# tailuzhecom/wiser

Hardware: AMD Instinct MI355X
Metric: queries/sec + p50 lat, 2-term AND BM25 top-10 on Wikipedia, 1/2/4/8 GPU (higher is better)
Workload: dtype u32/f64; 1 GPU; C3 stand-in (en-Wikipedia-shaped): 5500000 docs, the en-Wikipedia df histogram x 1 (gen_synthetic_log.py:8-16), 100000 two-term AND queries (:191-214 rule, seed 7), 4096 queries per GPU per step, top-10, device-resident; global_batch=4096, parallelism=replicas1, k=10

## Files before the change

include/wiser_hip.h:

```cpp
#ifndef WISER_HIP_H
#define WISER_HIP_H

#include <stdint.h>

#ifdef __cplusplus
extern "C" {
#endif

#define WSR_MAX_TERMS 16
#define WSR_MAX_QUERY_TERMS 1024
#define WSR_MAX_PHRASE_TERMS 8
#define WSR_MAX_OR_TERMS 16
#define WSR_MAX_K 1024
#define WSR_SERVER_MAX_K WSR_MAX_K

enum {
  WSR_OK = 0,
  WSR_E_INVALID = -1,
  WSR_E_IO = -2,
  WSR_E_HIP = -3,
  WSR_E_LIMIT = -4,
  WSR_E_INTERNAL = -5
};

typedef struct wsr_handle wsr_handle;
typedef struct wsr_batch wsr_batch;

typedef struct wsr_open_opts {
  int32_t device;
  uint32_t doc_lo;
  uint32_t doc_hi;
  int32_t threads;
  int32_t positions;
  int32_t bloom_factor;
} wsr_open_opts;

typedef struct wsr_query {
  int32_t n_terms;
  int32_t k;
  int32_t list_ids[WSR_MAX_TERMS];
  int32_t flags;
  const int32_t* more_ids;
} wsr_query;
#define WSR_QUERY_PHRASE 1
#define WSR_QUERY_OR 2

typedef struct wsr_hit {
  int32_t doc_id;
  int32_t pad;
  double score;
} wsr_hit;

int wsr_snippet(wsr_handle* h, const wsr_query* q, int32_t doc_id, int32_t n_passages,
                char* out, int32_t cap, int32_t* len);
int wsr_snippets_batch(wsr_handle* h, const wsr_query* q, int32_t nq, const wsr_hit* hits,
                       const int32_t* n_hits, int32_t stride, int32_t n_passages, int32_t threads,
                       char* buf, uint64_t cap, uint64_t* ends, uint64_t* total);
int wsr_doc_get(wsr_handle* h, int32_t doc_id, char* out, int32_t cap, int32_t* len);
typedef struct wsr_docs wsr_docs;
int wsr_docs_open(const char* dir, wsr_docs** out);
void wsr_docs_close(wsr_docs* d);
int wsr_docs_lookup(wsr_docs* d, const char* term, int32_t* list_id, int32_t* doc_freq);
int wsr_docs_snippet(wsr_docs* d, const wsr_query* q, int32_t doc_id, int32_t n_passages, char* out,
                     int32_t cap, int32_t* len);
int wsr_docs_get(wsr_docs* d, int32_t doc_id, char* out, int32_t cap, int32_t* len);
int wsr_highlight(const int32_t* pairs, const int32_t* counts, int32_t n_terms, int32_t n_passages,
                  const char* text, char* out, int32_t cap, int32_t* len);

typedef struct wsr_batch_stats {
  uint64_t work_items;
  uint64_t survivors;
  uint64_t driver_blocks;
  uint64_t other_blocks;
  uint64_t algo_bytes;
  double plan_ms, segment_ms, replay_ms;
  uint64_t events;
  uint64_t max_query_events;
  double lean_ms;
  uint64_t skippable_blocks;
} wsr_batch_stats;

typedef struct wsr_image_info {
  uint64_t total_bytes;
  uint64_t blob_bytes;
  uint64_t dense_bytes;
  uint64_t tf8_bytes;
  uint64_t plen_bytes;
  uint64_t dir_bytes;
  uint64_t pos_bytes;
  uint32_t n_lists, dense_lists;
  uint64_t impact_bytes;
} wsr_image_info;

const char* wsr_last_error(void);
const char* wsr_version(void);
int wsr_runtime_info(char* buf, int32_t cap);

int wsr_open(const char* vacuum_dir, const wsr_open_opts* opts, wsr_handle** out);
void wsr_close(wsr_handle* h);
int wsr_image_info_get(wsr_handle* h, wsr_image_info* out);
int wsr_image_size(const char* dir, uint32_t doc_lo, uint32_t doc_hi, int32_t positions, int32_t bloom_factor,
                   int32_t threads, wsr_image_info* out);
int wsr_term_count(wsr_handle* h, int32_t* out);
int wsr_n_docs(wsr_handle* h, int32_t* out);
int wsr_lookup(wsr_handle* h, const char* term, int32_t* list_id, int32_t* doc_freq);
int wsr_list_bytes(wsr_handle* h, int32_t list_id, uint64_t* out);
int wsr_impact_byte(double avg, uint32_t tf, uint32_t c4, uint32_t* byte, double* value);

int wsr_check_query(wsr_handle* h, const wsr_query* q);

int wsr_search_batch(wsr_handle* h, const wsr_query* q, int32_t nq, int32_t hit_stride,
                     wsr_hit* hits, int32_t* n_hits);

int wsr_resolve_text(wsr_handle* h, const char* text, int64_t len, int32_t k, int32_t max_q,
                     wsr_query* q, int32_t* nq, int32_t* more_store, int64_t more_cap);
int wsr_search_text(wsr_handle* h, const char* text, int64_t len, int32_t k, int32_t hit_stride,
                    int32_t max_q, wsr_hit* hits, int32_t* n_hits, int32_t* nq);

int wsr_class_order(const wsr_query* q, int32_t nq, int32_t* order, int32_t* n_conj);

int wsr_batch_create(wsr_handle* h, int32_t max_queries, int32_t hit_stride, wsr_batch** out);
void wsr_batch_destroy(wsr_handle* h, wsr_batch* b);
int wsr_batch_upload(wsr_handle* h, wsr_batch* b, const wsr_query* q, int32_t nq);
int wsr_batch_run(wsr_handle* h, wsr_batch* b);
int wsr_sync(wsr_handle* h);
int wsr_batch_fetch(wsr_handle* h, wsr_batch* b, wsr_hit* hits, int32_t* n_hits);
int wsr_batch_stats_get(wsr_handle* h, wsr_batch* b, wsr_batch_stats* out);
typedef struct wsr_or_stats {
  uint64_t items, windows, windows_skipped, touched_docs, events;
} wsr_or_stats;
int wsr_batch_or_stats_get(wsr_handle* h, wsr_batch* b, wsr_or_stats* out);
int wsr_batch_fetch_cols(wsr_handle* h, wsr_batch* b, wsr_hit* hits, int32_t* n_hits, int32_t cols);
int wsr_pinned_alloc(uint64_t bytes, void** out);
void wsr_pinned_free(void* p);
int wsr_batch_ready(wsr_handle* h, wsr_batch* b);

typedef struct wsr_server wsr_server;
typedef struct wsr_serve_stats {
  uint64_t queries;
  double seconds, qps;
  double p50_ms, p99_ms;
  uint64_t batches;
  double mean_batch;
  double queue_ms;
  double gpu_ms;
  double handoff_ms;
} wsr_serve_stats;
int wsr_server_open(wsr_handle* h, int32_t max_batch, int32_t window_us, wsr_server** out);
void wsr_server_close(wsr_server* s);
int wsr_server_search(wsr_server* s, const wsr_query* q, wsr_hit* hits, int32_t* n_hits);
int wsr_server_bench(wsr_server* s, const wsr_query* q, int32_t nq, int32_t n_clients,
                     int32_t depth, double seconds, wsr_serve_stats* st);

int wsr_batch_fetch_range(wsr_handle* h, wsr_batch* b, int32_t q0, int32_t nq, wsr_hit* hits,
                          int32_t* n_hits);
int wsr_stream(wsr_handle* h, void** stream);
int wsr_batch_stream(wsr_handle* h, wsr_batch* b, void** stream);
int wsr_shard_fill(wsr_handle* h, wsr_batch* b, int32_t n_owners, int64_t* owner_totals);

#define WSR_COMM_ID_BYTES 128
typedef struct wsr_comm wsr_comm;
int wsr_comm_unique_id(uint8_t* id );
int wsr_comm_open(const uint8_t* id, int32_t world, int32_t rank, int32_t device, wsr_comm** out);
void wsr_comm_close(wsr_comm* c);
int wsr_shard_step(wsr_handle* h, wsr_batch* b, wsr_comm* c, int32_t q_per_owner, int64_t slot);
int wsr_shard_steps(wsr_handle* h, wsr_batch* const* b, int32_t n, wsr_comm* c, int32_t q_per_owner,
                    int64_t slot);
int wsr_comm_flush(wsr_comm* c);
typedef struct wsr_comm_stats {
  int64_t groups, steps, replays_in_lean, replays_on_stream;
} wsr_comm_stats;
int wsr_comm_stats_get(wsr_comm* c, wsr_comm_stats* out);
typedef struct wsr_loopback wsr_loopback;
int wsr_loopback_create(int32_t world, wsr_loopback** out);
void wsr_loopback_destroy(wsr_loopback* l);
int wsr_comm_open_loopback(wsr_loopback* l, int32_t rank, int32_t device, wsr_comm** out);
int wsr_shard_step_regions(int32_t q_per_owner, int64_t slot, uint64_t* region_bytes);
int wsr_shard_step_emit(wsr_handle* h, wsr_batch* b, int32_t world, int32_t q_per_owner, int64_t slot,
                        void* host_send);
int wsr_shard_step_replay(wsr_handle* h, wsr_batch* b, int32_t rank, int32_t world, int32_t q_per_owner,
                          int64_t slot, const void* host_recv);
int wsr_shard_step_replay_deferred(wsr_handle* h, wsr_batch* b, int32_t rank, int32_t world, int32_t q_per_owner,
                                   int64_t slot, const void* host_recv);
int wsr_shard_step_emit_async(wsr_handle* h, wsr_batch* b, int32_t world, int32_t q_per_owner, int64_t slot,
                              void* host_send);
int wsr_batch_stream_sync(wsr_handle* h, wsr_batch* b);
int wsr_batch_set_item_blocks(wsr_handle* h, wsr_batch* b, int32_t blocks);

int wsr_debug_decode_block(wsr_handle* h, int32_t list_id, int32_t block, int32_t which,
                           uint32_t* out, int32_t* count);

int wsr_debug_wg_stats(wsr_handle* h, wsr_batch* b, uint32_t* out, int32_t max_words,
                       int32_t* n_wg, int32_t* stride);

enum {
  WSR_CLASS_TWO_CONJ = 1 << 0,
  WSR_CLASS_ONE_CONJ = 1 << 1,
  WSR_CLASS_HAS_PHRASE = 1 << 2,
  WSR_CLASS_TWO_PH = 1 << 3,
  WSR_CLASS_HAS_WIDE = 1 << 4,
  WSR_CLASS_GEN_PHRASE = 1 << 5,
  WSR_CLASS_HAS_CONJ_LEAN = 1 << 6,
  WSR_CLASS_HAS_GEN = 1 << 7,
  WSR_CLASS_HAS_OR = 1 << 8,
  WSR_CLASS_RAN_CONJ = 1 << 9,
  WSR_CLASS_RAN_GEN = 1 << 10
};
int wsr_debug_batch_class(wsr_handle* h, wsr_batch* b, uint32_t* flags);

int wsr_debug_fail_runs(int32_t n);

int wsr_debug_dense_lookup(const char* dir, uint32_t doc_lo, uint32_t doc_hi, uint32_t dense_div,
                           const char* term, const uint32_t* docs, int32_t n, int32_t* tf_out,
                           int32_t* is_dense);

typedef struct wsr_build_stats {
  int64_t n_docs, n_terms, n_postings, vacuum_bytes, docs_char4_ge_0x80;
  double avg_length;
} wsr_build_stats;

int wsr_build_from_linedoc(const char* linedoc, int64_t n_rows, const char* format,
                           const char* out_dir, wsr_build_stats* st);
int wsr_build_from_linedoc_bloom(const char* linedoc, int64_t n_rows, const char* format,
                                 const char* out_dir, float ratio, int32_t expected_entries,
                                 wsr_build_stats* st);
int wsr_build_synthetic(const char* out_dir, int64_t n_docs, int64_t vocab, double zipf_s,
                        uint64_t seed, int32_t with_positions, int32_t threads,
                        wsr_build_stats* st);
int wsr_build_wiki_standin(const char* out_dir, int64_t n_docs, double term_scale, uint64_t seed,
                           int32_t threads, wsr_build_stats* st);
int wsr_build_wiki_standin_topics(const char* out_dir, int64_t n_docs, double term_scale, uint64_t seed,
                                  int32_t threads, int32_t topics, int32_t topics_per_term, double affinity,
                                  wsr_build_stats* st);
int wsr_gen_two_term_log(const char* index_dir, int64_t n_queries, uint64_t seed,
                         const char* out_path, int64_t* n_written);
int wsr_gen_mixed_log(const char* index_dir, int64_t n_queries, uint64_t seed,
                      const char* out_path, int64_t* n_written);
int wsr_gen_single_term_log(const char* index_dir, int32_t high, int64_t n_queries, uint64_t seed,
                            const char* out_path, int64_t* n_written);
int wsr_gen_phrase_log(const char* index_dir, int64_t n_queries, uint64_t seed,
                       const char* out_path, int64_t* n_written);

#ifdef __cplusplus
}
#endif

#endif
```

wiser_amd/_capi.py:

```python
from __future__ import annotations

import ctypes as C
import os
import re

HERE = os.path.dirname(os.path.abspath(__file__))
LIB_PATH = os.environ.get("WISER_HIP_LIB") or os.path.join(HERE, "_lib", "libwiser_hip.so")
HEADER = os.path.join(os.path.dirname(HERE), "include", "wiser_hip.h")

MAX_TERMS = 16
MAX_QUERY_TERMS = 1024
MAX_PHRASE_TERMS = 8
MAX_OR_TERMS = 16
MAX_K = 1024
SERVER_MAX_K = MAX_K

WSR_OK = 0
E_INVALID, E_IO, E_HIP, E_LIMIT, E_INTERNAL = -1, -2, -3, -4, -5
ERRORS = {-1: "WSR_E_INVALID", -2: "WSR_E_IO", -3: "WSR_E_HIP", -4: "WSR_E_LIMIT",
          -5: "WSR_E_INTERNAL"}


QUERY_PHRASE = 1
QUERY_OR = 2

CLASS_BITS = {"two_conj": 1 << 0, "one_conj": 1 << 1, "has_phrase": 1 << 2, "two_ph": 1 << 3,
              "has_wide": 1 << 4, "gen_phrase": 1 << 5, "has_conj_lean": 1 << 6, "has_gen": 1 << 7,
              "has_or": 1 << 8, "ran_conj": 1 << 9, "ran_gen": 1 << 10}


class OpenOpts(C.Structure):
    _fields_ = [("device", C.c_int32), ("doc_lo", C.c_uint32), ("doc_hi", C.c_uint32),
                ("threads", C.c_int32), ("positions", C.c_int32), ("bloom_factor", C.c_int32)]


class Query(C.Structure):
    _fields_ = [("n_terms", C.c_int32), ("k", C.c_int32), ("list_ids", C.c_int32 * MAX_TERMS),
                ("flags", C.c_int32), ("more_ids", C.POINTER(C.c_int32))]


class Hit(C.Structure):
    _fields_ = [("doc_id", C.c_int32), ("pad", C.c_int32), ("score", C.c_double)]


class BatchStats(C.Structure):
    _fields_ = [("work_items", C.c_uint64), ("survivors", C.c_uint64),
                ("driver_blocks", C.c_uint64), ("other_blocks", C.c_uint64),
                ("algo_bytes", C.c_uint64), ("plan_ms", C.c_double),
                ("segment_ms", C.c_double), ("replay_ms", C.c_double),
                ("events", C.c_uint64), ("max_query_events", C.c_uint64),
                ("lean_ms", C.c_double), ("skippable_blocks", C.c_uint64)]


class OrStats(C.Structure):
    _fields_ = [("items", C.c_uint64), ("windows", C.c_uint64), ("windows_skipped", C.c_uint64),
                ("touched_docs", C.c_uint64), ("events", C.c_uint64)]


class ImageInfo(C.Structure):
    _fields_ = [("total_bytes", C.c_uint64), ("blob_bytes", C.c_uint64), ("dense_bytes", C.c_uint64),
                ("tf8_bytes", C.c_uint64), ("plen_bytes", C.c_uint64), ("dir_bytes", C.c_uint64),
                ("pos_bytes", C.c_uint64), ("n_lists", C.c_uint32), ("dense_lists", C.c_uint32),
                ("impact_bytes", C.c_uint64)]


class ServeStats(C.Structure):
    _fields_ = [("queries", C.c_uint64), ("seconds", C.c_double), ("qps", C.c_double),
                ("p50_ms", C.c_double), ("p99_ms", C.c_double), ("batches", C.c_uint64),
                ("mean_batch", C.c_double), ("queue_ms", C.c_double), ("gpu_ms", C.c_double),
                ("handoff_ms", C.c_double)]


class CommStats(C.Structure):
    _fields_ = [("groups", C.c_int64), ("steps", C.c_int64), ("replays_in_lean", C.c_int64),
                ("replays_on_stream", C.c_int64)]


class BuildStats(C.Structure):
    _fields_ = [("n_docs", C.c_int64), ("n_terms", C.c_int64), ("n_postings", C.c_int64),
                ("vacuum_bytes", C.c_int64), ("docs_char4_ge_0x80", C.c_int64),
                ("avg_length", C.c_double)]


class WiserError(RuntimeError):
    def __init__(self, code, msg):
        super().__init__(f"{ERRORS.get(code, code)}: {msg}")
        self.code = code


if not os.path.exists(LIB_PATH):
    raise ImportError(f"{LIB_PATH} is missing: build it with `make` or __graft_entry__.build() "
                      "(the HIP engine has no CPU fallback)")

lib = C.CDLL(LIB_PATH)

_P = C.c_void_p
_sigs = {
    "wsr_last_error": (C.c_char_p, []),
    "wsr_version": (C.c_char_p, []),
    "wsr_runtime_info": (C.c_int, [C.c_char_p, C.c_int32]),
    "wsr_open": (C.c_int, [C.c_char_p, C.POINTER(OpenOpts), C.POINTER(_P)]),
    "wsr_close": (None, [_P]),
    "wsr_image_info_get": (C.c_int, [_P, C.POINTER(ImageInfo)]),
    "wsr_image_size": (C.c_int, [C.c_char_p, C.c_uint32, C.c_uint32, C.c_int32, C.c_int32, C.c_int32,
                                 C.POINTER(ImageInfo)]),
    "wsr_term_count": (C.c_int, [_P, C.POINTER(C.c_int32)]),
    "wsr_n_docs": (C.c_int, [_P, C.POINTER(C.c_int32)]),
    "wsr_lookup": (C.c_int, [_P, C.c_char_p, C.POINTER(C.c_int32), C.POINTER(C.c_int32)]),
    "wsr_list_bytes": (C.c_int, [_P, C.c_int32, C.POINTER(C.c_uint64)]),
    "wsr_impact_byte": (C.c_int, [C.c_double, C.c_uint32, C.c_uint32, C.POINTER(C.c_uint32),
                                  C.POINTER(C.c_double)]),
    "wsr_search_batch": (C.c_int, [_P, C.POINTER(Query), C.c_int32, C.c_int32, C.POINTER(Hit),
                                   C.POINTER(C.c_int32)]),
    "wsr_check_query": (C.c_int, [_P, C.POINTER(Query)]),
    "wsr_resolve_text": (C.c_int, [_P, C.c_char_p, C.c_int64, C.c_int32, C.c_int32, C.POINTER(Query),
                                   C.POINTER(C.c_int32), C.POINTER(C.c_int32), C.c_int64]),
    "wsr_search_text": (C.c_int, [_P, C.c_char_p, C.c_int64, C.c_int32, C.c_int32, C.c_int32,
                                  C.POINTER(Hit), C.POINTER(C.c_int32), C.POINTER(C.c_int32)]),
    "wsr_class_order": (C.c_int, [C.POINTER(Query), C.c_int32, C.POINTER(C.c_int32), C.POINTER(C.c_int32)]),
    "wsr_batch_create": (C.c_int, [_P, C.c_int32, C.c_int32, C.POINTER(_P)]),
    "wsr_batch_destroy": (None, [_P, _P]),
    "wsr_batch_upload": (C.c_int, [_P, _P, C.POINTER(Query), C.c_int32]),
    "wsr_batch_run": (C.c_int, [_P, _P]),
    "wsr_sync": (C.c_int, [_P]),
    "wsr_batch_fetch": (C.c_int, [_P, _P, C.POINTER(Hit), C.POINTER(C.c_int32)]),
    "wsr_batch_stats_get": (C.c_int, [_P, _P, C.POINTER(BatchStats)]),
    "wsr_batch_or_stats_get": (C.c_int, [_P, _P, C.POINTER(OrStats)]),
    "wsr_batch_fetch_range": (C.c_int, [_P, _P, C.c_int32, C.c_int32, C.POINTER(Hit),
                                        C.POINTER(C.c_int32)]),
    "wsr_stream": (C.c_int, [_P, C.POINTER(_P)]),
    "wsr_batch_stream": (C.c_int, [_P, _P, C.POINTER(_P)]),
    "wsr_shard_fill": (C.c_int, [_P, _P, C.c_int32, C.POINTER(C.c_int64)]),
    "wsr_comm_unique_id": (C.c_int, [C.POINTER(C.c_uint8)]),
    "wsr_comm_open": (C.c_int, [C.POINTER(C.c_uint8), C.c_int32, C.c_int32, C.c_int32, C.POINTER(_P)]),
    "wsr_comm_close": (None, [_P]),
    "wsr_loopback_create": (C.c_int, [C.c_int32, C.POINTER(_P)]),
    "wsr_loopback_destroy": (None, [_P]),
    "wsr_comm_open_loopback": (C.c_int, [_P, C.c_int32, C.c_int32, C.POINTER(_P)]),
    "wsr_comm_flush": (C.c_int, [_P]),
    "wsr_comm_stats_get": (C.c_int, [_P, C.POINTER(CommStats)]),
    "wsr_shard_step": (C.c_int, [_P, _P, _P, C.c_int32, C.c_int64]),
    "wsr_shard_steps": (C.c_int, [_P, _P, C.c_int32, _P, C.c_int32, C.c_int64]),
    "wsr_shard_step_emit_async": (C.c_int, [_P, _P, C.c_int32, C.c_int32, C.c_int64, _P]),
    "wsr_batch_stream_sync": (C.c_int, [_P, _P]),
    "wsr_batch_set_item_blocks": (C.c_int, [_P, _P, C.c_int32]),
    "wsr_shard_step_regions": (C.c_int, [C.c_int32, C.c_int64, C.POINTER(C.c_uint64)]),
    "wsr_shard_step_emit": (C.c_int, [_P, _P, C.c_int32, C.c_int32, C.c_int64, _P]),
    "wsr_shard_step_replay": (C.c_int, [_P, _P, C.c_int32, C.c_int32, C.c_int32, C.c_int64, _P]),
    "wsr_shard_step_replay_deferred": (C.c_int, [_P, _P, C.c_int32, C.c_int32, C.c_int32, C.c_int64, _P]),
    "wsr_debug_wg_stats": (C.c_int, [_P, _P, C.POINTER(C.c_uint32), C.c_int32,
                                     C.POINTER(C.c_int32), C.POINTER(C.c_int32)]),
    "wsr_debug_batch_class": (C.c_int, [_P, _P, C.POINTER(C.c_uint32)]),
    "wsr_debug_fail_runs": (C.c_int, [C.c_int32]),
    "wsr_debug_decode_block": (C.c_int, [_P, C.c_int32, C.c_int32, C.c_int32,
                                         C.POINTER(C.c_uint32), C.POINTER(C.c_int32)]),
    "wsr_debug_dense_lookup": (C.c_int, [C.c_char_p, C.c_uint32, C.c_uint32, C.c_uint32, C.c_char_p,
                                         C.POINTER(C.c_uint32), C.c_int32, C.POINTER(C.c_int32),
                                         C.POINTER(C.c_int32)]),
    "wsr_build_from_linedoc": (C.c_int, [C.c_char_p, C.c_int64, C.c_char_p, C.c_char_p,
                                         C.POINTER(BuildStats)]),
    "wsr_build_from_linedoc_bloom": (C.c_int, [C.c_char_p, C.c_int64, C.c_char_p, C.c_char_p,
                                               C.c_float, C.c_int32, C.POINTER(BuildStats)]),
    "wsr_build_synthetic": (C.c_int, [C.c_char_p, C.c_int64, C.c_int64, C.c_double, C.c_uint64,
                                      C.c_int32, C.c_int32, C.POINTER(BuildStats)]),
    "wsr_build_wiki_standin": (C.c_int, [C.c_char_p, C.c_int64, C.c_double, C.c_uint64,
                                         C.c_int32, C.POINTER(BuildStats)]),
    "wsr_build_wiki_standin_topics": (C.c_int, [C.c_char_p, C.c_int64, C.c_double, C.c_uint64, C.c_int32,
                                                C.c_int32, C.c_int32, C.c_double, C.POINTER(BuildStats)]),
    "wsr_gen_two_term_log": (C.c_int, [C.c_char_p, C.c_int64, C.c_uint64, C.c_char_p,
                                       C.POINTER(C.c_int64)]),
    "wsr_batch_ready": (C.c_int, [_P, _P]),
    "wsr_pinned_alloc": (C.c_int, [C.c_uint64, C.POINTER(_P)]),
    "wsr_pinned_free": (None, [_P]),
    "wsr_batch_fetch_cols": (C.c_int, [_P, _P, C.POINTER(Hit), C.POINTER(C.c_int32), C.c_int32]),
    "wsr_server_open": (C.c_int, [_P, C.c_int32, C.c_int32, C.POINTER(_P)]),
    "wsr_server_close": (None, [_P]),
    "wsr_server_search": (C.c_int, [_P, C.POINTER(Query), C.POINTER(Hit), C.POINTER(C.c_int32)]),
    "wsr_server_bench": (C.c_int, [_P, C.POINTER(Query), C.c_int32, C.c_int32, C.c_int32,
                                   C.c_double, C.POINTER(ServeStats)]),
    "wsr_gen_mixed_log": (C.c_int, [C.c_char_p, C.c_int64, C.c_uint64, C.c_char_p,
                                    C.POINTER(C.c_int64)]),
    "wsr_gen_single_term_log": (C.c_int, [C.c_char_p, C.c_int32, C.c_int64, C.c_uint64, C.c_char_p,
                                          C.POINTER(C.c_int64)]),
    "wsr_gen_phrase_log": (C.c_int, [C.c_char_p, C.c_int64, C.c_uint64, C.c_char_p,
                                     C.POINTER(C.c_int64)]),
    "wsr_snippet": (C.c_int, [_P, C.POINTER(Query), C.c_int32, C.c_int32, C.c_char_p, C.c_int32,
                              C.POINTER(C.c_int32)]),
    "wsr_doc_get": (C.c_int, [_P, C.c_int32, C.c_char_p, C.c_int32, C.POINTER(C.c_int32)]),
    "wsr_snippets_batch": (C.c_int, [_P, C.POINTER(Query), C.c_int32, C.POINTER(Hit),
                                     C.POINTER(C.c_int32), C.c_int32, C.c_int32, C.c_int32, C.c_char_p,
                                     C.c_uint64, C.POINTER(C.c_uint64), C.POINTER(C.c_uint64)]),
    "wsr_docs_open": (C.c_int, [C.c_char_p, C.POINTER(_P)]),
    "wsr_docs_close": (None, [_P]),
    "wsr_docs_lookup": (C.c_int, [_P, C.c_char_p, C.POINTER(C.c_int32), C.POINTER(C.c_int32)]),
    "wsr_docs_snippet": (C.c_int, [_P, C.POINTER(Query), C.c_int32, C.c_int32, C.c_char_p, C.c_int32,
                                   C.POINTER(C.c_int32)]),
    "wsr_docs_get": (C.c_int, [_P, C.c_int32, C.c_char_p, C.c_int32, C.POINTER(C.c_int32)]),
    "wsr_highlight": (C.c_int, [C.POINTER(C.c_int32), C.POINTER(C.c_int32), C.c_int32, C.c_int32,
                                C.c_char_p, C.c_char_p, C.c_int32, C.POINTER(C.c_int32)]),
}
for _name, (_res, _args) in _sigs.items():
    _f = getattr(lib, _name)
    _f.restype = _res
    _f.argtypes = _args


def check(rc):
    if rc != WSR_OK:
        raise WiserError(rc, lib.wsr_last_error().decode(errors="replace"))
    return rc


def text_call(fn, *args, cap: int = 4096) -> str:
    while True:
        buf = C.create_string_buffer(cap)
        n = C.c_int32()
        check(fn(*args, buf, cap, C.byref(n)))
        if n.value <= cap:
            return buf.raw[: n.value].decode("utf-8", errors="surrogateescape")
        cap = n.value


def snippets_batch(h, queries, hits, n_hits, stride: int, n_passages: int, threads: int = 0):
    nq = len(n_hits)
    ends = (C.c_uint64 * max(1, nq * stride))()
    total = C.c_uint64()
    cap = 1 << 16
    while True:
        buf = C.create_string_buffer(cap)
        rc = lib.wsr_snippets_batch(h, queries, nq, hits, n_hits, stride, n_passages, threads, buf, cap,
                                    ends, C.byref(total))
        if rc == -4 and total.value > cap:
            cap = total.value
            continue
        check(rc)
        break
    raw = buf.raw
    out, at = [], 0
    for i in range(nq):
        row = []
        for j in range(stride):
            e = ends[i * stride + j]
            if j < n_hits[i]:
                row.append(raw[at:e].decode("utf-8", errors="surrogateescape"))
            at = e
        out.append(row)
    return out


def highlight(offsets, n_passages: int, text: str) -> str:
    flat = [v for term in offsets for pr in term for v in pr]
    pairs = (C.c_int32 * max(1, len(flat)))(*flat)
    counts = (C.c_int32 * max(1, len(offsets)))(*[len(t) for t in offsets])
    return text_call(lib.wsr_highlight, pairs, counts, len(offsets), n_passages, text.encode())


def header_symbols(path: str = HEADER):
    text = open(path).read()
    return sorted(set(re.findall(r"^\s*(?:const\s+)?[\w\s\*]+?\b(wsr_\w+)\s*\(", text, re.M)))


def runtime_info() -> str:
    buf = C.create_string_buffer(1024)
    check(lib.wsr_runtime_info(buf, 1024))
    return buf.value.decode()
```

wiser_amd/csrc/engine.cc:

```cpp
#include <hip/hip_runtime.h>
#include <rccl/rccl.h>
#include <dlfcn.h>

#include <cstdio>

#include <algorithm>
#include <atomic>
#include <cmath>
#include <cstring>
#include <memory>
#include <cstdlib>
#include <mutex>
#include <stdexcept>
#include <string>
#include <thread>
#include <vector>

#include "engine_impl.h"
#include "format.h"
#include "writer.h"

using namespace wiser;

namespace wiser {
thread_local std::string g_err;
void set_last_error(const std::string& msg) { g_err = msg; }
}

namespace {

template <class T, class A>
uint64_t dev_upload(gpu::DevBuf<T>& dst, const std::vector<T, A>& src) {
  dst.alloc(std::max<size_t>(src.size(), 1));
  if (!src.empty()) HIP_OK(hipMemcpy(dst.get(), src.data(), src.size() * sizeof(T), hipMemcpyHostToDevice));
  return dst.bytes();
}

}

namespace {
template <class V>
uint64_t dev_bytes(const V& v) {
  return std::max<uint64_t>(v.size(), 1) * sizeof(typename V::value_type);
}

wsr_image_info image_info_of(const HostImage& img, size_t n_c4) {
  wsr_image_info o{};
  if (img.has_blooms) o.pos_bytes += dev_bytes(img.blm) + dev_bytes(img.blm_hash);
  if (img.has_positions)
    o.pos_bytes += dev_bytes(img.pos_blob) + dev_bytes(img.pos_lists) + dev_bytes(img.pos_pk) +
                   dev_bytes(img.pos_tail) + dev_bytes(img.pos_start);
  o.dense_bytes = dev_bytes(img.dense) + dev_bytes(img.dense_rank) + dev_bytes(img.bkt);
  o.tf8_bytes = dev_bytes(img.tf8);
  o.blob_bytes = dev_bytes(img.blob);
  o.plen_bytes = dev_bytes(img.plen);
  o.dir_bytes = dev_bytes(img.tails) + dev_bytes(img.lists) + dev_bytes(img.blocks) + dev_bytes(img.blk_last) +
                dev_bytes(img.blk_meta) + dev_bytes(img.bmax) + std::max<uint64_t>(n_c4, 1);
  o.impact_bytes = dev_bytes(img.impact);
  o.dir_bytes += o.impact_bytes;
  o.dense_lists = img.dense_lists;
  o.n_lists = static_cast<uint32_t>(img.lists.size());
  o.total_bytes = o.blob_bytes + o.dense_bytes + o.tf8_bytes + o.plen_bytes + o.dir_bytes + o.pos_bytes;
  return o;
}

uint32_t dense_div_knob() { return static_cast<uint32_t>(env_number("WSR_DENSE_DIV", 8192)); }
uint64_t dense_budget_knob() { return static_cast<uint64_t>(env_number("WSR_DENSE_BUDGET_GB", 48) * 1e9); }
}

extern "C" {

const char* wsr_last_error(void) { return g_err.c_str(); }
const char* wsr_version(void) { return "wiser-hip 0.2 (gfx950)"; }

int wsr_image_info_get(wsr_handle* h, wsr_image_info* out) {
  if (!h || !out) return fail(WSR_E_INVALID, "null argument");
  *out = h->info;
  out->total_bytes = out->blob_bytes + out->dense_bytes + out->tf8_bytes + out->plen_bytes + out->dir_bytes +
                     out->pos_bytes;
  return WSR_OK;
}


int wsr_image_size(const char* dir, uint32_t doc_lo, uint32_t doc_hi, int32_t positions, int32_t bloom_factor,
                   int32_t threads, wsr_image_info* out) {
  if (!dir || !out) return fail(WSR_E_INVALID, "null argument");
  try {
    VacuumIndex idx;
    idx.open(dir);
    const int t = threads > 0 ? threads : static_cast<int>(std::thread::hardware_concurrency());
    const HostImage img = build_image(idx, doc_lo, doc_hi ? doc_hi : 0xFFFFFFFFu, std::min(t, 32), dense_div_knob(),
                                      positions != 0, dense_budget_knob(), positions && bloom_factor > 0);
    *out = image_info_of(img, idx.char4_lengths().size());
  } catch (const std::exception& e) {
    return fail(WSR_E_IO, e.what());
  }
  return WSR_OK;
}

int wsr_runtime_info(char* buf, int32_t cap) {
  if (!buf || cap <= 0) return fail(WSR_E_INVALID, "null argument");
  int ver = 0;
  (void)hipRuntimeGetVersion(&ver);
  Dl_info hip{}, rccl{};
  const char* hp = dladdr(reinterpret_cast<void*>(&hipRuntimeGetVersion), &hip) && hip.dli_fname ? hip.dli_fname : "?";
  const char* rp = dladdr(reinterpret_cast<void*>(&ncclGetUniqueId), &rccl) && rccl.dli_fname ? rccl.dli_fname : "?";
  std::snprintf(buf, static_cast<size_t>(cap), "hipRuntimeGetVersion=%d libamdhip64=%s librccl=%s", ver, hp, rp);
  return WSR_OK;
}

int wsr_open(const char* dir, const wsr_open_opts* opts, wsr_handle** out) {
  if (!dir || !out) return fail(WSR_E_INVALID, "null argument");
  *out = nullptr;
  std::unique_ptr<wsr_handle> h(new wsr_handle());
  try {
    h->idx.open(dir);
    h->docs.open(dir);
    h->rows.reset(new SkipRowCache(h->idx));
  } catch (const std::exception& e) {
    return fail(WSR_E_IO, e.what());
  }
  try {
    const int dev = opts ? opts->device : 0;
    int ndev = 0;
    if (hipGetDeviceCount(&ndev) != hipSuccess || ndev <= dev)
      return fail(WSR_E_HIP, "no HIP device " + std::to_string(dev) + " (MI355X required; no CPU fallback)");
    HIP_OK(hipSetDevice(dev));
    h->device = dev;
    uint32_t lo = opts ? opts->doc_lo : 0, hi = opts ? opts->doc_hi : 0;
    if (hi == 0) hi = 0xFFFFFFFFu;
    int threads = opts && opts->threads > 0 ? opts->threads : static_cast<int>(std::thread::hardware_concurrency());
    const uint32_t dense_div = dense_div_knob();
    const uint64_t dense_budget = dense_budget_knob();
    const float dense_ratio = static_cast<float>(env_number("WSR_DENSE_RATIO", 1.0));
    h->positions = opts && opts->positions;
    const uint32_t bloom_factor = opts && opts->bloom_factor > 0 ? static_cast<uint32_t>(opts->bloom_factor) : 0u;
    size_t hbm_free = 0, hbm_total = 0;
    HIP_OK(hipMemGetInfo(&hbm_free, &hbm_total));
    HostImage img = build_image(h->idx, lo, hi, std::min(threads, 32), dense_div, h->positions, dense_budget,
                                bloom_factor > 0, hbm_free);
    if (img.has_blooms) {
      h->info.pos_bytes += dev_upload(h->d_blm, img.blm);
      h->info.pos_bytes += dev_upload(h->d_blm_hash, img.blm_hash);
      h->args.blm = reinterpret_cast<const uint4*>(h->d_blm.get());
      h->args.blm_hash = reinterpret_cast<const uint2*>(h->d_blm_hash.get());
      h->args.blm_bits = img.blm_bits;
      h->args.blm_hashes = img.blm_hashes;
      h->args.bloom_factor = bloom_factor;
      big_vector<uint8_t>().swap(img.blm);
    }
    if (h->positions) {
      h->info.pos_bytes += dev_upload(h->d_pos_blob, img.pos_blob);
      h->info.pos_bytes += dev_upload(h->d_pos_lists, img.pos_lists);
      h->info.pos_bytes += dev_upload(h->d_pos_pk, img.pos_pk);
      h->info.pos_bytes += dev_upload(h->d_pos_tail, img.pos_tail);
      h->info.pos_bytes += dev_upload(h->d_pos_start, img.pos_start);
      h->args.pos_blob = h->d_pos_blob.get();
      h->args.pos_lists = h->d_pos_lists.get();
      h->args.pos_pk = reinterpret_cast<const uint2*>(h->d_pos_pk.get());
      h->args.pos_tail = h->d_pos_tail.get();
      h->args.pos_start = reinterpret_cast<const uint2*>(h->d_pos_start.get());
      h->pos_bytes = img.pos_list_bytes;
      std::vector<uint8_t>().swap(img.pos_blob);
      std::vector<uint32_t>().swap(img.pos_start);
    }
    h->info.dense_bytes = dev_upload(h->d_dense, img.dense);
    h->info.dense_bytes += dev_upload(h->d_dense_rk, img.dense_rank);
    h->info.dense_bytes += dev_upload(h->d_bkt, img.bkt);
    h->info.tf8_bytes = dev_upload(h->d_tf8, img.tf8);
    h->dense_lists = img.dense_lists;
    h->info.dense_lists = img.dense_lists;
    h->info.n_lists = static_cast<uint32_t>(img.lists.size());
    h->args.dense = h->d_dense.get();
    h->args.dense_rk = h->d_dense_rk.get();
    h->args.bkt = reinterpret_cast<const uint2*>(h->d_bkt.get());
    h->args.tf8 = h->d_tf8.get();
    h->args.dense_span = img.dense_span;
    h->args.dense_ratio = dense_ratio;
    h->args.seg_cap = kSegCost;
    h->info.blob_bytes = dev_upload(h->d_blob, img.blob);
    h->info.plen_bytes = dev_upload(h->d_plen, img.plen);
    h->args.plen = h->d_plen.get();
    h->info.impact_bytes = dev_upload(h->d_impact, img.impact);
    h->info.dir_bytes += h->info.impact_bytes;
    h->args.impact = h->d_impact.get();
    {
      float nm = static_cast<float>(img.norm_min);
      if (static_cast<double>(nm) > img.norm_min) nm = std::nextafter(nm, 0.0f);
      h->args.norm_min = nm;
    }
    h->info.dir_bytes += dev_upload(h->d_bmax, img.bmax);
    h->args.bmax = h->d_bmax.get();
    h->info.dir_bytes += dev_upload(h->d_tails, img.tails);
    h->args.tails = h->d_tails.get();
    h->info.dir_bytes += dev_upload(h->d_lists, img.lists);
    h->info.dir_bytes += dev_upload(h->d_blocks, img.blocks);
    h->info.dir_bytes += dev_upload(h->d_last, img.blk_last);
    h->info.dir_bytes += dev_upload(h->d_meta, img.blk_meta);
    h->info.dir_bytes += dev_upload(h->d_c4, h->idx.char4_lengths());
    std::vector<double> cache(h->idx.bm25_cache(), h->idx.bm25_cache() + 256);
    dev_upload(h->d_cache, cache);
    h->lists = img.lists;
    h->blocks.assign(img.blocks.begin(), img.blocks.end());
    h->meta.assign(img.blk_meta.begin(), img.blk_meta.end());
    h->list_bytes = img.list_bytes;
    h->args.blob = h->d_blob.get();
    h->args.lists = h->d_lists.get();
    h->args.blocks = h->d_blocks.get();
    h->args.blk_last = h->d_last.get();
    h->args.blk_meta = h->d_meta.get();
    h->args.c4 = h->d_c4.get();
    h->args.cache = h->d_cache.get();
    h->args.n_c4 = static_cast<uint32_t>(h->idx.char4_lengths().size());
    h->args.n_lists = static_cast<uint32_t>(img.lists.size());
    h->args.doc_lo = lo;
    h->args.doc_hi = hi;
    h->args.avg = h->idx.avg_length();
    h->stream = gpu::make_stream();

    hipDeviceProp_t prop;
    HIP_OK(hipGetDeviceProperties(&prop, dev));
    int occ = segment_kernel_occupancy();
    if (occ < 1) occ = 1;
    h->grid = prop.multiProcessorCount * std::min(occ, 32);
    const int gen_per_cu = static_cast<int>(env_number("WSR_GEN_PER_CU", 4));
    h->gen_cap = prop.multiProcessorCount * std::max(1, std::min(std::min(occ, 32), gen_per_cu) + 1);
    int locc = lean_kernel_occupancy(false);
    if (locc < 1) locc = 1;
    h->lean_wgs = prop.multiProcessorCount * std::min(locc, 16);
    int pocc = lean_kernel_occupancy(true);
    if (pocc < 1) pocc = 1;
    h->lean_wgs_ph = prop.multiProcessorCount * std::min(std::min(pocc, locc), 16);
    h->lean_wgs_two = prop.multiProcessorCount * std::min(locc + 1, 16);
  } catch (const std::exception& e) {
    return fail(WSR_E_HIP, e.what());
  }
  *out = h.release();
  return WSR_OK;
}

void wsr_close(wsr_handle* h) {
  if (!h) return;
  for (wsr_batch* b : h->pool) wsr_batch_destroy(h, b);
  h->pool.clear();
  if (h->stream) (void)hipStreamSynchronize(h->stream);
  delete h;
}

int wsr_term_count(wsr_handle* h, int32_t* out) {
  if (!h || !out) return fail(WSR_E_INVALID, "null argument");
  *out = h->idx.n_lists();
  return WSR_OK;
}

int wsr_n_docs(wsr_handle* h, int32_t* out) {
  if (!h || !out) return fail(WSR_E_INVALID, "null argument");
  *out = h->idx.n_docs();
  return WSR_OK;
}

int wsr_lookup(wsr_handle* h, const char* term, int32_t* list_id, int32_t* df) {
  if (!h || !term) return fail(WSR_E_INVALID, "null argument");
  const int32_t id = h->idx.find(term);
  if (list_id) *list_id = id;
  if (df) *df = id < 0 ? 0 : static_cast<int32_t>(h->idx.df(id));
  return WSR_OK;
}

struct wsr_docs {
  VacuumIndex idx;
  DocStore docs;
  std::unique_ptr<SkipRowCache> rows;
};

namespace {
int copy_out(const std::string& s, char* out, int32_t cap, int32_t* len) {
  if (len) *len = static_cast<int32_t>(s.size());
  if (out && cap > 0) std::memcpy(out, s.data(), std::min<size_t>(s.size(), static_cast<size_t>(cap)));
  return WSR_OK;
}

int check_snippet_query(const VacuumIndex& idx, const DocStore& docs, const wsr_query* q) {
  if (q->n_terms < 1 || q->n_terms > WSR_MAX_QUERY_TERMS) return fail(WSR_E_LIMIT, "bad term count");
  if (q->n_terms > WSR_MAX_TERMS && !q->more_ids) return fail(WSR_E_INVALID, "more_ids missing");
  if (q->flags & WSR_QUERY_OR) return fail(WSR_E_INVALID, "no snippets for a disjunctive query");
  if (!docs.is_open()) return fail(WSR_E_INVALID, "the index has no doc store (my.fdx / my.fdt)");
  for (int32_t id : query_terms(*q))
    if (id < 0 || id >= idx.n_lists())
      return fail(WSR_E_INVALID, "a query term is not in the index (no result entries)");
  return WSR_OK;
}

int snippet_of(const VacuumIndex& idx, const SkipRowCache& rows, const DocStore& docs, const wsr_query* q,
               int32_t doc, int32_t n_passages, char* out, int32_t cap, int32_t* len) {
  if (!q || !len || n_passages < 0) return fail(WSR_E_INVALID, "bad snippet arguments");
  const int rc = check_snippet_query(idx, docs, q);
  if (rc != WSR_OK) return rc;
  try {
    const std::vector<int32_t> ids = query_terms(*q);
    return copy_out(make_snippet(idx, rows, docs, ids.data(), q->n_terms,
                                 (q->flags & WSR_QUERY_PHRASE) != 0, doc, n_passages),
                    out, cap, len);
  } catch (const std::exception& e) {
    return fail(WSR_E_INVALID, e.what());
  }
}

int doc_text(const DocStore& docs, int32_t doc, char* out, int32_t cap, int32_t* len) {
  if (!len) return fail(WSR_E_INVALID, "null argument");
  try {
    return copy_out(docs.get(doc), out, cap, len);
  } catch (const std::exception& e) {
    return fail(WSR_E_INVALID, e.what());
  }
}
}

int wsr_snippet(wsr_handle* h, const wsr_query* q, int32_t doc, int32_t n_passages, char* out,
                int32_t cap, int32_t* len) {
  if (!h) return fail(WSR_E_INVALID, "null argument");
  return snippet_of(h->idx, *h->rows, h->docs, q, doc, n_passages, out, cap, len);
}

int wsr_snippets_batch(wsr_handle* h, const wsr_query* q, int32_t nq, const wsr_hit* hits,
                       const int32_t* n_hits, int32_t stride, int32_t n_passages, int32_t threads,
                       char* buf, uint64_t cap, uint64_t* ends, uint64_t* total) {
  if (!h || (nq > 0 && (!q || !hits || !n_hits || !ends)) || !total || nq < 0 || stride <= 0 ||
      n_passages < 0)
    return fail(WSR_E_INVALID, "bad snippet batch arguments");
  std::vector<std::pair<int32_t, int32_t>> work;
  for (int32_t i = 0; i < nq; ++i) {
    if (n_hits[i] < 0 || n_hits[i] > stride) return fail(WSR_E_INVALID, "bad hit count");
    if (n_hits[i] == 0) continue;
    const int rc = check_snippet_query(h->idx, h->docs, &q[i]);
    if (rc != WSR_OK) return rc;
    for (int32_t j = 0; j < n_hits[i]; ++j) work.emplace_back(i, j);
  }
  std::vector<std::string> out(static_cast<size_t>(nq) * stride);
// ... 578 lines not shown
  auto disj = [&](int32_t i) { return (q[i].flags & WSR_QUERY_OR) != 0; };
  auto phrase = [&](int32_t i) {
    return !disj(i) && (q[i].flags & WSR_QUERY_PHRASE) != 0 && q[i].n_terms > 1;
  };
  int32_t n = 0;
  for (int32_t i = 0; i < nq; ++i)
    if (!phrase(i) && !disj(i)) order[n++] = i;
  *n_conj = n;
  for (int32_t i = 0; i < nq; ++i)
    if (phrase(i)) order[n++] = i;
  for (int32_t i = 0; i < nq; ++i)
    if (disj(i)) order[n++] = i;
  return WSR_OK;
}

int wsr_shard_fill(wsr_handle* h, wsr_batch* b, int32_t n_owners, int64_t* owner_totals) {
  if (!h || !b || !b->x.fused || !owner_totals || n_owners <= 0 || n_owners > b->x.world)
    return fail(WSR_E_INVALID, "call wsr_shard_step (or wsr_shard_step_emit) first");
  try {
    HIP_OK(hipSetDevice(h->device));
    HIP_OK(hipStreamSynchronize(b->st));
    if (b->x.join()) HIP_OK(hipEventSynchronize(b->x.ev[1]));
    std::vector<uint32_t> fill(n_owners);
    HIP_OK(hipMemcpy(fill.data(), b->d_ctr + kNumCounters, sizeof(uint32_t) * n_owners, hipMemcpyDeviceToHost));
    for (int i = 0; i < n_owners; ++i) owner_totals[i] = fill[i];
  } catch (const std::exception& e) {
    return fail(WSR_E_HIP, e.what());
  }
  return WSR_OK;
}

int wsr_batch_stream(wsr_handle* h, wsr_batch* b, void** stream) {
  if (!h || !b || !stream) return fail(WSR_E_INVALID, "null argument");
  *stream = b->st;
  return WSR_OK;
}

int wsr_batch_set_item_blocks(wsr_handle* h, wsr_batch* b, int32_t blocks) {
  if (!h || !b || blocks < 1 || blocks > kSegCost) return fail(WSR_E_INVALID, "item blocks must be 1..63");
  b->seg_cap = static_cast<uint32_t>(blocks);
  return WSR_OK;
}

int wsr_batch_stream_sync(wsr_handle* h, wsr_batch* b) {
  if (!h || !b) return fail(WSR_E_INVALID, "null argument");
  const hipError_t e = hipStreamSynchronize(b->st);
  return e == hipSuccess ? WSR_OK : fail(WSR_E_HIP, hipGetErrorString(e));
}

int wsr_batch_fetch_range(wsr_handle* h, wsr_batch* b, int32_t q0, int32_t nq, wsr_hit* hits,
                          int32_t* n_hits) {
  if (!h || !b || q0 < 0 || nq < 0 || q0 + nq > b->nq) return fail(WSR_E_INVALID, "bad range");
  try {
    HIP_OK(hipSetDevice(h->device));
    HIP_OK(hipStreamSynchronize(b->st));
    if (b->x.join()) HIP_OK(hipEventSynchronize(b->x.ev[1]));
    uint32_t ctr[kNumCounters];
    HIP_OK(hipMemcpy(ctr, b->d_ctr, sizeof ctr, hipMemcpyDeviceToHost));
    if (ctr[kCtrError])
      return fail(WSR_E_INTERNAL, "device reported error flags " + std::to_string(ctr[kCtrError]) +
                                      (ctr[kCtrError] & kErrExchange ? " (an exchange slot overflowed)" : ""));
    if (nq && hits)
      HIP_OK(hipMemcpy(hits, b->d_hits + static_cast<size_t>(q0) * b->stride,
                       sizeof(HitDev) * static_cast<size_t>(nq) * b->stride, hipMemcpyDeviceToHost));
    if (nq && n_hits)
      HIP_OK(hipMemcpy(n_hits, b->d_nhits + q0, sizeof(int32_t) * nq, hipMemcpyDeviceToHost));
  } catch (const std::exception& e) {
    return fail(WSR_E_HIP, e.what());
  }
  return WSR_OK;
}

int wsr_stream(wsr_handle* h, void** stream) {
  if (!h || !stream) return fail(WSR_E_INVALID, "null argument");
  *stream = h->stream;
  return WSR_OK;
}

int wsr_debug_decode_block(wsr_handle* h, int32_t id, int32_t block, int32_t which, uint32_t* out,
                           int32_t* count) {
  if (!h || !out || id < 0 || id >= static_cast<int32_t>(h->lists.size()))
    return fail(WSR_E_INVALID, "bad list id");
  const ListDev& L = h->lists[id];
  if (block < 0 || static_cast<uint32_t>(block) >= L.nblk) return fail(WSR_E_INVALID, "bad block");
  std::lock_guard<std::mutex> g(h->mu);
  const BlockDev& bd = h->blocks[L.blk0 + block];
  const uint32_t cnt = static_cast<uint32_t>(block) == L.nblk - 1 ? L.tail_cnt : 128u;
  try {
    gpu::DevBuf<uint32_t> d_out;
    d_out.alloc(128);
    const uint8_t* p = h->d_blob.get() + L.base + (which ? bd.tf_rel : bd.doc_rel);
    const uint32_t bits = which ? (h->meta[L.blk0 + block] >> 8) : (h->meta[L.blk0 + block] & 0xFF);
    HIP_OK(launch_decode_probe(p, bits, cnt, which == 0, bd.prev, d_out, h->stream));
    HIP_OK(hipStreamSynchronize(h->stream));
    HIP_OK(hipMemcpy(out, d_out, d_out.bytes(), hipMemcpyDeviceToHost));
  } catch (const std::exception& ex) {
    return fail(WSR_E_HIP, ex.what());
  }
  if (count) *count = static_cast<int32_t>(cnt);
  return WSR_OK;
}

int wsr_debug_wg_stats(wsr_handle* h, wsr_batch* b, uint32_t* out, int32_t max_words,
                       int32_t* n_wg, int32_t* stride) {
  if (!h || !b) return fail(WSR_E_INVALID, "null argument");
  std::lock_guard<std::mutex> g(h->mu);
  const int rows = b->cls.seg_grid + kLeanWaves * (b->cls.lean_wgs + (b->cls.has_phrase ? b->cls.lean_wgs_ph : 0));
  if (n_wg) *n_wg = rows;
  if (stride) *stride = kStatStride;
  if (!out) return WSR_OK;
  const size_t n = std::min<size_t>(static_cast<size_t>(std::max(max_words, 0)),
                                    static_cast<size_t>(kStatStride) * rows);
  try {
    HIP_OK(hipStreamSynchronize(b->st));
    if (b->x.join()) HIP_OK(hipEventSynchronize(b->x.ev[1]));
    HIP_OK(hipMemcpy(out, b->d_stats, n * sizeof(uint32_t), hipMemcpyDeviceToHost));
  } catch (const std::exception& e) {
    return fail(WSR_E_HIP, e.what());
  }
  return WSR_OK;
}

int wsr_debug_batch_class(wsr_handle* h, wsr_batch* b, uint32_t* flags) {
  if (!h || !b || !flags) return fail(WSR_E_INVALID, "null argument");
  const BatchClass& c = b->cls;
  *flags = (c.two_conj ? WSR_CLASS_TWO_CONJ : 0u) | (c.one_conj ? WSR_CLASS_ONE_CONJ : 0u) |
           (c.has_phrase ? WSR_CLASS_HAS_PHRASE : 0u) | (c.two_ph ? WSR_CLASS_TWO_PH : 0u) |
           (c.has_wide ? WSR_CLASS_HAS_WIDE : 0u) | (c.gen_phrase ? WSR_CLASS_GEN_PHRASE : 0u) |
           (c.has_conj_lean ? WSR_CLASS_HAS_CONJ_LEAN : 0u) | (c.has_gen ? WSR_CLASS_HAS_GEN : 0u) |
           (c.has_or ? WSR_CLASS_HAS_OR : 0u) | (b->launched.conj ? WSR_CLASS_RAN_CONJ : 0u) |
           (b->launched.gen ? WSR_CLASS_RAN_GEN : 0u);
  return WSR_OK;
}

int wsr_debug_dense_lookup(const char* dir, uint32_t doc_lo, uint32_t doc_hi, uint32_t dense_div,
                           const char* term, const uint32_t* docs, int32_t n, int32_t* tf_out,
                           int32_t* is_dense) {
  if (!dir || !term || (n > 0 && (!docs || !tf_out))) return fail(WSR_E_INVALID, "null argument");
  try {
    VacuumIndex idx;
    idx.open(dir);
    const HostImage img = build_image(idx, doc_lo, doc_hi ? doc_hi : 0xFFFFFFFFu, 4, dense_div);
    const int32_t id = idx.find(term);
    const bool dense = id >= 0 && img.lists[id].bm != kNoDense;
    if (is_dense) *is_dense = dense ? 1 : 0;
    for (int32_t i = 0; i < n; ++i)
      tf_out[i] = dense ? static_cast<int32_t>(dense_lookup_host(img, img.lists[id], docs[i])) : -1;
  } catch (const std::exception& e) {
    return fail(WSR_E_IO, e.what());
  }
  return WSR_OK;
}

static void fill_stats(const BuildStats& s, wsr_build_stats* st) {
  if (!st) return;
  st->n_docs = s.n_docs;
  st->n_terms = s.n_terms;
  st->n_postings = s.n_postings;
  st->vacuum_bytes = s.vacuum_bytes;
  st->docs_char4_ge_0x80 = s.docs_char4_ge_0x80;
  st->avg_length = s.avg_length;
}

int wsr_build_from_linedoc(const char* linedoc, int64_t n_rows, const char* format,
                           const char* out_dir, wsr_build_stats* st) {
  if (!linedoc || !format || !out_dir) return fail(WSR_E_INVALID, "null argument");
  try {
    fill_stats(build_from_linedoc(linedoc, n_rows, format, out_dir), st);
  } catch (const std::exception& e) {
    return fail(WSR_E_IO, e.what());
  }
  return WSR_OK;
}

int wsr_build_from_linedoc_bloom(const char* linedoc, int64_t n_rows, const char* format,
                                 const char* out_dir, float ratio, int32_t expected_entries,
                                 wsr_build_stats* st) {
  if (!linedoc || !format || !out_dir) return fail(WSR_E_INVALID, "null argument");
  if (!(ratio > 0.0f && ratio < 1.0f) || expected_entries < 1)
    return fail(WSR_E_INVALID, "bloom ratio must be in (0, 1) and expected entries >= 1");
  try {
    BloomSpec b;
    b.on = true;
    b.ratio = ratio;
    b.entries = expected_entries;
    fill_stats(build_from_linedoc(linedoc, n_rows, format, out_dir, b), st);
  } catch (const std::exception& e) {
    return fail(WSR_E_IO, e.what());
  }
  return WSR_OK;
}

int wsr_build_synthetic(const char* out_dir, int64_t n_docs, int64_t vocab, double zipf_s,
                        uint64_t seed, int32_t with_positions, int32_t threads,
                        wsr_build_stats* st) {
  if (!out_dir || n_docs <= 0 || vocab <= 0) return fail(WSR_E_INVALID, "bad arguments");
  try {
    SyntheticSpec sp;
    sp.n_docs = n_docs;
    sp.vocab = vocab;
    sp.zipf_s = zipf_s;
    sp.seed = seed;
    sp.with_positions = with_positions != 0;
    sp.threads = threads;
    fill_stats(build_synthetic(sp, out_dir), st);
  } catch (const std::exception& e) {
    return fail(WSR_E_IO, e.what());
  }
  return WSR_OK;
}

int wsr_build_wiki_standin(const char* out_dir, int64_t n_docs, double term_scale, uint64_t seed,
                           int32_t threads, wsr_build_stats* st) {
  if (!out_dir || n_docs < 16 || !(term_scale > 0)) return fail(WSR_E_INVALID, "bad arguments");
  try {
    WikiSpec sp;
    sp.n_docs = n_docs;
    sp.term_scale = term_scale;
    sp.seed = seed;
    sp.threads = threads;
    fill_stats(build_wiki_standin(sp, out_dir), st);
  } catch (const std::exception& e) {
    return fail(WSR_E_IO, e.what());
  }
  return WSR_OK;
}

int wsr_build_wiki_standin_topics(const char* out_dir, int64_t n_docs, double term_scale, uint64_t seed,
                                  int32_t threads, int32_t topics, int32_t topics_per_term, double affinity,
                                  wsr_build_stats* st) {
  if (!out_dir || n_docs < 16 || !(term_scale > 0) || topics < 1 || topics_per_term < 1 || topics_per_term > 16 ||
      !(affinity >= 0 && affinity <= 1) || topics > n_docs)
    return fail(WSR_E_INVALID, "bad arguments");
  try {
    WikiSpec sp;
    sp.n_docs = n_docs;
    sp.term_scale = term_scale;
    sp.seed = seed;
    sp.threads = threads;
    sp.topics = topics;
    sp.topics_per_term = topics_per_term;
    sp.affinity = affinity;
    fill_stats(build_wiki_standin(sp, out_dir), st);
  } catch (const std::exception& e) {
    return fail(WSR_E_IO, e.what());
  }
  return WSR_OK;
}

int wsr_gen_two_term_log(const char* index_dir, int64_t n_queries, uint64_t seed,
                         const char* out_path, int64_t* n_written) {
  if (!index_dir || !out_path) return fail(WSR_E_INVALID, "null argument");
  try {
    int64_t n = gen_two_term_log(index_dir, n_queries, seed, out_path);
    if (n_written) *n_written = n;
  } catch (const std::exception& e) {
    return fail(WSR_E_IO, e.what());
  }
  return WSR_OK;
}

int wsr_gen_mixed_log(const char* index_dir, int64_t n_queries, uint64_t seed,
                      const char* out_path, int64_t* n_written) {
  if (!index_dir || !out_path) return fail(WSR_E_INVALID, "null argument");
  try {
    int64_t n = gen_mixed_log(index_dir, n_queries, seed, out_path);
    if (n_written) *n_written = n;
  } catch (const std::exception& e) {
    return fail(WSR_E_IO, e.what());
  }
  return WSR_OK;
}

int wsr_gen_single_term_log(const char* index_dir, int32_t high, int64_t n_queries, uint64_t seed,
                      const char* out_path, int64_t* n_written) {
  if (!index_dir || !out_path) return fail(WSR_E_INVALID, "null argument");
  try {
    int64_t n = gen_single_term_log(index_dir, high != 0, n_queries, seed, out_path);
    if (n_written) *n_written = n;
  } catch (const std::exception& e) {
    return fail(WSR_E_IO, e.what());
  }
  return WSR_OK;
}

int wsr_gen_phrase_log(const char* index_dir, int64_t n_queries, uint64_t seed,
                       const char* out_path, int64_t* n_written) {
  if (!index_dir || !out_path) return fail(WSR_E_INVALID, "null argument");
  try {
    int64_t n = gen_phrase_log(index_dir, n_queries, seed, out_path);
    if (n_written) *n_written = n;
  } catch (const std::exception& e) {
    return fail(WSR_E_IO, e.what());
  }
  return WSR_OK;
}

}
```

wiser_amd/csrc/engine_impl.h:

```cpp
#pragma once

#include <hip/hip_runtime.h>

#include <atomic>
#include <cstdlib>
#include <deque>
#include <memory>
#include <mutex>
#include <string>
#include <vector>

#include "../../include/wiser_hip.h"
#include "batch_plan.h"
#include "dev_mem.h"
#include "engine_types.h"
#include "index.h"
#include "kernels.h"
#include "shard_layout.h"
#include "snippet.h"

namespace wiser {
extern thread_local std::string g_err;
inline int fail(int code, const std::string& msg) {
  g_err = msg;
  return code;
}

inline double env_number(const char* name, double dflt) {
  const char* v = std::getenv(name);
  if (!v || !*v) return dflt;
  char* end = nullptr;
  const double x = std::strtod(v, &end);
  return (end && *end == 0 && x >= 0) ? x : dflt;
}
}

struct wsr_handle {
  std::mutex mu;
  int device = 0;
  gpu::Stream stream;
  wiser::VacuumIndex idx;
  wiser::DocStore docs;
  std::unique_ptr<wiser::SkipRowCache> rows;
  std::mutex pool_mu;
  std::vector<wsr_batch*> pool;
  wiser::IndexArgs args{};
  gpu::DevBuf<uint8_t> d_blob;
  gpu::DevBuf<wiser::ListDev> d_lists;
  gpu::DevBuf<wiser::BlockDev> d_blocks;
  gpu::DevBuf<uint32_t> d_last, d_meta;
  gpu::DevBuf<uint8_t> d_c4;
  gpu::DevBuf<double> d_cache;
  gpu::DevBuf<wiser::DenseEnt> d_dense;
  gpu::DevBuf<uint32_t> d_dense_rk;
  gpu::DevBuf<uint32_t> d_bkt;
  gpu::DevBuf<uint8_t> d_tf8, d_plen, d_impact;
  gpu::DevBuf<float> d_bmax;
  gpu::DevBuf<uint32_t> d_tails;
  gpu::DevBuf<uint8_t> d_pos_blob;
  gpu::DevBuf<wiser::PosDev> d_pos_lists;
  gpu::DevBuf<uint32_t> d_pos_pk, d_pos_tail, d_pos_start;
  gpu::DevBuf<uint8_t> d_blm;
  gpu::DevBuf<uint32_t> d_blm_hash;
  bool positions = false;
  uint32_t dense_lists = 0;
  wsr_image_info info{};
  std::vector<wiser::ListDev> lists;
  std::vector<uint64_t> list_bytes;
  std::vector<uint64_t> pos_bytes;
  std::vector<wiser::BlockDev> blocks;
  std::vector<uint32_t> meta;
  std::mutex hdef_mu;
  std::deque<wsr_batch*> hdef_q;
  int grid = 0;
  int lean_wgs = 0;
  int lean_wgs_ph = 0;
  int lean_wgs_two = 0;
  int gen_cap = 0;
  wiser::ImageView view() const {
    wiser::ImageView v;
    v.lists = lists.data();
    v.n_lists = lists.size();
    v.blocks = blocks.data();
    v.n_blocks = blocks.size();
    v.list_bytes = list_bytes.data();
    v.pos_bytes = pos_bytes.empty() ? nullptr : pos_bytes.data();
    v.dense_ratio = args.dense_ratio;
    v.doc_lo = args.doc_lo;
    v.doc_hi = args.doc_hi;
    v.positions = positions;
    v.lean_wgs = lean_wgs;
    v.lean_wgs_two = lean_wgs_two;
    v.lean_wgs_ph = lean_wgs_ph;
    v.gen_cap = gen_cap;
    return v;
  }
};

struct ShardExchange {
  explicit ShardExchange(wsr_batch* b) : batch(b) {}
  wsr_batch* const batch;
  gpu::DevBuf<wiser::Event> send, recv;
  int pairs = 0;
  gpu::Event ev[2];
  std::atomic<bool> pending{false};
  std::atomic<uint64_t> req{0};
  std::atomic<uint64_t> enq{0};
  std::atomic<wsr_comm*> comm{nullptr};
  bool fused = false;
  std::atomic<wsr_handle*> hdef{nullptr};
  int32_t hdef_rank = 0;
  int world = 0, qpr = 0;
  int64_t slot = 0;
  wiser::ShardLayout layout() const { return wiser::ShardLayout(qpr, slot); }

  void request() { req.fetch_add(1, std::memory_order_acq_rel); }
  void enqueued(bool ok, bool deferred) {
    if (ok) pending = true;
    if (deferred) comm.store(nullptr, std::memory_order_release);
    enq.fetch_add(1, std::memory_order_release);
  }
  bool join();
};

struct wsr_batch {
  int max_q = 0, stride = 0, nq = 0;
  gpu::DevBuf<uint8_t> d_qb;
  wiser::QueryIn* d_q() const { return reinterpret_cast<wiser::QueryIn*>(d_qb.get()); }
  gpu::DevBuf<wiser::QueryPlan> d_plan;
  gpu::DevBuf<wiser::QueryDesc> d_desc;
  gpu::DevBuf<wiser::PlanPart> d_part;
  gpu::DevBuf<uint32_t> d_ctr;
  gpu::PinnedBuf<uint32_t> h_ctr;
  gpu::DevBuf<wiser::Event> d_events;
  gpu::DevBuf<uint32_t> d_evcnt, d_itemq;
  gpu::DevBuf<wiser::HitDev> d_hits;
  gpu::DevBuf<int32_t> d_nhits;
  gpu::DevBuf<uint32_t> d_qdone;
  gpu::DevBuf<uint64_t> d_pub;
  gpu::DevBuf<uint32_t> d_stats;
  gpu::DevBuf<uint32_t> d_ph;
  wiser::BatchClass cls;
  wiser::Launches launched;
  uint32_t seg_cap = wiser::kSegCost;
  ShardExchange x{this};
  gpu::DevBuf<wiser::OrQuery> d_orq;
  gpu::DevBuf<wiser::OrItem> d_oritem;
  gpu::DevBuf<uint32_t> d_orevcnt;
  gpu::DevBuf<wiser::Event> d_orev;
  gpu::DevBuf<unsigned long long> d_orstat;
  gpu::Event ev[5];
  gpu::Stream st, st2, st_pad;
  gpu::Event fork, join, join_ph;
  bool ran = false;
};

int batch_run(wsr_handle* h, wsr_batch* b, const wiser::EmitView* se = nullptr, const wiser::OwnerJob* oj = nullptr);
wsr_batch* take_host_replay(wsr_handle* h, const wsr_batch* b, wiser::OwnerJob* oj);
bool host_replay_enqueue(wsr_batch* pb, wsr_handle* h);
```

wiser_amd/csrc/engine_types.h:

```cpp
#pragma once

#include <cstdint>

namespace wiser {

constexpr int kMaxTerms = 16;
constexpr int kMaxQueryTerms = 1024;
constexpr int kMaxPhraseTerms = 8;
constexpr int kMaxK = 64;
constexpr int kMaxKWide = 1024;

struct ListDev {
  uint64_t base;
  uint32_t blk0;
  uint32_t nblk;
  uint32_t df;
  uint32_t tail_cnt;
  double idf;
  uint64_t bm;
  uint64_t tf8;
  uint64_t tail;
  uint32_t last;
  uint32_t tfmax;
};
static_assert(sizeof(ListDev) == 64, "ListDev layout");
constexpr uint64_t kNoTail = ~0ull;

constexpr uint64_t kNoDense = ~0ull;
constexpr uint8_t kTf8Escape = 255;

constexpr float kImpactScale = 0x1.010102p-8f;
inline double impact_value(uint32_t q) { return static_cast<double>(static_cast<float>(q) * kImpactScale); }
inline uint8_t impact_byte(uint32_t tf, double nrm) {
  const double f = static_cast<double>(static_cast<int32_t>(tf));
  const double x = f / (f + nrm);
  if (!(x > 0.0)) return 0;
  if (!(x < 1.0)) return 255;
  uint32_t q = static_cast<uint32_t>(x * 255.0);
  while (q < 255 && impact_value(q) < x) ++q;
  return static_cast<uint8_t>(q);
}

constexpr uint32_t kProbeShiftBit = 56;
constexpr uint64_t kProbeBaseMask = (1ull << kProbeShiftBit) - 1;
constexpr uint32_t kBucketDensity = 40;
constexpr uint32_t kBucketMinShift = 3, kBucketMaxShift = 8;
constexpr uint32_t kBucketInline = 4;
constexpr uint32_t kBucketWindow = 9;
constexpr uint32_t kBucketCrowdedDiv = 1024;
inline uint32_t probe_shift(uint64_t bm) { return static_cast<uint32_t>(bm >> kProbeShiftBit); }
inline uint64_t bucket_count(uint32_t span, uint32_t c) { return (static_cast<uint64_t>(span) + (1u << c) - 1) >> c; }
inline uint32_t bucket_shift(uint64_t n, uint32_t span) {
  if (!span || n * kBucketDensity >= span || n >= (1u << 23) - 1024) return 0;
  uint32_t c = kBucketMinShift;
  while (c < kBucketMaxShift && (n << (c + 1)) <= 2ull * span) ++c;
  return c;
}
inline uint64_t bucket_words(uint64_t n, uint32_t span, uint32_t c) {
  return 2 * bucket_count(span, c) + (n + 7) / 8 * 2;
}

constexpr uint32_t kDenseDocs = 32;
struct DenseEnt {
  uint32_t w;
};
static_assert(sizeof(DenseEnt) == 4, "DenseEnt layout");
constexpr uint32_t kRankWords = 2;
constexpr uint64_t kDenseEntBytes = 4 + 4 * kRankWords;

inline bool dense_ent_bit(const DenseEnt& e, uint32_t sh) { return (e.w >> sh) & 1u; }
inline uint32_t dense_ent_rank(const DenseEnt& e, uint32_t rank, uint32_t sh) {
  return rank + static_cast<uint32_t>(__builtin_popcount(e.w & ((1u << sh) - 1u)));
}

struct BlockDev {
  uint32_t prev;
  uint32_t last;
  uint32_t doc_rel;
  uint32_t tf_rel;
};
static_assert(sizeof(BlockDev) == 16, "BlockDev layout");

struct QueryIn {
  int32_t n_terms;
  int32_t k;
  int32_t list[kMaxTerms];
  int32_t flags;
  uint32_t ext;
};
static_assert(sizeof(QueryIn) == 80, "QueryIn layout");
constexpr int32_t kQueryPhrase = 1;

constexpr int kLeanWaves = 4;
constexpr int kSegCost = 63;
static_assert(kSegCost < 64, "a segment's driver directory is one entry per lane");
constexpr int kSingleWindows = 8;

template <class Image>
constexpr bool probe_by_bitmap(const Image& ix, bool has_bm, uint32_t nblk_b, uint32_t nblk_driver) {
  return has_bm && static_cast<float>(nblk_b) >= ix.dense_ratio * static_cast<float>(nblk_driver);
}
constexpr bool is_phrase_query(int32_t n_terms, int32_t flags) { return n_terms > 1 && (flags & kQueryPhrase); }
constexpr bool is_lean_query(bool others_by_bitmap, int32_t n_terms, int32_t flags) {
  return others_by_bitmap && !(n_terms > 2 && (flags & kQueryPhrase));
}

struct PosDev {
  uint64_t base;
  uint64_t tail;
  uint32_t pk0;
  uint32_t npk;
};
static_assert(sizeof(PosDev) == 24, "PosDev layout");

struct QueryPlan {
  uint32_t item_base;
  uint32_t n_items;
  uint32_t seg_blocks;
  uint32_t driver;
  uint64_t ev_base;
};
static_assert(sizeof(QueryPlan) == 24, "QueryPlan layout");

struct QueryDesc {
  uint64_t a_base;
  uint64_t a_tail;
  uint64_t o_bm;
  uint64_t o_tf8;
  uint64_t ev_base;
  uint64_t rsv0, rsv1;
  double a_idf, o_idf;
  uint32_t a_blk0, a_nblk, a_tail_cnt;
  uint32_t min_last;
  uint32_t item_base, n_items, seg;
  uint32_t slots;
  uint32_t o_list;
  uint32_t k;
  float b_id, b_iom, b_m;
  uint32_t nt;
};
static_assert(sizeof(QueryDesc) == 128, "QueryDesc layout");
constexpr uint32_t kNoSlot = 0xFFFFu;

constexpr int32_t kQueryOr = 2;
constexpr int kMaxOrTerms = 16;
constexpr uint32_t kOrWindow = 2048;
struct OrQuery {
  int32_t q;
  int32_t k;
  int32_t nt;
  uint32_t item_base;
  uint32_t n_items;
  uint32_t pad;
  int32_t list[kMaxOrTerms];
  double ubsum[kMaxOrTerms];
};
static_assert(sizeof(OrQuery) == 216, "OrQuery layout");
struct OrItem {
  uint32_t oq;
  uint32_t doc_lo, doc_hi;
  uint32_t ev_cap;
  uint64_t ev_base;
};
static_assert(sizeof(OrItem) == 24, "OrItem layout");
enum { kOrStatItems = 0, kOrStatWindows, kOrStatSkipped, kOrStatTouched, kOrStatEvents, kNumOrStats };

struct Event {
  double score;
  int32_t doc;
  int32_t pad;
};
static_assert(sizeof(Event) == 16, "Event layout");

struct HitDev {
  int32_t doc;
  int32_t pad;
  double score;
};
static_assert(sizeof(HitDev) == 16, "HitDev layout");

struct OwnerJob {
  const QueryIn* qs;
  const int32_t* meta;
  const Event* recv;
  HitDev* hits;
  int32_t* n_hits;
  uint32_t* counters;
  uint64_t meta_stride, stride;
  int32_t q0, nq, n_shards, hit_stride;
};

}
```

wiser_amd/csrc/index.cc:

```cpp
#include "index.h"

#include <algorithm>
#include <atomic>
#include <chrono>
#include <cstdio>
#include <cstdlib>
#include <cmath>
#include <cstring>
#include <fcntl.h>
#include <fstream>
#include <limits>
#include <mutex>
#include <stdexcept>
#include <sys/mman.h>
#include <sys/stat.h>
#include <thread>
#include <unistd.h>

#include "bloom.h"
#include "format.h"

namespace wiser {

VacuumIndex::~VacuumIndex() {
// ... 151 lines not shown
    {
      const size_t n = ents.size();
      const int nt = static_cast<int>(std::max<size_t>(1, std::min<size_t>(16, n / 65536)));
      std::atomic<size_t> bad{~size_t{0}};
      auto work = [&](int t) {
        for (size_t i = n * t / nt; i < n * (t + 1) / nt; ++i) {
          Ent& e = ents[i];
          uint64_t df = 0;
          if (e.off + 2 > map_len_ || map_[e.off] != kPostingListMagic ||
              !get_varint(map_ + e.off + 1, map_ + map_len_, &df) || df == 0) {
            size_t cur = bad.load();
            while (i < cur && !bad.compare_exchange_weak(cur, i)) {}
            return;
          }
          e.df = df;
        }
      };
      std::vector<std::thread> ts;
      for (int t = 1; t < nt; ++t) ts.emplace_back(work, t);
      work(0);
      for (auto& t : ts) t.join();
      if (bad.load() != ~size_t{0})
        throw std::runtime_error("posting list of '" + all.substr(ents[bad].at, ents[bad].len) +
                                 "' has a wrong magic byte or a bad doc freq");
    }
    uint64_t cap = 16;
    while (cap < 2 * ents.size()) cap <<= 1;
    tslot_.assign(cap, 0);
    tmask_ = cap - 1;
    terms_.reserve(ents.size());
    off_.reserve(ents.size());
    df_.reserve(ents.size());
    for (const Ent& e : ents) {
      const uint64_t off = e.off, df = e.df;
      const int32_t next = static_cast<int32_t>(terms_.size());
      terms_.emplace_back(all, e.at, e.len);
      const int32_t id = insert_term(terms_.back().data(), terms_.back().size(), next);
      if (id != next) {
        terms_.pop_back();
        off_[id] = off;
        df_[id] = static_cast<uint32_t>(df);
        continue;
      }
      off_.push_back(off);
      df_.push_back(static_cast<uint32_t>(df));
    }
  }
  idf_.resize(df_.size());
  for (size_t i = 0; i < df_.size(); ++i) {
    const int N = n_docs_, d = static_cast<int>(df_[i]);
    idf_[i] = std::log(1 + (N - d + 0.5) / (d + 0.5));
  }
}

std::vector<SkipRow> VacuumIndex::rows(int32_t id) const {
  std::vector<SkipRow> out;
  rows_into(id, &out);
  return out;
}

void VacuumIndex::rows_into(int32_t id, std::vector<SkipRow>* dst) const {
  const uint8_t* end = map_ + map_len_;
  const uint8_t* p = map_ + off_[id];
  uint64_t v;
  int l = get_varint(p + 1, end, &v);
  if (!l) throw std::runtime_error("bad df varint");
  p += 1 + l + 8;
  if (p >= end || p[0] != kSkipListMagic) throw std::runtime_error("bad skip list magic");
  uint64_t n = 0;
  l = get_varint(p + 1, end, &n);
  p += 1 + l;
  if (n > map_len_) throw std::runtime_error("bad skip list length");
  std::vector<SkipRow>& out = *dst;
  out.resize(n);
  uint64_t pd = 0, pdo = 0, pto = 0, ppo = 0, poo = 0;
  for (uint64_t r = 0; r < n; ++r) {
    uint64_t f[7];
    for (int k = 0; k < 7; ++k) {
      l = get_varint(p, end, &f[k]);
      if (!l) throw std::runtime_error("truncated skip list");
      p += l;
    }
    pd = static_cast<uint32_t>(pd + f[0]);
    pdo += f[1]; pto += f[2]; ppo += f[3]; poo += f[5];
    out[r] = SkipRow{static_cast<uint32_t>(pd), pdo, pto, ppo, static_cast<uint32_t>(f[4]), poo,
                     static_cast<uint32_t>(f[6])};
  }
}

bool host_decode_block(const uint8_t* p, const uint8_t* end, int cnt, bool delta,
                       uint32_t prev, uint32_t* out) {
  if (p >= end) return false;
  if (p[0] == kPackMagic) {
    if (cnt != kPackSize || p + 2 > end) return false;
    const int b = p[1];
    if (b < 1 || b > 32 || p + 2 + 16 * b > end) return false;
    const uint8_t* d = p + 2;
    const uint64_t mask = b == 32 ? 0xFFFFFFFFull : ((1ull << b) - 1);
    for (int j = 0; j < kPackSize; ++j) {
      const uint64_t bit = static_cast<uint64_t>(j) * b;
      uint64_t w = 0;
      const uint64_t at = bit >> 3, avail = 16u * b - at;
      std::memcpy(&w, d + at, avail < 8 ? avail : 8);
      out[j] = static_cast<uint32_t>((w >> (bit & 7)) & mask);
    }
  } else if (p[0] == kVIntsMagic) {
    uint64_t nb = 0;
    int l = get_varint(p + 1, end, &nb);
    if (!l) return false;
    const uint8_t* q = p + 1 + l;
    const uint8_t* qe = q + nb;
    if (qe > end) return false;
    for (int j = 0; j < cnt; ++j) {
      uint64_t v;
      int m = get_varint(q, qe, &v);
      if (!m) return false;
      q += m;
      out[j] = static_cast<uint32_t>(v);
    }
  } else {
    return false;
  }
  if (delta) {
    uint32_t acc = prev;
    for (int j = 0; j < cnt; ++j) { acc += out[j]; out[j] = acc; }
  }
  return true;
}

namespace {
template <class F>
void for_each_list(int32_t L, int threads, F&& fn) {
  std::atomic<int32_t> next{0};
  std::atomic<bool> failed{false};
  std::string err;
  std::mutex err_mu;
  auto work = [&](int worker) {
    try {
      for (int32_t s; (s = next.fetch_add(256)) < L && !failed;)
        for (int32_t id = s; id < std::min(L, s + 256) && !failed; ++id) fn(id, worker);
    } catch (const std::exception& ex) {
      std::lock_guard<std::mutex> g(err_mu);
      if (!failed.exchange(true)) err = ex.what();
    }
  };
  std::vector<std::thread> ts;
  for (int i = 1; i < threads; ++i) ts.emplace_back(work, i);
  work(0);
  for (auto& t : ts) t.join();
  if (failed) throw std::runtime_error(err);
}
}

HostImage build_image(const VacuumIndex& idx, uint32_t doc_lo, uint32_t doc_hi, int threads,
                      uint32_t dense_div, bool positions, uint64_t dense_budget, bool blooms,
                      uint64_t hbm_free) {
  const int32_t L = idx.n_lists();
  const uint8_t* file = idx.file();
  const uint8_t* fend = file + idx.file_bytes();
  const uint64_t span_end = std::min<uint64_t>(doc_hi, static_cast<uint64_t>(std::max(idx.n_docs(), 0)));
  const uint32_t span = span_end > doc_lo ? static_cast<uint32_t>(span_end - doc_lo) : 0u;
  const uint64_t n_ent = (static_cast<uint64_t>(span) + kDenseDocs - 1) / kDenseDocs;
  const std::vector<uint8_t>& c4 = idx.char4_lengths();
  const double* norm = idx.bm25_cache();
  struct Info {
    uint32_t r0 = 0, r1 = 0;
    uint32_t fcnt = 0;
    uint32_t tail_cnt = 0;
    uint64_t bytes = 0;
    uint8_t dense = 0, vtail = 0;
    uint8_t shift = 0;
  };
  std::vector<Info> info(L);
  struct Scratch {
    std::vector<SkipRow> rows;
    std::vector<uint32_t> last, docs, tfs;
    bool code_used[256] = {false};
  };
  if (threads < 1) threads = 1;
  std::vector<Scratch> scratch(threads);
  auto load_rows = [&](int32_t id, Scratch& s, uint32_t* fcnt) {
    idx.rows_into(id, &s.rows);
    const uint32_t df = idx.df(id);
    const uint64_t nrows = s.rows.size();
    if (nrows == 0 || nrows != (df + kPackSize - 1) / kPackSize)
      throw std::runtime_error("skip rows do not match df for '" + idx.term(id) + "'");
    s.last.resize(nrows);
    for (uint64_t r = 0; r + 1 < nrows; ++r) s.last[r] = s.rows[r + 1].prev_doc;
    *fcnt = static_cast<uint32_t>(df - kPackSize * (nrows - 1));
    uint32_t tmp[kPackSize];
    if (!host_decode_block(file + s.rows[nrows - 1].doc_off, fend, static_cast<int>(*fcnt), true,
                           s.rows[nrows - 1].prev_doc, tmp))
      throw std::runtime_error("cannot decode the last block of '" + idx.term(id) + "'");
    s.last[nrows - 1] = tmp[*fcnt - 1];
  };
  auto row_cnt = [](const Info& in, uint64_t r, uint64_t nrows) {
    return r + 1 == nrows ? static_cast<int>(in.fcnt) : kPackSize;
  };

  const bool timing = std::getenv("WSR_LOAD_TIMING") != nullptr;
  auto t_mark = std::chrono::steady_clock::now();
  auto lap = [&](const char* what) {
    if (!timing) return;
    const auto now = std::chrono::steady_clock::now();
    std::fprintf(stderr, "[wsr load] %s %.3f s\n", what, std::chrono::duration<double>(now - t_mark).count());
    t_mark = now;
  };
  for_each_list(L, threads, [&](int32_t id, int worker) {
    Scratch& s = scratch[worker];
    Info& in = info[id];
    load_rows(id, s, &in.fcnt);
    const uint64_t nrows = s.rows.size();
    uint64_t r0 = nrows, r1 = 0;
    for (uint64_t r = 0; r < nrows; ++r) {
      const bool below_hi = (r == 0) || (static_cast<uint64_t>(s.rows[r].prev_doc) + 1 < doc_hi);
      if (below_hi && s.last[r] >= doc_lo) { r0 = std::min(r0, r); r1 = r + 1; }
    }
    if (r0 >= r1) { in.r0 = in.r1 = 0; return; }
    in.r0 = static_cast<uint32_t>(r0);
    in.r1 = static_cast<uint32_t>(r1);
    const uint64_t d0 = s.rows[r0].doc_off;
    const uint64_t d1 = s.rows[r1 - 1].doc_off + blob_bytes(file + s.rows[r1 - 1].doc_off, fend);
    const uint64_t t0 = s.rows[r0].tf_off;
    const uint64_t t1 = s.rows[r1 - 1].tf_off + blob_bytes(file + s.rows[r1 - 1].tf_off, fend);
    if (d1 <= d0 || t1 <= t0 || d1 > idx.file_bytes() || t1 > idx.file_bytes() ||
        d1 - d0 + (t1 - t0) >= (1ull << 32))
      throw std::runtime_error("bad blob span for '" + idx.term(id) + "'");
    in.bytes = (d1 - d0) + (t1 - t0);
    in.tail_cnt = (r1 == nrows) ? in.fcnt : kPackSize;
    in.vtail = r1 == nrows && file[s.rows[nrows - 1].doc_off] == kVIntsMagic;
    const uint64_t n_img = (r1 - r0 - 1) * kPackSize + in.tail_cnt;
    if (dense_div && span && n_img * dense_div >= span) {
      bool ok = true;
      const uint64_t lim = static_cast<uint64_t>(doc_lo) + span;
      for (uint64_t r = r0; r < r1 && ok; ++r) {
        if (s.last[r] < lim) continue;
        if (r > 0 && static_cast<uint64_t>(s.rows[r].prev_doc) + 1 >= doc_hi) continue;
        uint32_t docs[kPackSize];
        const int cnt = row_cnt(in, r, nrows);
        if (!host_decode_block(file + s.rows[r].doc_off, fend, cnt, true, s.rows[r].prev_doc, docs))
          throw std::runtime_error("cannot decode a block for the dense image");
        for (int i = 0; i < cnt; ++i)
          if (docs[i] >= lim && docs[i] < doc_hi) ok = false;
      }
      in.dense = ok;
      uint64_t n_in = 0;
      for (uint64_t r = r0; r < r1 && ok; ++r) {
        const int cnt = row_cnt(in, r, nrows);
        const bool inside = (r == 0 ? doc_lo == 0 : s.rows[r].prev_doc + 1ull >= doc_lo) && s.last[r] < lim;
        if (inside) {
          n_in += static_cast<uint64_t>(cnt);
        } else {
          uint32_t docs[kPackSize];
          if (!host_decode_block(file + s.rows[r].doc_off, fend, cnt, true, s.rows[r].prev_doc, docs))
            throw std::runtime_error("cannot decode a block for the dense image");
          for (int i = 0; i < cnt; ++i) n_in += docs[i] >= doc_lo && docs[i] < lim;
        }
      }
      in.shift = static_cast<uint8_t>(bucket_shift(n_in, span));
      if (in.shift) {
        const uint32_t c = in.shift;
        uint64_t crowded = 0, run = 0, cur = ~0ull;
        for (uint64_t r = r0; r < r1; ++r) {
          uint32_t docs[kPackSize];
          const int cnt = row_cnt(in, r, nrows);
          if (!host_decode_block(file + s.rows[r].doc_off, fend, cnt, true, s.rows[r].prev_doc, docs))
            throw std::runtime_error("cannot decode a block for the dense image");
          for (int i = 0; i < cnt; ++i) {
            if (docs[i] < doc_lo || docs[i] >= lim) continue;
            const uint64_t bk = (docs[i] - doc_lo) >> c;
            if (bk != cur) { cur = bk; run = 0; }
            if (++run == kBucketWindow + 1) ++crowded;
          }
        }
        if (crowded * kBucketCrowdedDiv > bucket_count(span, c)) in.shift = 0;
      }
    }
  });

  lap("pass 1 (sizes)");
  if (hbm_free) {
    uint64_t other = static_cast<uint64_t>(std::max(idx.n_docs(), 0));
    for (int32_t id = 0; id < L; ++id) {
      const Info& in = info[id];
      if (in.r1 <= in.r0) continue;
      const uint64_t nbl = in.r1 - in.r0;
      other += in.bytes + nbl * (sizeof(BlockDev) + 12 + 2 * kPackSize) + (in.vtail ? 8ull * in.tail_cnt : 0);
      if (blooms && positions) other += nbl * kPackSize * 32;
    }
    const uint64_t cap = hbm_free / 10 * 9;
    const uint64_t room = cap > other ? cap - other : 0;
    if (!dense_budget || dense_budget > room) dense_budget = room ? room : 1;
  }
  if (dense_budget) {
    std::vector<std::pair<uint64_t, int32_t>> cand;
    for (int32_t id = 0; id < L; ++id)
      if (info[id].dense)
        cand.emplace_back((info[id].r1 - info[id].r0 - 1) * uint64_t{kPackSize} + info[id].tail_cnt, id);
    std::sort(cand.begin(), cand.end(), [](const auto& a, const auto& b) {
      return a.first != b.first ? a.first > b.first : a.second < b.second;
    });
    uint64_t used = 0;
    for (const auto& c : cand) {
      const uint32_t sh = info[c.second].shift;
      const uint64_t bytes = (sh ? 4 * bucket_words(c.first, span, sh) : n_ent * kDenseEntBytes) + c.first;
      if (used + bytes > dense_budget) info[c.second].dense = 0;
      else used += bytes;
    }
  }
  HostImage img;
  img.doc_lo = doc_lo;
  img.doc_hi = doc_hi;
  img.dense_span = span;
  img.lists.resize(L);
  img.list_bytes.resize(L);
  img.has_positions = positions;
  uint64_t at = 0, nb = 0, ne = 0, ntf8 = 0, ntail = 0, nbk = 0;
  for (int32_t id = 0; id < L; ++id) {
    const Info& in = info[id];
    ListDev& ld = img.lists[id];
    const uint32_t nbl = in.r1 > in.r0 ? in.r1 - in.r0 : 0u;
    ld.base = at;
    ld.blk0 = static_cast<uint32_t>(nb);
    ld.nblk = nbl;
    ld.df = idx.df(id);
    ld.tail_cnt = nbl ? in.tail_cnt : 0u;
    ld.idf = idx.idf(id);
    ld.bm = kNoDense;
    ld.tf8 = 0;
    ld.tail = kNoTail;
    ld.last = 0;
    ld.tfmax = 0;
    if (!nbl) { img.list_bytes[id] = 0; continue; }
    if (in.vtail) { ld.tail = ntail; ntail += 2ull * in.tail_cnt; }
    if (in.dense) {
      const uint64_t n_img = (nbl - 1) * static_cast<uint64_t>(kPackSize) + in.tail_cnt;
      if (in.shift) {
        ld.bm = (static_cast<uint64_t>(in.shift) << kProbeShiftBit) | (nbk / 2);
        nbk += bucket_words(n_img, span, in.shift);
        ++img.bucket_lists;
      } else {
        ld.bm = ne;
        ne += n_ent;
      }
      ld.tf8 = ntf8;
      ntf8 += n_img;
      ++img.dense_lists;
    }
    img.list_bytes[id] = in.bytes;
    img.docid_tf_bytes += in.bytes;
    at += (in.bytes + 15) & ~15ull;
    nb += nbl;
  }
  if (nb >= (1ull << 32)) throw std::runtime_error("more than 2^32 blocks in one image");
  img.blob.resize(at + 64);
  std::memset(&img.blob[at], 0, 64);
  img.blocks.resize(nb);
  img.blk_last.resize(nb);
  img.blk_meta.resize(nb);
  img.plen.resize(nb * kPackSize);
  img.impact.resize(nb * kPackSize);
  img.bmax.resize(nb);
  img.tails.resize(ntail);
  img.dense.resize(ne);
  img.dense_rank.resize(kRankWords * ne);
  img.tf8.resize(ntf8);
  img.bkt.resize(nbk + 4);
  for (uint64_t i = nbk; i < nbk + 4; ++i) img.bkt[i] = 0;

  lap("pass 2 (offsets, allocation)");
  struct PosPart {
    std::vector<uint8_t> bytes;
    std::vector<uint32_t> pk, tail;
  };
  std::vector<PosPart> pos_parts(positions ? L : 0);
  if (positions) {
    img.pos_start.assign(2 * nb * kPackSize, 0);
  }
  const BloomShape bshape(static_cast<int>(idx.bloom_entries()), idx.bloom_ratio());
  const uint32_t bbytes = idx.bloom_bytes();
  const bool with_blm = blooms && positions && idx.has_bloom() && bbytes >= 1 && bbytes <= 16 &&
                        bshape.bits > 0 && static_cast<uint32_t>(bshape.bits) <= 8 * bbytes && bshape.hashes > 0;
  if (with_blm) {
    img.has_blooms = true;
    img.blm_bits = static_cast<uint32_t>(bshape.bits);
    img.blm_hashes = static_cast<uint32_t>(bshape.hashes);
    img.blm.resize(nb * kPackSize * 32);
    img.blm_hash.assign(2 * static_cast<size_t>(L), 0);
  }
  for_each_list(L, threads, [&](int32_t id, int worker) {
    const Info& in = info[id];
    if (with_blm) {
      const std::string& t = idx.term(id);
      const uint32_t a = murmurhash2(t.data(), static_cast<int>(t.size()), 0x9747b28c);
      img.blm_hash[2 * id] = a;
      img.blm_hash[2 * id + 1] = murmurhash2(t.data(), static_cast<int>(t.size()), a);
    }
    if (in.r1 <= in.r0) return;
    Scratch& s = scratch[worker];
    uint32_t fcnt;
    load_rows(id, s, &fcnt);
    const uint64_t nrows = s.rows.size();
    const uint64_t r0 = in.r0, r1 = in.r1;
    const ListDev& ld = img.lists[id];
    const uint64_t d0 = s.rows[r0].doc_off;
    const uint64_t d1 = s.rows[r1 - 1].doc_off + blob_bytes(file + s.rows[r1 - 1].doc_off, fend);
    const uint64_t t0 = s.rows[r0].tf_off;
    const uint64_t t1 = s.rows[r1 - 1].tf_off + blob_bytes(file + s.rows[r1 - 1].tf_off, fend);
    std::memcpy(&img.blob[ld.base], file + d0, d1 - d0);
    std::memcpy(&img.blob[ld.base + (d1 - d0)], file + t0, t1 - t0);
    const uint64_t gap = ((in.bytes + 15) & ~15ull) - in.bytes;
    if (gap) std::memset(&img.blob[ld.base + in.bytes], 0, gap);
    const uint64_t n_img = (r1 - r0 - 1) * kPackSize + in.tail_cnt;
    if (in.dense) { s.docs.resize(n_img); s.tfs.resize(n_img); }
    uint32_t tfmax = 0;
    for (uint64_t r = r0; r < r1; ++r) {
      const uint64_t j = ld.blk0 + (r - r0);
      img.blocks[j] = BlockDev{s.rows[r].prev_doc, s.last[r], static_cast<uint32_t>(s.rows[r].doc_off - d0),
                               static_cast<uint32_t>((d1 - d0) + s.rows[r].tf_off - t0)};
      img.blk_last[j] = s.last[r];
      if (r == r1 - 1) img.lists[id].last = s.last[r];
      const uint8_t* pd = file + s.rows[r].doc_off;
      const uint8_t* pf = file + s.rows[r].tf_off;
      const uint32_t bd = pd[0] == kPackMagic ? pd[1] : 0u;
      const uint32_t bf = pf[0] == kPackMagic ? pf[1] : 0u;
      if ((pd[0] != kPackMagic && pd[0] != kVIntsMagic) || (pf[0] != kPackMagic && pf[0] != kVIntsMagic) ||
          bd > 32 || bf > 32 || (pd[0] == kPackMagic && bd == 0) || (pf[0] == kPackMagic && bf == 0))
        throw std::runtime_error("bad blob header in '" + idx.term(id) + "'");
      img.blk_meta[j] = bd | (bf << 8);
      const int cnt = row_cnt(in, r, nrows);
      uint32_t docs[kPackSize], tfs[kPackSize];
      if (!host_decode_block(pd, fend, cnt, true, s.rows[r].prev_doc, docs))
        throw std::runtime_error("cannot decode a block of '" + idx.term(id) + "'");
      uint8_t* o = &img.plen[j * kPackSize];
      for (int i = 0; i < cnt; ++i) o[i] = docs[i] < c4.size() ? c4[docs[i]] : 0;
      for (int i = cnt; i < kPackSize; ++i) o[i] = 0;
      const bool last_vints = in.vtail && r + 1 == nrows;
      if (!host_decode_block(pf, fend, cnt, false, 0, tfs))
        throw std::runtime_error("cannot decode the tfs of '" + idx.term(id) + "'");
      double bm = 0.0;
      for (int i = 0; i < cnt; ++i) {
        tfmax = std::max(tfmax, tfs[i]);
        const double f = static_cast<double>(static_cast<int32_t>(tfs[i]));
        const double t = (f * (1.2 + 1)) / (f + norm[o[i]]);
        bm = t > bm ? t : bm;
      }
      uint8_t* im = &img.impact[j * kPackSize];
      for (int i = 0; i < cnt; ++i) {
        im[i] = impact_byte(tfs[i], norm[o[i]]);
        s.code_used[o[i]] = true;
      }
      for (int i = cnt; i < kPackSize; ++i) im[i] = 0;
      float bmf = static_cast<float>(bm);
      if (static_cast<double>(bmf) < bm) bmf = std::nextafter(bmf, std::numeric_limits<float>::infinity());
      img.bmax[j] = bmf;
      if (last_vints) {
        std::memcpy(&img.tails[ld.tail], docs, cnt * sizeof(uint32_t));
        std::memcpy(&img.tails[ld.tail + cnt], tfs, cnt * sizeof(uint32_t));
      }
      if (in.dense) {
        std::memcpy(&s.docs[(r - r0) * kPackSize], docs, cnt * sizeof(uint32_t));
        std::memcpy(&s.tfs[(r - r0) * kPackSize], tfs, cnt * sizeof(uint32_t));
      }
    }
    img.lists[id].tfmax = tfmax;
    if (in.dense && in.shift) {
      const uint32_t c = in.shift, w = 1u << c;
      const uint64_t nbkt = bucket_count(span, c);
      uint32_t* ent = &img.bkt[2 * (ld.bm & kProbeBaseMask)];
      uint8_t* offs = reinterpret_cast<uint8_t*>(ent + 2 * nbkt);
      uint64_t i = 0;
      for (uint64_t e = 0; e < nbkt; ++e) {
        const uint64_t start = doc_lo + (e << c);
        while (i < n_img && s.docs[i] < start) ++i;
        uint64_t j = i;
        uint32_t in4 = 0xFFFFFFFFu;
        while (j < n_img && s.docs[j] < start + w) {
          const uint32_t o = static_cast<uint32_t>(s.docs[j] - start);
          offs[j] = static_cast<uint8_t>(o);
          if (j - i < kBucketInline) in4 = (in4 & ~(0xFFu << (8 * (j - i)))) | (o << (8 * (j - i)));
          ++j;
        }
        ent[2 * e] = static_cast<uint32_t>(i << 9 | (j - i));
        ent[2 * e + 1] = in4;
      }
      for (uint64_t j = n_img; j < (n_img + 7) / 8 * 8; ++j) offs[j] = 0;
      uint8_t* t8 = &img.tf8[ld.tf8];
      for (uint64_t j = 0; j < n_img; ++j) t8[j] = static_cast<uint8_t>(s.tfs[j] < kTf8Escape ? s.tfs[j] : kTf8Escape);
    } else if (in.dense) {
      DenseEnt* de = &img.dense[ld.bm];
      uint64_t i = 0;
      for (uint64_t e = 0; e < n_ent; ++e) {
        const uint64_t start = doc_lo + e * kDenseDocs;
        while (i < n_img && s.docs[i] < start) ++i;
        DenseEnt ent{};
        img.dense_rank[kRankWords * (ld.bm + e)] = static_cast<uint32_t>(i);
        uint32_t t4 = 0xFFFFFFFFu;
        for (uint64_t j = i, n = 0; n < 4 && j < n_img && s.docs[j] < start + kDenseDocs; ++j, ++n) {
          const uint32_t t = s.tfs[j] < kTf8Escape ? s.tfs[j] : kTf8Escape;
          t4 = (t4 & ~(0xFFu << (8 * n))) | (t << (8 * n));
        }
        img.dense_rank[kRankWords * (ld.bm + e) + 1] = t4;
        for (uint64_t j = i; j < n_img && s.docs[j] < start + kDenseDocs; ++j)
          ent.w |= 1u << static_cast<uint32_t>(s.docs[j] - start);
        de[e] = ent;
      }
      uint8_t* t8 = &img.tf8[ld.tf8];
      for (uint64_t j = 0; j < n_img; ++j) t8[j] = static_cast<uint8_t>(s.tfs[j] < kTf8Escape ? s.tfs[j] : kTf8Escape);
    }
    if (positions) {
      PosPart& pt = pos_parts[id];
      const std::string& term = idx.term(id);
      std::vector<uint64_t> cum(nrows * kPackSize + 1, 0);
      uint64_t n = 0;
      for (uint64_t r = 0; r < nrows; ++r) {
        const int cnt = row_cnt(in, r, nrows);
        uint32_t tfs[kPackSize];
        if (!host_decode_block(file + s.rows[r].tf_off, fend, cnt, false, 0, tfs))
          throw std::runtime_error("cannot decode the tfs of '" + term + "'");
        for (int i = 0; i < cnt; ++i) { cum[n + 1] = cum[n] + tfs[i]; ++n; }
      }
      const uint64_t total = cum[n];
      if (total >= (1ull << 32)) throw std::runtime_error("position box of '" + term + "' over 2^32 entries");
      const uint64_t p0 = s.rows[0].pos_off;
      const uint64_t npk = total / kPackSize, rem = total % kPackSize;
      std::vector<uint64_t> blob_at(npk + (rem ? 1 : 0));
      std::vector<uint32_t> width(npk);
      uint64_t pa = p0;
      for (uint64_t k = 0; k < npk; ++k) {
        const uint8_t* b = file + pa;
        if (b + 2 > fend || b[0] != kPackMagic || b[1] < 1 || b[1] > 32)
          throw std::runtime_error("bad position pack in '" + term + "'");
        blob_at[k] = pa;
        width[k] = b[1];
        pa += 2 + 16ull * b[1];
      }
      if (rem) {
        blob_at[npk] = pa;
        pt.tail.resize(rem);
        if (file[pa] != kVIntsMagic ||
            !host_decode_block(file + pa, fend, static_cast<int>(rem), false, 0, pt.tail.data()))
          throw std::runtime_error("bad position VInts blob in '" + term + "'");
        pa += blob_bytes(file + pa, fend);
      }
      if (pa > idx.file_bytes() || pa - p0 >= (1ull << 32))
        throw std::runtime_error("position box of '" + term + "' out of range");
      for (uint64_t r = 0; r < nrows; ++r) {
        const uint64_t e = cum[r * kPackSize];
        if (s.rows[r].pos_off != blob_at[e / kPackSize] || s.rows[r].pos_idx != e % kPackSize)
          throw std::runtime_error("skip row position pointer disagrees with the box of '" + term + "'");
      }
      const uint64_t e_lo = cum[r0 * kPackSize], e_hi = cum[std::min<uint64_t>(n, r1 * kPackSize)];
      const uint64_t k0 = std::min<uint64_t>(e_lo / kPackSize, npk);
      const uint64_t k1 = std::min<uint64_t>((e_hi + kPackSize - 1) / kPackSize, npk);
      const bool with_tail = rem && e_hi > npk * kPackSize;
      const uint64_t b_lo = k0 < blob_at.size() ? blob_at[k0] : pa;
      const uint64_t b_hi = k1 < blob_at.size() ? blob_at[k1] : pa;
      for (uint64_t k = k0; k < k1; ++k) {
        pt.pk.push_back(static_cast<uint32_t>(blob_at[k] - b_lo));
        pt.pk.push_back(width[k]);
      }
      if (!with_tail) pt.tail.clear();
      pt.bytes.assign(file + b_lo, file + std::max(b_lo, b_hi));
      const uint64_t e0 = k0 * kPackSize;
      const uint64_t n_pk = k1 - k0;
      for (uint64_t r = r0; r < r1; ++r)
        for (uint64_t i = 0; i < kPackSize && r * kPackSize + i < n; ++i) {
          const uint64_t slot = (ld.blk0 + r - r0) * kPackSize + i;
          const uint64_t er = cum[r * kPackSize + i] - e0;
          img.pos_start[2 * slot] = static_cast<uint32_t>(er);
          const uint64_t kk = er / kPackSize;
          if (kk < n_pk && pt.pk[2 * kk] < (1u << 26))
            img.pos_start[2 * slot + 1] = (pt.pk[2 * kk] << 6) | pt.pk[2 * kk + 1];
        }
    }
    if (with_blm) {
      const std::string& term = idx.term(id);
      const uint8_t* pl = file + idx.list_offset(id);
      uint64_t v, so[2];
      const uint8_t* q = pl + 1;
      int l = get_varint(q, fend, &v);
      q += l;
      for (int side = 0; side < 2; ++side) {
        l = get_varint(q, fend, &so[side]);
        if (!l) throw std::runtime_error("bad bloom section pointer in '" + term + "'");
        q += l;
      }
      uint8_t* dst = &img.blm[ld.blk0 * kPackSize * 32];
      std::memset(dst, 0, (r1 - r0) * kPackSize * 32);
      for (int side = 0; side < 2; ++side) {
        const uint8_t* p = pl + so[side];
        uint64_t nbox = 0;
        if (p >= fend || p[0] != kBloomSkipListMagic || !(l = get_varint(p + 1, fend, &nbox)) || nbox != nrows)
          throw std::runtime_error("bad bloom skip list in '" + term + "'");
        p += 1 + l;
        uint64_t boff = 0;
        for (uint64_t b = 0; b < r1; ++b) {
          uint64_t d;
          if (!(l = get_varint(p, fend, &d))) throw std::runtime_error("truncated bloom skip list in '" + term + "'");
          p += l;
          boff += d;
          if (b < r0) continue;
          const uint8_t* bx = pl + boff;
          uint64_t n = 0;
          if (bx >= fend || bx[0] != kBloomBoxMagic || !(l = get_varint(bx + 1, fend, &n)) || n > kPackSize)
            throw std::runtime_error("bad bloom box in '" + term + "'");
          const uint8_t* bm = bx + 1 + l;
          const uint8_t* items = bm + (n + 7) / 8;
          if (items > fend) throw std::runtime_error("bloom box bitmap of '" + term + "' out of range");
          uint64_t phys = 0;
          for (uint64_t i = 0; i < n; ++i) {
            if (!(bm[i / 8] & (0x80u >> (i % 8)))) continue;
            const uint8_t* a = items + phys * bbytes;
            if (a + bbytes > fend) throw std::runtime_error("bloom box of '" + term + "' out of range");
            std::memcpy(dst + ((b - r0) * kPackSize + i) * 32 + side * 16, a, bbytes);
            ++phys;
          }
        }
      }
    }
  });

  lap("pass 3 (fill)");
  {
    bool any = false;
    double nm = 0.0;
    for (int c = 0; c < 256; ++c) {
      bool used = false;
      for (const Scratch& s : scratch) used = used || s.code_used[c];
      if (used && (!any || norm[c] < nm)) { nm = norm[c]; any = true; }
    }
    if (!any) {
      nm = norm[0];
      for (int c = 1; c < 256; ++c) nm = std::min(nm, norm[c]);
    }
    img.norm_min = nm;
  }
  if (positions) {
    uint64_t pb = 0;
    for (auto& p : pos_parts) pb += (p.bytes.size() + 15) & ~15ull;
    img.pos_blob.resize(pb + 64, 0);
    img.pos_lists.resize(L, PosDev{0, 0, 0, 0});
    img.pos_list_bytes.assign(L, 0);
    uint64_t pat = 0;
    for (int32_t id = 0; id < L; ++id) {
      PosPart& p = pos_parts[id];
      PosDev& pd = img.pos_lists[id];
      pd.base = pat;
      pd.pk0 = static_cast<uint32_t>(img.pos_pk.size() / 2);
      pd.npk = static_cast<uint32_t>(p.pk.size() / 2);
      pd.tail = img.pos_tail.size();
      img.pos_list_bytes[id] = p.bytes.size();
      if (!p.bytes.empty()) std::memcpy(&img.pos_blob[pat], p.bytes.data(), p.bytes.size());
      pat += (p.bytes.size() + 15) & ~15ull;
      img.pos_pk.insert(img.pos_pk.end(), p.pk.begin(), p.pk.end());
      img.pos_tail.insert(img.pos_tail.end(), p.tail.begin(), p.tail.end());
      PosPart().bytes.swap(p.bytes);
    }
  }
  return img;
}

int64_t dense_lookup_host(const HostImage& img, const ListDev& L, uint32_t doc) {
  if (L.bm == kNoDense || doc < img.doc_lo || doc >= img.doc_hi) return -1;
  const uint32_t rel = doc - img.doc_lo;
  if (rel >= img.dense_span) return -1;
  uint32_t idx = 0;
  if (const uint32_t c = probe_shift(L.bm)) {
    const uint64_t base = L.bm & kProbeBaseMask;
    const uint32_t* ent = &img.bkt[2 * (base + (rel >> c))];
    const uint8_t* offs = reinterpret_cast<const uint8_t*>(&img.bkt[2 * (base + bucket_count(img.dense_span, c))]);
    const uint32_t rank = ent[0] >> 9, cnt = ent[0] & 511u, o = rel & ((1u << c) - 1u);
    bool hit = false;
    for (uint32_t j = 0; j < cnt && !hit; ++j) {
      const uint32_t b = j < kBucketInline ? (ent[1] >> (8 * j)) & 255u : offs[rank + j];
      if (b == o) { hit = true; idx = rank + j; }
    }
    if (!hit) return -1;
  } else {
    const DenseEnt& e = img.dense[L.bm + rel / kDenseDocs];
    const uint32_t sh = rel % kDenseDocs;
    if (!dense_ent_bit(e, sh)) return -1;
    idx = dense_ent_rank(e, img.dense_rank[kRankWords * (L.bm + rel / kDenseDocs)], sh);
  }
  const uint8_t t = img.tf8[L.tf8 + idx];
  if (t != kTf8Escape) return t;
  const uint32_t j = idx / kPackSize;
  const BlockDev& bd = img.blocks[L.blk0 + j];
  const uint32_t cnt = j + 1 == L.nblk ? L.tail_cnt : kPackSize;
  uint32_t out[kPackSize];
  const uint8_t* p = img.blob.data() + L.base + bd.tf_rel;
  if (!host_decode_block(p, img.blob.data() + img.blob.size(), static_cast<int>(cnt), false, 0, out))
    return -1;
  return out[idx % kPackSize];
}

}
```

wiser_amd/csrc/index.h:

```cpp
#pragma once

#include <cstdint>
#include <string>
#include <memory>
#include <unordered_map>
#include <utility>
#include <vector>

#include "engine_types.h"

namespace wiser {

struct SkipRow {
  uint32_t prev_doc;
  uint64_t doc_off;
  uint64_t tf_off;
  uint64_t pos_off;
  uint32_t pos_idx;
  uint64_t off_off;
  uint32_t off_idx;
};

class VacuumIndex {
 public:
  VacuumIndex() = default;
  ~VacuumIndex();
  VacuumIndex(const VacuumIndex&) = delete;
  VacuumIndex& operator=(const VacuumIndex&) = delete;

  void open(const std::string& dir);

  int32_t n_lists() const { return static_cast<int32_t>(terms_.size()); }
  int32_t find(const std::string& term) const;
  int32_t find(const char* p, size_t n) const;
  void find_many(const char* const* p, const uint32_t* n, size_t cnt, int32_t* out) const;
  const std::string& term(int32_t id) const { return terms_[id]; }
  uint32_t df(int32_t id) const { return df_[id]; }
  uint64_t list_offset(int32_t id) const { return off_[id]; }
  double idf(int32_t id) const { return idf_[id]; }

  int32_t n_docs() const { return n_docs_; }
  double avg_length() const { return avg_; }
  const std::vector<uint8_t>& char4_lengths() const { return c4_; }
  const double* bm25_cache() const { return cache_; }

  std::vector<SkipRow> rows(int32_t id) const;
  void rows_into(int32_t id, std::vector<SkipRow>* out) const;
  const uint8_t* file() const { return map_; }
  bool has_bloom() const { return has_bloom_; }
  uint32_t bloom_bytes() const { return bloom_bytes_; }
  uint32_t bloom_entries() const { return bloom_entries_; }
  float bloom_ratio() const { return bloom_ratio_; }
  uint64_t file_bytes() const { return map_len_; }

 private:
  std::vector<std::string> terms_;
  std::vector<uint64_t> tslot_;
  uint64_t tmask_ = 0;
  int32_t insert_term(const char* p, size_t n, int32_t id);
  std::vector<uint64_t> off_;
  std::vector<uint32_t> df_;
  std::vector<double> idf_;
  std::vector<uint8_t> c4_;
  int32_t n_docs_ = 0;
  double avg_ = 0;
  double cache_[256] = {0};
  uint8_t* map_ = nullptr;
  uint64_t map_len_ = 0;
  bool has_bloom_ = false;
  uint32_t bloom_bytes_ = 0, bloom_entries_ = 0;
  float bloom_ratio_ = 0;
};

template <class T>
struct uninit_alloc : std::allocator<T> {
  template <class U>
  struct rebind { using other = uninit_alloc<U>; };
  uninit_alloc() = default;
  template <class U>
  uninit_alloc(const uninit_alloc<U>&) {}
  template <class U, class... A>
  void construct(U* p, A&&... a) {
    if constexpr (sizeof...(A) == 0) ::new (static_cast<void*>(p)) U;
    else ::new (static_cast<void*>(p)) U(std::forward<A>(a)...);
  }
};
template <class T>
using big_vector = std::vector<T, uninit_alloc<T>>;

struct HostImage {
  big_vector<uint8_t> blob;
  std::vector<ListDev> lists;
  big_vector<BlockDev> blocks;
  big_vector<uint32_t> blk_last;
  big_vector<uint32_t> blk_meta;
  std::vector<uint64_t> list_bytes;
  uint32_t doc_lo = 0, doc_hi = 0;
  uint64_t docid_tf_bytes = 0;
  big_vector<DenseEnt> dense;
  big_vector<uint32_t> dense_rank;
  big_vector<uint8_t> tf8;
  big_vector<uint32_t> bkt;
  uint32_t dense_span = 0;
  uint32_t dense_lists = 0;
  uint32_t bucket_lists = 0;
  big_vector<uint32_t> tails;
  big_vector<uint8_t> plen;
  big_vector<float> bmax;
  big_vector<uint8_t> impact;
  double norm_min = 0.0;
  bool has_positions = false;
  std::vector<uint8_t> pos_blob;
  std::vector<PosDev> pos_lists;
  std::vector<uint32_t> pos_pk;
  std::vector<uint32_t> pos_tail;
  std::vector<uint32_t> pos_start;
  std::vector<uint64_t> pos_list_bytes;
  bool has_blooms = false;
  uint32_t blm_bits = 0, blm_hashes = 0;
  big_vector<uint8_t> blm;
  std::vector<uint32_t> blm_hash;
};

bool host_decode_block(const uint8_t* p, const uint8_t* end, int cnt, bool delta,
                       uint32_t prev, uint32_t* out);

HostImage build_image(const VacuumIndex& idx, uint32_t doc_lo, uint32_t doc_hi, int threads,
                      uint32_t dense_div = 0, bool positions = false, uint64_t dense_budget = 0,
                      bool blooms = false, uint64_t hbm_free = 0);

int64_t dense_lookup_host(const HostImage& img, const ListDev& L, uint32_t doc);

}
```

wiser_amd/csrc/kernels.h:

```cpp
#pragma once

#include <hip/hip_runtime.h>

#include <cstdint>

#include "engine_types.h"

namespace wiser {

struct IndexArgs {
  const uint8_t* blob;
  const ListDev* lists;
  const BlockDev* blocks;
  const uint32_t* blk_last;
  const uint32_t* blk_meta;
  const uint8_t* c4;
  const double* cache;
  uint32_t n_c4;
  uint32_t n_lists;
  uint32_t doc_lo, doc_hi;
  double avg;
  const DenseEnt* dense;
  const uint32_t* dense_rk;
  const uint2* bkt;
  const uint8_t* tf8;
  uint32_t dense_span;
  float dense_ratio;
  uint32_t seg_cap;
  const uint8_t* plen;
  const float* bmax;
  const uint8_t* impact;
  float norm_min;
  const uint32_t* tails;
  const uint8_t* pos_blob;
  const PosDev* pos_lists;
  const uint2* pos_pk;
  const uint32_t* pos_tail;
  const uint2* pos_start;
  const uint4* blm;
  const uint2* blm_hash;
  uint32_t blm_bits, blm_hashes, bloom_factor;
};

enum { kCtrItems = 0, kCtrEvCap = 2, kCtrError = 4, kCtrLean = 6, kCtrLeanConj = 8, kCtrHead0 = 16,
       kQueueShards = 8,
       kCtrPHead0 = kCtrHead0 + 16 * kQueueShards,
       kCtrGHead0 = kCtrPHead0 + 16 * kQueueShards,
       kNumCounters = kCtrGHead0 + 16 * kQueueShards };
constexpr uint32_t kPlanSlotMask = 0x7FFu;
constexpr int kPlanBucketShift = 12;
constexpr uint32_t kPlanLean = 1u << 16;
constexpr uint32_t kPlanPhrase = 1u << 17;
static_assert(kMaxQueryTerms <= static_cast<int>(kPlanSlotMask) + 1, "driver slot field");
constexpr int kStatStride = 4;
enum { kErrLimit = 1, kErrCapacity = 2, kErrExchange = 4, kErrClass = 8 };
constexpr int kMaxOwners = 1024;

constexpr uint32_t kPhraseSegCap = 48;
constexpr int kCostBuckets = 5;
constexpr uint32_t kHeavyQueryItems = 4;
constexpr float kItemFixedCost = 4.0f;

struct FusedReplay {
  uint32_t* q_done;
  HitDev* hits;
  int hit_stride;
  int32_t* n_hits;
  Event* x_send;
  int32_t* x_meta;
  uint32_t* x_fill;
  uint32_t* x_err;
  uint64_t x_slot;
  uint64_t x_stride;
  uint64_t x_meta_stride;
  int32_t x_qpr;
  OwnerJob oj;
  __device__ int32_t* meta_of(uint32_t q) const {
    const uint32_t o = q / static_cast<uint32_t>(x_qpr);
    return x_meta + o * x_meta_stride + 2ull * (q - o * static_cast<uint32_t>(x_qpr));
  }
};

constexpr int kPlanThreads = 256;
struct PlanPart {
  uint32_t items[3 * kCostBuckets];
  uint64_t cap;
};

constexpr int kPhraseScratch = kMaxPhraseTerms * 256;

hipError_t launch_plan(const IndexArgs& ix, const QueryIn* q, int nq, QueryPlan* plan,
                       uint32_t* counters, uint64_t ev_capacity, uint32_t item_capacity,
                       int lean_grid, int lean_grid_ph, int seg_grid, const FusedReplay& fr, uint32_t* item_q,
                       uint64_t* pub, QueryDesc* desc, PlanPart* part, hipStream_t st);
hipError_t launch_segments(const IndexArgs& ix, const QueryIn* q, const QueryPlan* plan, int nq,
                           uint32_t* counters, Event* events, uint32_t* ev_cnt, uint32_t* stats,
                           int grid, const FusedReplay& fr, const uint32_t* item_q,
                           uint64_t* pub, uint32_t* ph, hipStream_t st);

hipError_t launch_lean(const IndexArgs& ix, const QueryIn* q, const QueryPlan* plan, int nq,
                       uint32_t* counters, Event* events, uint32_t* ev_cnt, uint32_t* stats,
                       int lean_wgs, const FusedReplay& fr, const uint32_t* item_q,
                       uint64_t* pub, const QueryDesc* desc, bool phrase, bool two, bool one,
                       hipStream_t st);
int lean_kernel_occupancy(bool phrase);
hipError_t launch_wide_replay(const QueryIn* q, const QueryPlan* plan, int nq, const Event* events,
                              const uint32_t* ev_cnt, HitDev* hits, int hit_stride, int32_t* n_hits,
                              hipStream_t st);
hipError_t launch_decode_probe(const uint8_t* p, uint32_t bits, uint32_t cnt, bool delta,
                               uint32_t seed, uint32_t* out, hipStream_t st);
hipError_t launch_owner_replay(const OwnerJob& oj, bool any_wide, hipStream_t st);
int segment_kernel_occupancy();

hipError_t launch_or_items(const IndexArgs& ix, const OrQuery* oq, const OrItem* items, uint32_t n_items,
                           int nt_max, Event* events, uint32_t* ev_cnt, uint32_t* counters,
                           unsigned long long* stats, hipStream_t st);
hipError_t launch_or_replay(const OrQuery* oq, uint32_t n_or, const OrItem* items, const Event* events,
                            const uint32_t* ev_cnt, HitDev* hits, int hit_stride, int32_t* n_hits,
                            bool narrow, bool wide, hipStream_t st);

}
```

wiser_amd/csrc/kernels.hip:

```cpp
#include <hip/hip_runtime.h>

#include <algorithm>
#include <cstdint>

#include "kernels.h"

namespace wiser {

constexpr uint32_t kNoBlock = 0xFFFFFFFFu;

__device__ __forceinline__ uint32_t uni(uint32_t x) { return __builtin_amdgcn_readfirstlane(x); }

__device__ __forceinline__ uint64_t lanemask_lt() {
  const uint32_t l = threadIdx.x & 63;
  return l ? (~0ull >> (64 - l)) : 0ull;
}

__device__ __forceinline__ double readlane_f64(double v, int lane) {
  const uint64_t u = __double_as_longlong(v);
  const uint32_t lo = __builtin_amdgcn_readlane(static_cast<uint32_t>(u), lane);
  const uint32_t hi = __builtin_amdgcn_readlane(static_cast<uint32_t>(u >> 32), lane);
  return __longlong_as_double(static_cast<long long>((static_cast<uint64_t>(hi) << 32) | lo));
}

// ... 313 lines not shown
}

template <class T>
__device__ __forceinline__ T wave_incl_scan_any(T x) {
  const uint32_t l = threadIdx.x & 63;
#pragma unroll
  for (int d = 1; d < 64; d <<= 1) {
    const T y = __shfl_up(x, d, 64);
    if (l >= static_cast<uint32_t>(d)) x += y;
  }
  return x;
}
template <int N>
struct ScanLds {
  uint32_t w[N][kPlanThreads / 64];
  uint64_t w64[kPlanThreads / 64];
};
template <int N>
__device__ __forceinline__ void block_excl_scan_n(const uint32_t (&x)[N], uint64_t y, uint32_t (&ex)[N],
                                                  uint32_t (&tot)[N], uint64_t& ey, uint64_t& toty,
                                                  ScanLds<N>& S) {
  const uint32_t w = threadIdx.x >> 6, l = threadIdx.x & 63;
  uint32_t inc[N];
#pragma unroll
  for (int k = 0; k < N; ++k) inc[k] = wave_incl_scan(x[k]);
  const uint64_t incy = wave_incl_scan_any(y);
  __syncthreads();
  if (l == 63) {
#pragma unroll
    for (int k = 0; k < N; ++k) S.w[k][w] = inc[k];
    S.w64[w] = incy;
  }
  __syncthreads();
#pragma unroll
  for (int k = 0; k < N; ++k) {
    uint32_t below = 0, t = 0;
#pragma unroll
    for (uint32_t i = 0; i < kPlanThreads / 64; ++i) {
      below += i < w ? S.w[k][i] : 0u;
      t += S.w[k][i];
    }
    ex[k] = below + inc[k] - x[k];
    tot[k] = t;
  }
  uint64_t below = 0, t = 0;
#pragma unroll
  for (uint32_t i = 0; i < kPlanThreads / 64; ++i) {
    below += i < w ? S.w64[i] : 0ull;
    t += S.w64[i];
  }
  ey = below + incy - y;
  toty = t;
}

__global__ __launch_bounds__(kPlanThreads) void plan_query_kernel(IndexArgs ix, const QueryIn* __restrict__ qs,
                                                         int nq, QueryPlan* __restrict__ plan,
                                                         uint32_t* __restrict__ counters, FusedReplay fr,
                                                         QueryDesc* __restrict__ desc,
                                                         PlanPart* __restrict__ part) {
  __shared__ ScanLds<kPlanKeys> S;
  const int i = blockIdx.x * blockDim.x + threadIdx.x;
  QueryPlan p{0, 0, 1, 0, 0};
  if (i < nq) {
    const QueryIn q = qs[i];
    const int32_t* ql = qlist_of(qs, i);
    const int nt = q.n_terms;
    bool ok = nt > 0 && q.k > 0;
    if (nt > kMaxQueryTerms || q.k > kMaxKWide || (nt > kMaxPhraseTerms && (q.flags & kQueryPhrase))) {
      ok = false;
      atomicOr(&counters[kCtrError], static_cast<uint32_t>(kErrLimit));
    }
    uint32_t d = 0, nd = 0xFFFFFFFFu, o1 = kNoSlot, min_last = 0xFFFFFFFFu;
    float cost = 1.0f;
    bool lean = true;
    if (nt <= kMaxTerms) {
      uint32_t nb[kMaxTerms], last[kMaxTerms];
      bool dn[kMaxTerms];
#pragma unroll
      for (int s = 0; s < kMaxTerms; ++s) {
        nb[s] = 0xFFFFFFFFu;
        last[s] = 0xFFFFFFFFu;
        dn[s] = false;
        const int32_t id = q.list[s];
        const bool in = s < nt;
        if (in && (id < 0 || static_cast<uint32_t>(id) >= ix.n_lists)) ok = false;
        if (in && id >= 0 && static_cast<uint32_t>(id) < ix.n_lists) {
          const ListDev& L = ix.lists[id];
          nb[s] = L.nblk;
          dn[s] = L.bm != kNoDense;
          last[s] = L.last;
        }
      }
#pragma unroll
      for (int s = 0; s < kMaxTerms; ++s)
        if (s < nt && nb[s] == 0) ok = false;
      nd = nb[0];
#pragma unroll
      for (int s = 1; s < kMaxTerms; ++s) if (nb[s] < nd) { d = s; nd = nb[s]; }
      uint32_t o_nb = 0xFFFFFFFFu;
#pragma unroll
      for (int s = 0; s < kMaxTerms; ++s) {
        if (s >= nt || s == static_cast<int>(d)) continue;
        const bool dense = use_dense(ix, dn[s], nb[s], nd);
        cost += dense ? 0.0f : fminf(static_cast<float>(nb[s]) / nd, 64.0f);
        if (!dense) lean = false;
        min_last = last[s] < min_last ? last[s] : min_last;
        if (nb[s] < o_nb) { o1 = s; o_nb = nb[s]; }
      }
    } else if (ok) {
      for (int s = 0; s < nt; ++s) {
        const int32_t id = ql[s];
        if (id < 0 || static_cast<uint32_t>(id) >= ix.n_lists) { ok = false; break; }
        const uint32_t n = ix.lists[id].nblk;
        if (n == 0) ok = false;
        if (n < nd) { d = s; nd = n; }
      }
      uint32_t o_nb = 0xFFFFFFFFu;
      for (int s = 0; ok && s < nt; ++s) {
        if (s == static_cast<int>(d)) continue;
        const ListDev& L = ix.lists[ql[s]];
        const bool dense = use_dense(ix, L.bm != kNoDense, L.nblk, nd);
        cost += dense ? 0.0f : fminf(static_cast<float>(L.nblk) / nd, 64.0f);
        if (!dense) lean = false;
        min_last = L.last < min_last ? L.last : min_last;
        if (L.nblk < o_nb) { o1 = s; o_nb = L.nblk; }
      }
    }
    lean = is_lean_query(lean, nt, q.flags);
    if (ok) {
      uint32_t seg = static_cast<uint32_t>(kSegCost / cost);
      seg = seg > ix.seg_cap ? ix.seg_cap : seg;
      if (nt == 1) seg *= kSingleWindows;
      if (is_phrase_query(nt, q.flags)) seg = seg > kPhraseSegCap ? kPhraseSegCap : seg;
      seg = seg < 1 ? 1 : (seg > nd ? nd : seg);
      const float item_cost = static_cast<float>(seg) * cost + kItemFixedCost;
      const uint32_t ic = static_cast<uint32_t>(item_cost);
      const uint32_t lg = 31u - __clz(ic > 4u ? ic : 4u);
      const uint32_t n_items = (nd + seg - 1) / seg;
      const uint32_t bucket = n_items >= kHeavyQueryItems ? static_cast<uint32_t>(kCostBuckets - 1)
                                                          : min(lg - 2u, static_cast<uint32_t>(kCostBuckets - 2));
      const bool lean_ph = lean && is_phrase_query(nt, q.flags);
      p.driver = d | (bucket << kPlanBucketShift) | (lean ? kPlanLean : 0u) | (lean_ph ? kPlanPhrase : 0u);
      p.seg_blocks = seg;
      p.n_items = n_items;
      if (lean) {
        const ListDev A = ix.lists[ql[d]];
        QueryDesc D;
        D.a_base = A.base;
        D.a_tail = A.tail;
        D.a_idf = A.idf;
        D.a_blk0 = A.blk0;
        D.a_nblk = A.nblk;
        D.a_tail_cnt = A.tail_cnt;
        D.o_bm = 0; D.o_tf8 = 0; D.o_idf = 0.0; D.o_list = 0;
        if (o1 != kNoSlot) {
          const ListDev O = ix.lists[ql[o1]];
          D.o_bm = O.bm; D.o_tf8 = O.tf8; D.o_idf = O.idf;
          D.o_list = static_cast<uint32_t>(ql[o1]);
        }
        D.min_last = min_last;
        D.ev_base = 0;
        D.item_base = 0;
        D.n_items = p.n_items;
        D.seg = seg;
        D.slots = d | (o1 << 16);
        D.k = static_cast<uint32_t>(q.k);
        double io = 0.0;
        uint32_t mm = 0;
        for (int s = 0; s < nt; ++s) {
          if (s == static_cast<int>(d)) continue;
          const ListDev& L = ix.lists[ql[s]];
          io += 2.2 * L.idf;
          mm = L.tfmax > mm ? L.tfmax : mm;
        }
        const float mf = o1 != kNoSlot ? static_cast<float>(mm) : 1.0f;
        D.b_id = static_cast<float>(2.2 * A.idf);
        D.b_m = mf;
        D.b_iom = static_cast<float>(io * static_cast<double>(mf));
        D.nt = static_cast<uint32_t>(nt);
        desc[i] = D;
      }
    }
    plan[i] = p;
    if (fr.q_done) {
      fr.q_done[i] = 0;
      if (p.n_items == 0) fr.n_hits[i] = 0;
      if (p.n_items == 0 && fr.x_meta) {
        int32_t* m = fr.meta_of(static_cast<uint32_t>(i));
        m[0] = 0;
        m[1] = 0;
      }
    }
  }
  const uint32_t key = plan_key(p.driver);
  uint32_t v[kPlanKeys], ex[kPlanKeys], tot[kPlanKeys];
#pragma unroll
  for (int k = 0; k < kPlanKeys; ++k) v[k] = key == static_cast<uint32_t>(k) ? p.n_items : 0u;
  uint64_t cex, ctot;
  block_excl_scan_n<kPlanKeys>(v, static_cast<uint64_t>(p.n_items) * p.seg_blocks * 128, ex, tot, cex, ctot, S);
  if (threadIdx.x == 0) {
#pragma unroll
    for (int k = 0; k < kPlanKeys; ++k) part[blockIdx.x].items[k] = tot[k];
    part[blockIdx.x].cap = ctot;
  }
}

__global__ __launch_bounds__(kPlanThreads) void plan_fill_kernel(int nq, QueryPlan* __restrict__ plan,
                                                        const PlanPart* __restrict__ part, int n_part,
                                                        uint32_t* __restrict__ counters,
                                                        uint64_t ev_capacity, uint32_t item_capacity,
                                                        uint32_t lean_grid, uint32_t lean_grid_ph,
                                                        uint32_t seg_grid,
                                                        uint32_t* __restrict__ item_q,
                                                        uint64_t* __restrict__ pub,
                                                        QueryDesc* __restrict__ desc) {
  __shared__ ScanLds<kPlanKeys> S;
  __shared__ uint32_t s_key_all[kPlanKeys], s_key_below[kPlanKeys];
  __shared__ uint64_t s_cap_all, s_cap_below;
  const uint32_t t = threadIdx.x;
  if (t < 64) {
    uint32_t all[kPlanKeys], below[kPlanKeys];
#pragma unroll
    for (int k = 0; k < kPlanKeys; ++k) all[k] = below[k] = 0;
    uint64_t call = 0, cbelow = 0;
    for (int g = static_cast<int>(t); g < n_part; g += 64) {
      const PlanPart P = part[g];
      const bool lo = g < static_cast<int>(blockIdx.x);
#pragma unroll
      for (int k = 0; k < kPlanKeys; ++k) { all[k] += P.items[k]; below[k] += lo ? P.items[k] : 0u; }
      call += P.cap;
      cbelow += lo ? P.cap : 0ull;
    }
#pragma unroll
    for (int k = 0; k < kPlanKeys; ++k) {
      all[k] = __builtin_amdgcn_readlane(wave_incl_scan(all[k]), 63);
      below[k] = __builtin_amdgcn_readlane(wave_incl_scan(below[k]), 63);
    }
    call = wave_incl_scan_any(call);
    cbelow = wave_incl_scan_any(cbelow);
    if (t == 63) {
#pragma unroll
      for (int k = 0; k < kPlanKeys; ++k) { s_key_all[k] = all[k]; s_key_below[k] = below[k]; }
      s_cap_all = call;
      s_cap_below = cbelow;
    }
  }
  __syncthreads();
  uint32_t key_base[kPlanKeys];
  uint32_t run = 0, n_lean = 0, n_conj = 0;
#pragma unroll
  for (int k = 0; k < kPlanKeys; ++k) {
    key_base[k] = run + s_key_below[k];
    run += s_key_all[k];
    if (k == kCostBuckets - 1) n_conj = run;
    if (k == 2 * kCostBuckets - 1) n_lean = run;
  }
  const uint32_t total_items = run;
  const bool fits = s_cap_all <= ev_capacity && total_items <= item_capacity;
  const int i = blockIdx.x * blockDim.x + t;
  QueryPlan p{0, 0, 1, 0, 0};
  if (i < nq) p = plan[i];
  const uint32_t key = plan_key(p.driver);
  uint32_t v[kPlanKeys], ex[kPlanKeys], tot[kPlanKeys];
#pragma unroll
  for (int k = 0; k < kPlanKeys; ++k) v[k] = key == static_cast<uint32_t>(k) ? p.n_items : 0u;
  const uint64_t cap = static_cast<uint64_t>(p.n_items) * p.seg_blocks * 128;
  uint64_t cex, ctot;
  block_excl_scan_n<kPlanKeys>(v, cap, ex, tot, cex, ctot, S);
  uint32_t base = 0;
#pragma unroll
  for (int k = 0; k < kPlanKeys; ++k)
    if (key == static_cast<uint32_t>(k)) base = key_base[k] + ex[k];
  const uint64_t cb = s_cap_below + cex;
  if (i < nq) {
    plan[i].item_base = base;
    plan[i].ev_base = cb;
    if (fits && (p.driver & kPlanLean)) {
      desc[i].item_base = base;
      desc[i].ev_base = cb;
    }
  }
  __shared__ ScanLds<1> S1;
  __shared__ uint32_t s_off[kPlanThreads + 1], s_base[kPlanThreads];
  const uint32_t mine[1] = {(i < nq && fits) ? p.n_items : 0u};
  uint32_t off[1], n_run[1];
  uint64_t u_ex, u_tot;
  block_excl_scan_n<1>(mine, 0ull, off, n_run, u_ex, u_tot, S1);
  s_off[t] = off[0];
  s_base[t] = base;
  if (t == 0) s_off[kPlanThreads] = n_run[0];
  __syncthreads();
  for (uint32_t j = t; j < n_run[0]; j += kPlanThreads) {
    uint32_t lo = 0, hi = kPlanThreads;
    while (hi - lo > 1) {
      const uint32_t mid = (lo + hi) >> 1;
      if (s_off[mid] <= j) lo = mid;
      else hi = mid;
    }
    const uint32_t slot = s_base[lo] + (j - s_off[lo]);
    item_q[slot] = blockIdx.x * blockDim.x + lo;
    if (pub) pub[slot] = 0;
  }
  if (blockIdx.x == 0) {
    if (t == 0) {
      if (!fits) atomicOr(&counters[kCtrError], static_cast<uint32_t>(kErrCapacity));
      if ((lean_grid == 0 && n_conj > 0) || (lean_grid_ph == 0 && n_lean > n_conj) ||
// ... 701 lines not shown
        }
        const uint32_t sh = static_cast<uint32_t>(bit - wb);
        const uint64_t x = ((static_cast<uint64_t>(w1) << 32) | w0) >> sh;
        v = static_cast<uint32_t>(x) & (bits >= 32 ? 0xFFFFFFFFu : ((1u << bits) - 1u));
      } else {
        v = pack_value(data, bits, e & 127u);
      }
    } else {
      v = ix.pos_tail[P.tail + (e - (P.npk << 7))];
    }
    ++e;
    cur += static_cast<int32_t>(v);
    return true;
  }
};

__device__ __forceinline__ bool bloom_may(const IndexArgs& ix, uint32_t slot, uint32_t side, int32_t elem) {
  const uint2 h = ix.blm_hash[elem];
  const uint4 w = ix.blm[2 * slot + side];
  for (uint32_t i = 0; i < ix.blm_hashes; ++i) {
    const uint32_t x = (h.x + i * h.y) % ix.blm_bits;
    const uint32_t q = x >> 5;
    const uint32_t d = q == 0 ? w.x : q == 1 ? w.y : q == 2 ? w.z : w.w;
    if (!((d >> (x & 31u)) & 1u)) return false;
  }
  return true;
}

__device__ __forceinline__ bool bloom_possible(const IndexArgs& ix, const int32_t* qlist, uint32_t nt,
                                               const uint32_t* ph, uint32_t v) {
  if (nt == 2) {
    const uint64_t f = ix.bloom_factor;
    const uint64_t s1 = ix.lists[qlist[0]].df, s2 = ix.lists[qlist[1]].df;
    if (f * s1 <= s2) return bloom_may(ix, ph[v], 1, qlist[1]);
    if (f * s2 < s1) return bloom_may(ix, ph[256 + v], 0, qlist[0]);
    return true;
  }
  for (uint32_t i = 0; i + 1 < nt; ++i)
    if (!bloom_may(ix, ph[i * 256 + v], 1, qlist[i + 1])) return false;
  return true;
}

__device__ __forceinline__ bool phrase_match2(const IndexArgs& ix, uint32_t l0, uint32_t l1, uint32_t slot0,
                                              uint32_t tf0, uint32_t slot1, uint32_t tf1) {
  if (ix.bloom_factor) {
    const uint64_t f = ix.bloom_factor;
    const uint64_t s1 = ix.lists[l0].df, s2 = ix.lists[l1].df;
    if (f * s1 <= s2) {
      if (!bloom_may(ix, slot0, 1, static_cast<int32_t>(l1))) return false;
    } else if (f * s2 < s1) {
      if (!bloom_may(ix, slot1, 0, static_cast<int32_t>(l0))) return false;
    }
  }
  const PosDev P0 = ix.pos_lists[l0], P1 = ix.pos_lists[l1];
  PosStream s0, s1;
  s0.init(ix, P0, slot0, tf0);
  s1.init(ix, P1, slot1, tf1);
  if (kPosPrime) {
    s0.prime();
    s1.prime();
  }
  if (!s0.next(ix, P0) || !s1.next(ix, P1)) return false;
  for (;;) {
    const int32_t a = s0.cur + 1, b = s1.cur;
    if (a == b) return true;
    if (a < b) { if (!s0.next(ix, P0)) return false; }
    else if (!s1.next(ix, P1)) return false;
  }
}

__device__ __noinline__ bool phrase_match(const IndexArgs& ix, const int32_t* qlist, uint32_t nt,
                                          const uint32_t* ph, uint32_t v) {
  if (ix.bloom_factor && !bloom_possible(ix, qlist, nt, ph, v)) return false;
  if (nt == 2) {
    const PosDev P0 = ix.pos_lists[qlist[0]], P1 = ix.pos_lists[qlist[1]];
    PosStream s0, s1;
    s0.init(ix, P0, ph[v], ph[128 + v]);
    s1.init(ix, P1, ph[256 + v], ph[384 + v]);
    if (!s0.next(ix, P0) || !s1.next(ix, P1)) return false;
    for (;;) {
      const int32_t a = s0.cur + 1, b = s1.cur;
      if (a == b) return true;
      if (a < b) { if (!s0.next(ix, P0)) return false; }
      else if (!s1.next(ix, P1)) return false;
    }
  }
  PosStream st[kMaxPhraseTerms];
#pragma unroll
  for (uint32_t i = 0; i < kMaxPhraseTerms; ++i) {
    const PosDev Pi = ix.pos_lists[i < nt ? qlist[i] : qlist[0]];
    st[i].init(ix, Pi, i < nt ? ph[i * 256 + v] : 0u, i < nt ? ph[i * 256 + 128 + v] : 0u);
    if (i < nt && !st[i].next(ix, Pi)) return false;
  }
  int32_t a = 0;
  for (;;) {
    bool moved = false;
#pragma unroll
    for (uint32_t i = 0; i < kMaxPhraseTerms; ++i) {
      if (i < nt) {
        const int32_t ii = static_cast<int32_t>(i);
        if (st[i].cur - ii < a) {
          const PosDev P = ix.pos_lists[qlist[i]];
          do {
            if (!st[i].next(ix, P)) return false;
          } while (st[i].cur - ii < a);
        }
        if (st[i].cur - ii > a) {
          a = st[i].cur - ii;
          moved = true;
        }
      }
    }
    if (!moved) return true;
  }
}

__device__ __forceinline__ uint32_t byte_word(const uint8_t* p, uint32_t* sh) {
  *sh = static_cast<uint32_t>(reinterpret_cast<uintptr_t>(p) & 3) << 3;
  return *reinterpret_cast<const uint32_t*>(__builtin_align_down(p, 4));
}

__device__ __forceinline__ void pair_words(const uint8_t* d, uint32_t b, uint32_t l, uint32_t& w0,
                                           uint32_t& w1, uint32_t& w2, uint32_t& sh) {
  const uint32_t bit = 2 * l * b;
  const uint8_t* a = d + (bit >> 3);
  const uint32_t mis = static_cast<uint32_t>(reinterpret_cast<uintptr_t>(a) & 3);
  const uint32_t* w = reinterpret_cast<const uint32_t*>(__builtin_align_down(a, 4));
  w0 = w[0];
  w1 = w[1];
  w2 = w[2];
  sh = (mis << 3) + (bit & 7);
}

__device__ __forceinline__ void pair_values(uint32_t w0, uint32_t w1, uint32_t w2, uint32_t sh,
                                            uint32_t b, uint32_t& v0, uint32_t& v1) {
  const uint32_t mask = b >= 32 ? 0xFFFFFFFFu : ((1u << b) - 1u);
  v0 = __builtin_amdgcn_alignbit(w1, w0, sh) & mask;
  const uint32_t s2 = sh + b;
  const bool up = s2 >= 32;
  v1 = __builtin_amdgcn_alignbit(up ? w2 : w1, up ? w1 : w0, s2 & 31u) & mask;
}

constexpr uint32_t kFloorRefresh = 8;
constexpr int kLeanDeep = 0;
constexpr uint32_t kLeanEvs = 64;
template <bool kPh>
struct LeanLdsT {
  uint32_t q[kPh ? 1536 : 1024];
  Event evs[kLeanEvs];
  uint4 dblk[64];
  uint32_t dmeta[64];
};

template <bool kPh, bool kTwo = false, bool kBk = false, int kDeep = 0>
__device__ __forceinline__ void lean_segment(const IndexArgs& ix, LeanLdsT<kPh>& S, const double* norm_tab,
                                             const QueryDesc& Q, const int32_t* qlist,
                                             bool phrase, uint32_t b0, uint32_t b1, bool dtail,
                                             uint32_t tdoc0, uint32_t tdoc1, uint32_t ttf0, uint32_t ttf1,
                                             uint64_t floor0, const uint64_t* prev_pub, uint32_t n_prev,
                                             uint64_t* my_pub,
                                             Event* ev_out, uint32_t& ev_n, uint32_t& evb,
                                             double& pt, uint32_t& pt_n,
                                             double& last_pub, uint32_t& n_surv, uint32_t& n_dblk,
                                             uint32_t& n_empty) {
  const uint32_t l = threadIdx.x & 63;
  const uint64_t lt = lanemask_lt();
  const uint32_t d = kTwo ? (Q.slots & 1u) : (Q.slots & 0xFFFFu);
  const uint32_t o1 = kTwo ? (d ^ 1u) : (Q.slots >> 16);
  const uint32_t nt = kTwo ? 2u : (Q.nt & 0xFFFFu), k = Q.k;
  const bool wide = !kTwo && k > static_cast<uint32_t>(kMaxK);
  const uint32_t min_last = in_vgpr(Q.min_last);
  const uint32_t* o_mk = kBk ? ix.blk_last : &ix.dense[Q.o_bm].w;
  const uint2* o_rk = kBk ? reinterpret_cast<const uint2*>(ix.blk_last)
                          : reinterpret_cast<const uint2*>(ix.dense_rk) + Q.o_bm;
  auto o_probe = [&](uint32_t e) __attribute__((always_inline)) { return o_mk[e]; };
  auto probe_bit = [&](uint32_t v, uint32_t sh) __attribute__((always_inline)) { return ((v >> sh) & 1u) != 0u; };
  auto probe_rank = [&](uint32_t v, uint32_t sh) __attribute__((always_inline)) {
    return static_cast<uint32_t>(__popc(v & ((1u << sh) - 1u)));
  };
  const uint8_t* o_tf8 = ix.tf8 + Q.o_tf8;
  const uint32_t bsh = kBk ? static_cast<uint32_t>(Q.o_bm >> kProbeShiftBit) : 0u;
  const uint2* o_bk = kBk ? ix.bkt + (Q.o_bm & kProbeBaseMask) : nullptr;
  const uint8_t* o_off = kBk ? bucket_offsets(ix, Q.o_bm) : nullptr;
  const uint32_t o_tf8_mis = static_cast<uint32_t>(reinterpret_cast<uintptr_t>(o_tf8)) & 3u;
  const uint32_t o_off_mis = static_cast<uint32_t>(reinterpret_cast<uintptr_t>(o_off)) & 3u;
  const uint8_t* a_blob = ix.blob + Q.a_base;
  const uint32_t lo = in_vgpr(ix.doc_lo), span = in_vgpr(ix.dense_span);
  const uint32_t hi_rel = in_vgpr(ix.doc_hi - ix.doc_lo);
  const double idf_d = in_vgpr(Q.a_idf), idf_o = in_vgpr(Q.o_idf);
  constexpr bool kImp = !kPh;
  uint32_t* qdoc = S.q;
  uint32_t* qc4 = qdoc + 256;
  uint32_t* qtd = qdoc + 512;
  uint32_t* qto = qdoc + 768;
  uint32_t* qpd = qdoc + (kPh ? 1024 : 256);
  uint32_t* qpo = qdoc + (kPh ? 1280 : 0);
  const uint32_t o_slot0 = (kPh && phrase) ? ix.lists[Q.o_list].blk0 * 128u : 0u;
  uint32_t qhead = 0, qtail = 0;
  uint32_t bend = b1;
  uint64_t floor_bits = prev_pub ? floor_max(floor0) : 0ull;
  double pub_val = 0.0;
  uint64_t floor_next = 0;
  double sent = 0.0;
  constexpr float kPruneMargin = 0.998f;
  const float b_idq = Q.b_id * kImpactScale;
  const float b_ob = Q.b_iom * __builtin_amdgcn_rcpf(Q.b_m + ix.norm_min);
  float thr_s = wide ? -1.0f
                     : static_cast<float>(__longlong_as_double(static_cast<long long>(
                           (static_cast<uint64_t>(uni(static_cast<uint32_t>(floor_bits >> 32))) << 32) |
                           uni(static_cast<uint32_t>(floor_bits))))) * kPruneMargin;
  auto bound = [&](uint32_t q) __attribute__((always_inline)) {
    return __builtin_fmaf(b_idq, static_cast<float>(q), b_ob);
  };
  const float b_id = Q.b_id, b_iom = Q.b_iom, b_m = Q.b_m;
  auto bound_tc = [&](uint32_t t, uint32_t c) __attribute__((always_inline)) {
    const float nf = static_cast<float>(norm_tab[c]);
    const float f = static_cast<float>(t);
    return b_id * f * __builtin_amdgcn_rcpf(f + nf) + b_iom * __builtin_amdgcn_rcpf(b_m + nf);
  };
  const uint32_t a_slot0 = Q.a_blk0 * 128u;

  auto flush = [&]() __attribute__((always_inline)) {
    __builtin_amdgcn_wave_barrier();
    if (l < evb) store_event_coherent(&ev_out[ev_n - evb + l], S.evs[l]);
    __builtin_amdgcn_wave_barrier();
    evb = 0;
  };
  auto score_chunk = [&](uint32_t n) __attribute__((always_inline)) {
    __builtin_amdgcn_wave_barrier();
    const uint32_t e = (qhead + l) & 255u;
    bool alive = l < n;
    const uint32_t doc = qdoc[e];
    const uint32_t pd = (!kImp || alive) ? qpd[e] : a_slot0 + b0 * 128u;
    uint32_t to = qto[e];
    const uint32_t po = kPh ? qpo[e] : 0u;
    const uint32_t pbi = kImp ? (pd - a_slot0) / 128u - b0 : 0u;
    const uint32_t ptb = S.dmeta[pbi] >> 8;
    const uint32_t ptw = S.dblk[pbi].w;
    uint32_t c4 = kImp ? 0u : (qc4[e] & 255u), td = kImp ? 0u : qtd[e];
    __builtin_amdgcn_wave_barrier();
    qhead += n;
    if constexpr (kImp) {
      uint32_t csh;
      const uint32_t cw = byte_word(ix.plen + pd, &csh);
      const uint32_t tb = ptb ? ptb : 1u;
      const uint32_t bit = (pd & 127u) * tb;
      const uint8_t* ta = a_blob + ptw + 2 + (bit >> 3);
      const uint32_t tsh = (static_cast<uint32_t>(reinterpret_cast<uintptr_t>(ta) & 3) << 3) + (bit & 7u);
      const uint32_t* tw = reinterpret_cast<const uint32_t*>(__builtin_align_down(ta, 4));
      const uint32_t t0 = tw[0], t1 = tw[1];
      const int tl4 = static_cast<int>((pd & 126u) << 1);
      const uint32_t v0 = static_cast<uint32_t>(__builtin_amdgcn_ds_bpermute(tl4, static_cast<int>(ttf0)));
      const uint32_t v1 = static_cast<uint32_t>(__builtin_amdgcn_ds_bpermute(tl4, static_cast<int>(ttf1)));
      c4 = (cw >> csh) & 0xFFu;
      const uint64_t both = (static_cast<uint64_t>(t1) << 32) | t0;
      td = static_cast<uint32_t>(both >> tsh) & (tb >= 32 ? 0xFFFFFFFFu : ((1u << tb) - 1u));
      if (ptb == 0) td = (pd & 1u) ? v1 : v0;
    }
    if (__ballot(alive && (to & 0x80000000u))) {
      const bool rk = alive && (to & 0x80000000u);
      uint32_t t = load_byte(o_tf8 + (rk ? (to & 0x7FFFFFFFu) : 0u));
      if (__ballot(rk && t == kTf8Escape)) {
        const ListDev O = ix.lists[Q.o_list];
        if (rk && t == kTf8Escape) t = dense_tf_slow(ix, O, to & 0x7FFFFFFFu);
      }
      if (rk) to = t;
    }
    const double norm = norm_tab[c4];
    double sc = 0.0;
    if constexpr (kTwo) {
      const double sd = bm25_term(idf_d, alive ? td : 0u, norm), so = bm25_term(idf_o, alive ? to : 0u, norm);
      if (d == 0) { sc += sd; sc += so; } else { sc += so; sc += sd; }
    }
    for (uint32_t s = 0; s < (kTwo ? 0u : nt); ++s) {
      if (s == d) {
        sc += bm25_term(idf_d, alive ? td : 0u, norm);
      } else if (s == o1) {
        sc += bm25_term(idf_o, alive ? to : 0u, norm);
      } else {
        const ListDev B = ix.lists[qlist[s]];
        uint32_t t = 0, x = 0;
        const DenseVal v = dense_load(ix, B, doc, alive);
        alive = alive && dense_resolve(ix, B, doc, v, &t, &x);
        if (__ballot(alive) == 0) break;
        sc += bm25_term(B.idf, alive ? t : 0u, norm);
      }
    }
    if (kPh && phrase && __ballot(alive)) {
      bool need = alive;
      if (!wide) {
        const uint64_t fb0 = floor_bits;
        const double flo0 = __longlong_as_double(static_cast<long long>(
            (static_cast<uint64_t>(uni(static_cast<uint32_t>(fb0 >> 32))) << 32) |
            uni(static_cast<uint32_t>(fb0))));
        const double kth0 = pt_n >= k ? readlane_f64(pt, static_cast<int>(k) - 1) : 0.0;
        need = alive && sc > flo0 && (pt_n < k || sc > kth0);
      }
      if (__ballot(need)) {
        const uint32_t so = o_slot0 + po;
        if (need)
          need = d == 0 ? phrase_match2(ix, qlist[0], qlist[1], pd, td, so, to)
                        : phrase_match2(ix, qlist[0], qlist[1], so, to, pd, td);
      }
      alive = need;
    }
    const uint64_t am = __ballot(alive);
    if (am == 0) return;
    n_surv += __popcll(am);
    if (wide) {
      if (evb + __popcll(am) > kLeanEvs) flush();
      if (alive) {
        Event ev;
        ev.score = sc;
        ev.doc = static_cast<int32_t>(doc);
        ev.pad = 0;
        S.evs[evb + __popcll(am & lt)] = ev;
      }
      ev_n += __popcll(am);
      evb += __popcll(am);
      return;
    }
    const uint64_t fb = floor_bits;
    const double flo = __longlong_as_double(static_cast<long long>(
        (static_cast<uint64_t>(uni(static_cast<uint32_t>(fb >> 32))) << 32) |
        uni(static_cast<uint32_t>(fb))));
    const double kth = pt_n >= k ? readlane_f64(pt, static_cast<int>(k) - 1) : 0.0;
    uint64_t cm = __ballot(alive && sc > flo && (pt_n < k || sc > kth));
    while (cm) {
      const int fl = __builtin_ctzll(cm);
      cm &= cm - 1;
      const double sv = readlane_f64(sc, fl);
      const uint32_t dv = __builtin_amdgcn_readlane(doc, fl);
      const uint32_t pos = __popcll(__ballot(l < pt_n && pt >= sv));
      if (pos < k) {
        if (evb == kLeanEvs) flush();
        if (l == 0) {
          Event ev;
          ev.score = sv;
          ev.doc = static_cast<int32_t>(dv);
          ev.pad = 0;
          S.evs[evb] = ev;
        }
        ++ev_n;
        ++evb;
        const double up = wave_shr1_f64(pt);
        if (l > pos) pt = up;
        else if (l == pos) pt = sv;
        pt_n = pt_n + 1 > k ? k : pt_n + 1;
      }
    }
    const double kn = pt_n >= k ? readlane_f64(pt, static_cast<int>(k) - 1) : 0.0;
    const double pv = kn > flo ? kn : flo;
    pub_val = pv > pub_val ? pv : pub_val;
    thr_s = static_cast<float>(pv) * kPruneMargin;
  };

  struct Regs {
    uint32_t w0 = 0, w1 = 0, w2 = 0;
    uint32_t wi = 0;
    uint32_t wc = 0;
    uint32_t wt0 = 0, wt1 = 0, wt2 = 0;
    uint32_t da0 = ~0u, da1 = ~0u;
    uint32_t dcc = 0, dt0 = 0, dt1 = 0;
    std::conditional_t<kBk, uint2, uint32_t> de0{}, de1{};
    uint32_t ha0 = 0, ha1 = 0;
    uint32_t hc0 = 0, hc1 = 0, ht0 = 0, ht1 = 0;
    uint2 hf0 = make_uint2(0, 0), hf1 = make_uint2(0, 0);
    uint32_t hx0 = 0x80000000u, hx1 = 0x80000000u;

  };
  Regs R0, R1;
  auto pair_shift = [&](uint32_t rel, uint32_t bits) __attribute__((always_inline)) {
    const uint32_t bit = 2 * l * bits;
    const uint32_t a = static_cast<uint32_t>(reinterpret_cast<uintptr_t>(a_blob)) + rel + 2 +
                       (bit >> 3);
    return ((a & 3u) << 3) + (bit & 7u);
  };

  auto issue_words = [&](uint32_t b, Regs& Y) __attribute__((always_inline)) {
    const uint32_t bi = b < b1 ? b - b0 : 0u;
    const uint32_t m = uni(S.dmeta[bi]);
    const uint4 e = S.dblk[bi];
    uint32_t sh;
    pair_words(a_blob + uni(e.z) + 2, (m & 0xFF) ? (m & 0xFF) : 1u, l, Y.w0, Y.w1, Y.w2, sh);
    if constexpr (kImp) {
      Y.wi = reinterpret_cast<const uint16_t*>(ix.impact)[(Q.a_blk0 + (b < b1 ? b : b0)) * 64u + l];
    } else {
      Y.wc = reinterpret_cast<const uint32_t*>(ix.plen)[(Q.a_blk0 + (b < b1 ? b : b0)) * 32u + (l >> 1)];
      pair_words(a_blob + uni(e.w) + 2, (m >> 8) ? (m >> 8) : 1u, l, Y.wt0, Y.wt1, Y.wt2, sh);
    }
  };
  auto stage_C = [&](Regs& X, Regs& Y, uint32_t j) __attribute__((always_inline)) {
    if (j >= b0 + 2 + kDeep) {
      uint32_t rk0, rk1, f0, f1, hx0 = X.hx0, hx1 = X.hx1;
      if constexpr (kBk) {
        const bool s0 = (hx0 >> 30) == 1u, s1 = (hx1 >> 30) == 1u;
        if (__ballot(s0 || s1)) {
          const uint32_t m = (1u << bsh) - 1u;
          auto resolve = [&](uint32_t hx, uint2 win, uint32_t doc) __attribute__((always_inline)) {
            const uint32_t rk = hx & 0x7FFFFFu, cn = (hx >> 23) & 127u, o = (doc - lo) & m;
            uint32_t next = 0;
            const uint32_t pos = bucket_window(win.x, win.y, (o_off_mis + rk + kBucketInline) & 3u, cn, o, &next);
            if (pos < 8u) return (rk + kBucketInline + pos) | 0x40000000u;
            if (pos == kWindowScan) {
              const uint32_t c = cn < 127u ? cn : (o_bk[(doc - lo) >> bsh].x & 511u);
              uint32_t i = 0;
              if (bucket_scan(o_off, rk, c, o, &i, next)) return i | 0x40000000u;
            }
            return 0x80000000u;
          };
          if (s0) hx0 = resolve(hx0, X.hf0, X.ha0);
          if (s1) hx1 = resolve(hx1, X.hf1, X.ha1);
        }
        rk0 = hx0 & 0x3FFFFFFFu;
        rk1 = hx1 & 0x3FFFFFFFu;
        f0 = (hx0 & 0x40000000u) ? kTf8Escape : (X.hf0.x >> (((o_tf8_mis + rk0) & 3u) << 3)) & 0xFFu;
        f1 = (hx1 & 0x40000000u) ? kTf8Escape : (X.hf1.x >> (((o_tf8_mis + rk1) & 3u) << 3)) & 0xFFu;
      } else {
        rk0 = X.hf0.x + hx0;
        rk1 = X.hf1.x + hx1;
        f0 = hx0 < 4u ? (X.hf0.y >> ((hx0 & 3u) << 3)) & 0xFFu : kTf8Escape;
        f1 = hx1 < 4u ? (X.hf1.y >> ((hx1 & 3u) << 3)) & 0xFFu : kTf8Escape;
      }
      const uint32_t to0 = f0 != kTf8Escape ? f0 : (0x80000000u | rk0);
      const uint32_t to1 = f1 != kTf8Escape ? f1 : (0x80000000u | rk1);
      const bool hh0 = !(hx0 >> 31), hh1 = !(hx1 >> 31);
      const uint64_t m0 = __ballot(hh0), m1 = __ballot(hh1);
      const uint32_t r0 = qtail + __popcll(m0 & lt) + __popcll(m1 & lt);
      const uint32_t r1 = r0 + (hh0 ? 1u : 0u);
      const uint32_t spare = (qhead - 1u) & 255u;
      const uint32_t e0 = hh0 ? (r0 & 255u) : spare, e1 = hh1 ? (r1 & 255u) : spare;
      const uint32_t pd0 = a_slot0 + (j - 2 - kDeep) * 128u + 2 * l;
      qdoc[e0] = X.ha0; qpd[e0] = pd0; qto[e0] = to0;
      qdoc[e1] = X.ha1; qpd[e1] = pd0 + 1; qto[e1] = to1;
      if (kPh) {
        qpo[e0] = rk0;
        qpo[e1] = rk1;
      }
      if (!kImp) {
        qc4[e0] = X.hc0; qtd[e0] = X.ht0;
        qc4[e1] = X.hc1; qtd[e1] = X.ht1;
      }
      qtail += __popcll(m0) + __popcll(m1);
#pragma nounroll
      for (int c = 0; c < 2 && qtail - qhead >= 64; ++c) score_chunk(64);
    }
  };
  auto stage_H = [&](Regs& X, Regs& Yh, uint32_t j) __attribute__((always_inline)) {
    Regs& Y = kDeep >= 2 ? X : Yh;
    if constexpr (kBk) {
      const uint32_t q0 = X.da0 - lo, q1 = X.da1 - lo;
      const uint32_t m = (1u << bsh) - 1u;
      const bool v0 = (X.da0 != ~0u) & (q0 < span), v1 = (X.da1 != ~0u) & (q1 < span);
      const uint32_t ps0 = bucket_pos(X.de0, q0 & m), ps1 = bucket_pos(X.de1, q1 & m);
      const bool h0 = v0 & (ps0 < kBucketInline), h1 = v1 & (ps1 < kBucketInline);
      const bool sc0 = v0 & (ps0 == kBucketScan), sc1 = v1 & (ps1 == kBucketScan);
      const uint32_t r0 = X.de0.x >> 9, r1 = X.de1.x >> 9;
      const uint32_t k0 = r0 + (h0 ? ps0 : 0u), k1 = r1 + (h1 ? ps1 : 0u);
      const uint32_t* p0 = reinterpret_cast<const uint32_t*>(
          sc0 ? __builtin_align_down(o_off + r0 + kBucketInline, 4) : __builtin_align_down(o_tf8 + (h0 ? k0 : 0u), 4));
      const uint32_t* p1 = reinterpret_cast<const uint32_t*>(
          sc1 ? __builtin_align_down(o_off + r1 + kBucketInline, 4) : __builtin_align_down(o_tf8 + (h1 ? k1 : 0u), 4));
      Y.hf0.x = p0[0];
      Y.hf1.x = p1[0];
      Y.hf0.y = p0[1];
      Y.hf1.y = p1[1];
      const uint32_t n0 = min(X.de0.x & 511u, 127u), n1 = min(X.de1.x & 511u, 127u);
      Y.hx0 = h0 ? k0 : sc0 ? (0x40000000u | (n0 << 23) | r0) : 0x80000000u;
      Y.hx1 = h1 ? k1 : sc1 ? (0x40000000u | (n1 << 23) | r1) : 0x80000000u;
      Y.ha0 = X.da0; Y.ha1 = X.da1;
      if (!kImp) {
        Y.hc0 = X.dcc & 0xFFu;
        Y.hc1 = X.dcc >> 8;
        Y.ht0 = X.dt0;
        Y.ht1 = X.dt1;
      }
    } else {
      const uint32_t q0 = X.da0 - lo, q1 = X.da1 - lo;
      const uint32_t s0 = q0 % kDenseDocs, s1 = q1 % kDenseDocs;
      const bool h0 = (X.da0 != ~0u) & (q0 < span) & probe_bit(X.de0, s0);
      const bool h1 = (X.da1 != ~0u) & (q1 < span) & probe_bit(X.de1, s1);
      const uint32_t x0 = probe_rank(X.de0, s0);
      const uint32_t x1 = probe_rank(X.de1, s1);
      Y.hf0 = o_rk[h0 ? q0 / kDenseDocs : 0u];
      Y.hf1 = o_rk[h1 ? q1 / kDenseDocs : 0u];
      Y.hx0 = h0 ? (x0 & 0x7FFFFFFFu) : 0x80000000u;
      Y.hx1 = h1 ? (x1 & 0x7FFFFFFFu) : 0x80000000u;

      Y.ha0 = X.da0; Y.ha1 = X.da1;
      if (!kImp) {
        Y.hc0 = X.dcc & 0xFFu;
        Y.hc1 = X.dcc >> 8;
        Y.ht0 = X.dt0;
        Y.ht1 = X.dt1;
      }
    }
  };
  auto stage_D = [&](Regs& X, Regs& Yd, uint32_t j) __attribute__((always_inline)) {
    Regs& Y = kDeep >= 1 ? X : Yd;
    {
      const bool live = j < bend;
      const uint32_t bi = j < b1 ? j - b0 : 0u;
      const uint4 be = S.dblk[bi];
      const uint32_t m = uni(S.dmeta[bi]);
      const uint32_t prev = uni(be.x);
      const uint32_t wbits = (m & 0xFF) ? (m & 0xFF) : 1u;
      const uint32_t cnt = live ? ((j == Q.a_nblk - 1) ? Q.a_tail_cnt : 128u) : 0u;
      uint32_t x0, x1;
      pair_values(X.w0, X.w1, X.w2, pair_shift(uni(be.z), wbits), wbits, x0, x1);
      const uint32_t sm = x0 + x1;
      const uint32_t inc = wave_incl_scan(sm);
      uint32_t a0 = prev + (inc - sm) + x0;
      uint32_t a1 = a0 + x1;
      const bool tl = live && dtail && j == b1 - 1;
      if (tl) { a0 = tdoc0; a1 = tdoc1; }
      const bool ok0 = (2 * l < cnt) & (a0 - lo < hi_rel);
      const bool ok1 = (2 * l + 1 < cnt) & (a1 - lo < hi_rel);
      bool p0, p1;
      if constexpr (kImp) {
        p0 = ok0 & (bound(X.wi & 0xFFu) > thr_s);
        p1 = ok1 & (bound((X.wi >> 8) & 0xFFu) > thr_s);
      } else {
        const uint32_t wtb = (m >> 8) ? (m >> 8) : 1u;
        uint32_t t0, t1;
        pair_values(X.wt0, X.wt1, X.wt2, pair_shift(uni(be.w), wtb), wtb, t0, t1);
        if (tl) { t0 = ttf0; t1 = ttf1; }
        const uint32_t c0 = (X.wc >> ((l & 1u) << 4)) & 0xFFu;
        const uint32_t c1 = (X.wc >> (((l & 1u) << 4) + 8)) & 0xFFu;
        p0 = ok0 & (bound_tc(t0, c0) > thr_s);
        p1 = ok1 & (bound_tc(t1, c1) > thr_s);
        Y.dcc = c0 | (c1 << 8);
        Y.dt0 = t0; Y.dt1 = t1;
      }
      const bool in0 = p0 & (a0 - lo < span);
      const bool in1 = p1 & (a1 - lo < span);
      if constexpr (kBk) {
        Y.de0 = o_bk[in0 ? (a0 - lo) >> bsh : 0u];
        Y.de1 = o_bk[in1 ? (a1 - lo) >> bsh : 0u];
      } else {
        Y.de0 = o_probe(in0 ? (a0 - lo) / kDenseDocs : 0u);
        Y.de1 = o_probe(in1 ? (a1 - lo) / kDenseDocs : 0u);
      }
      Y.da0 = p0 ? a0 : ~0u; Y.da1 = p1 ? a1 : ~0u;
      if (live) ++n_dblk;
      if (kImp && live && __ballot(ok0 | ok1) != 0 && __ballot(p0 | p1) == 0) ++n_empty;
      const uint64_t past = __ballot((ok0 & (a0 > min_last)) | (ok1 & (a1 > min_last)));
      if (live & (past != 0)) bend = j + 1;
    }
  };
  auto body = [&](Regs& X, Regs& Y, uint32_t j) __attribute__((always_inline)) {
    if (((j - b0) % kFloorRefresh) == kFloorRefresh - 1 && !wide) {
      const uint64_t fb = floor_max(floor_next);
      if (fb > floor_bits) {
        floor_bits = fb;
        const float t = static_cast<float>(__longlong_as_double(static_cast<long long>(fb))) * kPruneMargin;
        thr_s = t > thr_s ? t : thr_s;
      }
      if (my_pub && pub_val > sent) {
        if (l == 0)
          __hip_atomic_fetch_max(my_pub, static_cast<uint64_t>(__double_as_longlong(pub_val)),
                                 __ATOMIC_RELAXED, __HIP_MEMORY_SCOPE_AGENT);
        sent = pub_val;
      }
      floor_next = floor_lanes(prev_pub, n_prev);
    }
    issue_words(j + 1, Y);
    stage_C(X, Y, j);
    stage_H(X, Y, j);
    stage_D(X, Y, j);
  };
  issue_words(b0, R0);
  for (uint32_t j = b0; j < bend + 2 + kDeep; j += 2) {
    body(R0, R1, j);
    if (j + 1 >= bend + 2 + kDeep) break;
    body(R1, R0, j + 1);
  }
  if (qtail != qhead) score_chunk(qtail - qhead);
  if (my_pub && pub_val > last_pub && l == 0)
    __hip_atomic_fetch_max(my_pub, static_cast<uint64_t>(__double_as_longlong(pub_val)),
                           __ATOMIC_RELAXED, __HIP_MEMORY_SCOPE_AGENT);
  last_pub = pub_val;
  __builtin_amdgcn_wave_barrier();
}

constexpr bool kSingleQueue = true;
template <bool kPh>
__device__ __forceinline__ void single_segment(const IndexArgs& ix, LeanLdsT<kPh>& S, const double* norm_tab,
                                               const QueryDesc& Q, uint32_t b0, uint32_t b1, bool dtail,
                                               uint32_t tdoc0, uint32_t tdoc1, uint32_t ttf0, uint32_t ttf1,
                                               uint64_t floor0, const uint64_t* prev_pub, uint32_t n_prev,
                                               uint64_t* my_pub, Event* ev_out, uint32_t& ev_n, uint32_t& evb, double& pt,
                                               uint32_t& pt_n, double& last_pub, uint32_t& n_surv,
                                               uint32_t& n_dblk) {
  const uint32_t l = threadIdx.x & 63;
  const uint32_t k = Q.k;
  const bool wide = k > static_cast<uint32_t>(kMaxK);
  constexpr float kPruneMargin = 0.998f;
  const uint8_t* a_blob = ix.blob + Q.a_base;
  const uint32_t lo = in_vgpr(ix.doc_lo), hi_rel = in_vgpr(ix.doc_hi - ix.doc_lo);
  const double idf = Q.a_idf;
  const float b_id = Q.b_id, idf_f = static_cast<float>(Q.a_idf);
  uint32_t wb = b0, we = min(b0 + 64u, b1);
  float bmax = wb + l < we ? ix.bmax[Q.a_blk0 + wb + l] * idf_f : 0.0f;
  uint4 nx_dblk = {0u, 0u, 0u, 0u};
  uint32_t nx_dmeta = 0u;
  float nx_bmax = 0.0f;
  auto prefetch_window = [&](uint32_t from) __attribute__((always_inline)) {
    const uint32_t to = min(from + 64u, b1);
    if (from + l < to) {
      nx_dblk = reinterpret_cast<const uint4*>(ix.blocks)[Q.a_blk0 + from + l];
      nx_dmeta = ix.blk_meta[Q.a_blk0 + from + l];
      nx_bmax = ix.bmax[Q.a_blk0 + from + l] * idf_f;
    }
  };
  prefetch_window(we);
  const bool pre_in = !wide && b0 > 64u - l;
  const float pre = ix.bmax[Q.a_blk0 + (pre_in ? b0 - 64u + l : 0u)];
  uint64_t floor_bits = prev_pub ? floor_max(floor0) : 0ull;
  if (uni(static_cast<uint32_t>(__ballot(pre_in) != 0)) && k <= 64u) {
    uint32_t v = pre_in ? __float_as_uint(pre) : 0u;
    uint32_t kth = 0;
    for (uint32_t i = 0; i < k; ++i) {
      kth = wave_max(v);
      const uint64_t at = __ballot(v == kth);
      if (l == static_cast<uint32_t>(__builtin_ctzll(at))) v = 0u;
    }
    const double seed = idf * static_cast<double>(__uint_as_float(kth)) * (1.0 - 0x1.0p-21);
    const uint64_t sb = static_cast<uint64_t>(__double_as_longlong(seed));
    floor_bits = sb > floor_bits ? sb : floor_bits;
  }
  auto as_f64 = [](uint64_t b) __attribute__((always_inline)) {
    return __longlong_as_double(static_cast<long long>(
        (static_cast<uint64_t>(uni(static_cast<uint32_t>(b >> 32))) << 32) | uni(static_cast<uint32_t>(b))));
  };
  double flo = as_f64(floor_bits);
  float thr_s = wide ? -1.0f : static_cast<float>(flo) * kPruneMargin;
  double pub_val = 0.0, sent = 0.0;
  uint64_t floor_next = 0;
  uint32_t n_done = 0;
  auto next_block = [&](uint32_t b) __attribute__((always_inline)) {
    const uint64_t m = __ballot(wb + l >= b && bmax > thr_s);
    return m ? wb + static_cast<uint32_t>(__builtin_ctzll(m)) : we;
  };
  struct Regs {
    uint32_t w0 = 0, w1 = 0, w2 = 0, t0 = 0, t1 = 0, t2 = 0, wc = 0, b = 0;
  };
  auto issue = [&](uint32_t b, Regs& Y) __attribute__((always_inline)) {
    const uint32_t bi = b < we ? b - wb : 0u;
    const uint32_t m = uni(S.dmeta[bi]);
    const uint4 e = S.dblk[bi];
    uint32_t sh;
    pair_words(a_blob + uni(e.z) + 2, (m & 0xFF) ? (m & 0xFF) : 1u, l, Y.w0, Y.w1, Y.w2, sh);
    pair_words(a_blob + uni(e.w) + 2, (m >> 8) ? (m >> 8) : 1u, l, Y.t0, Y.t1, Y.t2, sh);
    Y.wc = reinterpret_cast<const uint32_t*>(ix.plen)[(Q.a_blk0 + (b < we ? b : wb)) * 32u + (l >> 1)];
    Y.b = b;
  };
  auto pair_shift = [&](uint32_t rel, uint32_t bits) __attribute__((always_inline)) {
    const uint32_t bit = 2 * l * bits;
    const uint32_t a = static_cast<uint32_t>(reinterpret_cast<uintptr_t>(a_blob)) + rel + 2 + (bit >> 3);
    return ((a & 3u) << 3) + (bit & 7u);
  };
  auto flush = [&]() __attribute__((always_inline)) {
    __builtin_amdgcn_wave_barrier();
    if (l < evb) store_event_coherent(&ev_out[ev_n - evb + l], S.evs[l]);
    __builtin_amdgcn_wave_barrier();
    evb = 0;
// ... 471 lines not shown
          }
          if (al1 && r1 == nd - 1) {
            p1 = lds_lower_bound(S.mb[0], B.tail_cnt, a1);
            h1 = p1 < B.tail_cnt && S.mb[0][p1] == a1;
          }
          const bool tv0 = h0 && r0 == nd - 1, tv1 = h1 && r1 == nd - 1;
          if (__ballot(tv0 || tv1)) {
            __syncthreads();
            decode_block(ix.blob + B.base + bb.tf_rel, bm >> 8, B.tail_cnt, false, 0, S.tf);
            if (tv0) t0 = S.tf[p0];
            if (tv1) t1 = S.tf[p1];
          }
          __syncthreads();
        }
        if (h0 && !(tail_vints && r0 == nd - 1)) {
          BlockDev bb;
          uint32_t bm;
          dir_entry(ix, B, S, c, wn, j0, &bb, &bm);
          t0 = pack_tf(ix.blob + B.base + bb.tf_rel, bm >> 8, p0);
        }
        if (h1 && !(tail_vints && r1 == nd - 1)) {
          BlockDev bb;
          uint32_t bm;
          dir_entry(ix, B, S, c, wn, j1, &bb, &bm);
          t1 = pack_tf(ix.blob + B.base + bb.tf_rel, bm >> 8, p1);
        }
        al0 = h0;
        al1 = h1;
        if (al0) s0 += bm25_term(B.idf, t0, nrm0);
        if (al1) s1 += bm25_term(B.idf, t1, nrm1);
        rec(s, (B.blk0 + j0) * 128u + p0, (B.blk0 + j1) * 128u + p1, t0, t1);
        if (l == 0 && nd && jlast > c && s < kMaxTerms) S.cur[s] = jlast;
      }
      if (__ballot(al0 || al1) == 0) return;
      if (phrase) {
        if (!wide) {
          const double flo0 = __longlong_as_double(static_cast<long long>(
              (static_cast<uint64_t>(uni(static_cast<uint32_t>(floor_bits >> 32))) << 32) |
              uni(static_cast<uint32_t>(floor_bits))));
          const double kth0 = pt_n >= k ? readlane_f64(pt, static_cast<int>(k) - 1) : 0.0;
          al0 = al0 && s0 > flo0 && (pt_n < k || s0 > kth0);
          al1 = al1 && s1 > flo0 && (pt_n < k || s1 > kth0);
        }
        const uint64_t m0 = __ballot(al0), m1 = __ballot(al1);
        const uint32_t n0 = __popcll(m0), nc = n0 + __popcll(m1);
        const uint32_t c0 = __popcll(m0 & lanemask_lt()), c1 = n0 + __popcll(m1 & lanemask_lt());
        bool r0 = false, r1 = false;
        for (uint32_t base = 0; base < nc; base += 64) {
          const uint32_t c = base + l;
          bool ok = false;
          if (c < nc) {
            const uint64_t m = c < n0 ? m0 : m1;
            uint32_t want = c < n0 ? c : c - n0, pos = 0;
            for (uint32_t step = 32; step; step >>= 1) {
              const uint32_t below = __popcll(m & ((2ull << (pos + step - 1)) - 1ull));
              if (below <= want) pos += step;
            }
            const uint32_t v = 2 * pos + (c < n0 ? 0u : 1u);
            ok = nt == 2 ? phrase_match2(ix, static_cast<uint32_t>(qlist[0]), static_cast<uint32_t>(qlist[1]), ph[v],
                                         ph[128 + v], ph[256 + v], ph[384 + v])
                         : phrase_match(ix, qlist, nt, ph, v);
          }
          const uint64_t res = __ballot(ok);
          if (al0 && c0 >= base && c0 < base + 64) r0 = (res >> (c0 - base)) & 1ull;
          if (al1 && c1 >= base && c1 < base + 64) r1 = (res >> (c1 - base)) & 1ull;
        }
        al0 = r0;
        al1 = r1;
        if (__ballot(al0 || al1) == 0) return;
      }
      n_surv += __popcll(__ballot(al0)) + __popcll(__ballot(al1));

      const double flo = __longlong_as_double(static_cast<long long>(
          (static_cast<uint64_t>(uni(static_cast<uint32_t>(floor_bits >> 32))) << 32) |
          uni(static_cast<uint32_t>(floor_bits))));
      const double kth = pt_n >= k ? readlane_f64(pt, static_cast<int>(k) - 1) : 0.0;
      uint64_t cm0 = __ballot(al0 && (wide || (s0 > flo && (pt_n < k || s0 > kth))));
      uint64_t cm1 = __ballot(al1 && (wide || (s1 > flo && (pt_n < k || s1 > kth))));
      while (cm0 | cm1) {
        const int fl = __builtin_ctzll(cm0 | cm1);
        const bool second = !((cm0 >> fl) & 1);
        if (second) cm1 &= cm1 - 1; else cm0 &= ~(1ull << fl);
        const double sv = readlane_f64(second ? s1 : s0, fl);
        const uint32_t dv = __builtin_amdgcn_readlane(second ? a1 : a0, fl);
        const uint32_t pos = wide ? 0u : __popcll(__ballot(l < pt_n && pt >= sv));
        if (wide || pos < k) {
          if (l == 0) {
            Event e;
            e.score = sv;
            e.doc = static_cast<int32_t>(dv);
            e.pad = 0;
            S.evs[evb] = e;
          }
          ++ev_n;
          if (++evb == 64) { flush_events(64); evb = 0; }
          if (!wide) {
            const double up = wave_shr1_f64(pt);
            if (l > pos) pt = up;
            else if (l == pos) pt = sv;
            pt_n = pt_n + 1 > k ? k : pt_n + 1;
          }
        }
      }
      if (my_pub && !wide) {
        const double kn = pt_n >= k ? readlane_f64(pt, static_cast<int>(k) - 1) : 0.0;
        const double pv = kn > flo ? kn : flo;
        if (pv > last_pub) {
          if (l == 0)
            __hip_atomic_fetch_max(my_pub, static_cast<uint64_t>(__double_as_longlong(pv)),
                                   __ATOMIC_RELAXED, __HIP_MEMORY_SCOPE_AGENT);
          last_pub = pv;
        }
      }
    };

    Stage sa, sb;
    if (b0 < b1) {
      issue_words(b0);
      fetch(b0, sa);
    }
    for (uint32_t b = b0; b < b1 && !done; b += 2) {
      step(sa, sb, b);
      if (b + 1 >= b1 || done) break;
      step(sb, sa, b + 1);
    }
    if (evb) flush_events(evb);
    finish_item<false>(qs, plan, qi, P.n_items, item, prev_pub, r, ev_out, ev_n, events, ev_cnt, fr);
    item = 0xFFFFFFFFu;
  }
  if (l == 0) {
    stats[blockIdx.x * kStatStride + 0] = n_surv;
    stats[blockIdx.x * kStatStride + 1] = n_dblk;
    stats[blockIdx.x * kStatStride + 2] = n_oblk;
  }
}


__device__ __noinline__ void owner_replay_tail(const QueryIn* qs, const int32_t* meta, const Event* recv,
                                               HitDev* hits, int32_t* n_hits, uint32_t* counters,
                                               uint32_t wave, uint32_t waves, uint64_t meta_stride,
                                               uint64_t stride, int32_t q0, int32_t nq, int32_t n_shards,
                                               int32_t hit_stride);

constexpr int kLeanWgs = kLeanDeep ? 4 : 5;
constexpr int kLeanWgsPhrase = 4;
template <bool kPh, bool kTwo = false, bool kOne = false>
__global__ __launch_bounds__(64 * kLeanWaves, kPh ? kLeanWgsPhrase : kLeanWgs) void lean_kernel(
    IndexArgs ix, const QueryIn* __restrict__ qs, const QueryPlan* __restrict__ plan, int nq,
    uint32_t* __restrict__ counters, Event* __restrict__ events, uint32_t* __restrict__ ev_cnt,
    uint32_t* __restrict__ stats, FusedReplay fr, const uint32_t* __restrict__ item_q,
    uint64_t* __restrict__ pub, const QueryDesc* __restrict__ desc) {
  __shared__ LeanLdsT<kPh> SW[kLeanWaves];
  __shared__ double norm[256];
  const uint32_t l = threadIdx.x & 63;
  const uint32_t w = uni(threadIdx.x >> 6);
  for (uint32_t i = threadIdx.x; i < 256; i += 64 * kLeanWaves) norm[i] = ix.cache[i];
  __syncthreads();
  LeanLdsT<kPh>& S = SW[w];
  const uint32_t wid = blockIdx.x * kLeanWaves + w;
  const uint32_t n_conj = uni(__hip_atomic_load(&counters[kCtrLeanConj], __ATOMIC_RELAXED,
                                                __HIP_MEMORY_SCOPE_AGENT));
  const uint32_t lo = kPh ? n_conj : 0u;
  const uint32_t n_lean = kPh ? uni(__hip_atomic_load(&counters[kCtrLean], __ATOMIC_RELAXED,
                                                      __HIP_MEMORY_SCOPE_AGENT))
                              : n_conj;
  uint32_t* heads = &counters[kPh ? kCtrPHead0 : kCtrHead0];
  uint32_t n_surv = 0, n_dblk = 0, n_empty = 0;
  uint32_t shard = wid % kQueueShards, tried = 0;
  uint32_t item = lo + wid;
  for (;;) {
    if (item >= n_lean) item = next_item(heads, lo, n_lean, shard, tried);
    if (item >= n_lean) break;
    const uint32_t qi = uni(item_q[item]);
    const QueryDesc Q = desc[qi];
    const uint32_t r = item - Q.item_base;
    const uint32_t seg = Q.seg;
    const uint32_t b0 = r * seg;
    const uint32_t b1 = min(b0 + seg, Q.a_nblk);
    Event* ev_out = events + Q.ev_base + static_cast<uint64_t>(r) * seg * 128;
    uint64_t* my_pub = pub ? pub + item : nullptr;
    const uint64_t* prev_pub = (pub && r > 0) ? pub + item - 1 : nullptr;

    const uint64_t floor0 = floor_lanes(prev_pub, r);
    __builtin_amdgcn_wave_barrier();
    if (b0 + l < b1) {
      S.dblk[l] = reinterpret_cast<const uint4*>(ix.blocks)[Q.a_blk0 + b0 + l];
      S.dmeta[l] = ix.blk_meta[Q.a_blk0 + b0 + l];
    }
    const bool dtail = b0 < b1 && b1 == Q.a_nblk && Q.a_tail != kNoTail;
    uint32_t tdoc0 = 0, tdoc1 = 0, ttf0 = 0, ttf1 = 0;
    if (dtail) {
      const uint32_t cnt = Q.a_tail_cnt;
      const uint32_t* t = ix.tails + Q.a_tail;
      if (2 * l < cnt) { tdoc0 = t[2 * l]; ttf0 = t[cnt + 2 * l]; }
      if (2 * l + 1 < cnt) { tdoc1 = t[2 * l + 1]; ttf1 = t[cnt + 2 * l + 1]; }
    }
    __builtin_amdgcn_wave_barrier();
    const uint32_t first_doc = b0 == 0 ? 0u : uni(S.dblk[0].x) + 1u;
    const bool done = first_doc > Q.min_last;
    double pt = 0.0, last_pub = 0.0;
    uint32_t pt_n = 0, ev_n = 0, evb = 0;
    if (!done && b0 < b1) {
      const bool phrase =
          kPh && (Q.nt & 0xFFFFu) > 1 && (uni(static_cast<uint32_t>(qs[qi].flags)) & kQueryPhrase);
      const int32_t* ql = qlist_of(qs, static_cast<int>(qi));
      if constexpr (kOne) {
        single_segment<kPh>(ix, S, norm, Q, b0, b1, dtail, tdoc0, tdoc1, ttf0, ttf1, floor0, prev_pub, r, my_pub,
                            ev_out, ev_n, evb, pt, pt_n, last_pub, n_surv, n_dblk);
      } else {
      if (!kTwo && !kPh && (Q.slots >> 16) == kNoSlot)
        single_segment<kPh>(ix, S, norm, Q, b0, b1, dtail, tdoc0, tdoc1, ttf0, ttf1, floor0, prev_pub, r, my_pub,
                            ev_out,
                            ev_n, evb, pt, pt_n, last_pub, n_surv, n_dblk);
      else if (uni(static_cast<uint32_t>(Q.o_bm >> kProbeShiftBit)))
        lean_segment<kPh, kTwo, true, kPh ? 0 : kLeanDeep>(ix, S, norm, Q, ql, phrase, b0, b1, dtail, tdoc0, tdoc1, ttf0, ttf1,
                                      floor0, prev_pub, r, my_pub, ev_out, ev_n, evb, pt, pt_n, last_pub, n_surv, n_dblk, n_empty);
      else
        lean_segment<kPh, kTwo, false, kPh ? 0 : kLeanDeep>(ix, S, norm, Q, ql, phrase, b0, b1, dtail, tdoc0, tdoc1, ttf0, ttf1,
                                       floor0, prev_pub, r, my_pub, ev_out, ev_n, evb, pt, pt_n, last_pub, n_surv, n_dblk, n_empty);
      }
    }
    __builtin_amdgcn_wave_barrier();
    const bool in_lds = ev_n == evb;
    double esc = 0.0;
    int32_t edc = 0;
    if (l < evb) {
      esc = S.evs[l].score;
      edc = S.evs[l].doc;
    }
    __builtin_amdgcn_wave_barrier();
    if (in_lds && Q.n_items == 1 && fr.q_done && !fr.x_send && Q.k <= static_cast<uint32_t>(kMaxK)) {
      replay_lds_call(esc, edc, evb, Q.k, fr.hits + static_cast<int64_t>(qi) * fr.hit_stride, &fr.n_hits[qi]);
      if (l == 0) ev_cnt[item] = ev_n;
    } else {
      const uint64_t* refilter = prev_pub;
      if (in_lds && prev_pub && ev_n > 0) {
        const double fl_end =
            __longlong_as_double(static_cast<long long>(floor_max(floor_lanes(prev_pub, r))));
        const bool keep = l < evb && esc > fl_end;
        const uint64_t km = __ballot(keep);
        if (keep) {
          Event e;
          e.score = esc;
          e.doc = edc;
          e.pad = 0;
          store_event_coherent(&ev_out[__popcll(km & lanemask_lt())], e);
        }
        ev_n = __popcll(km);
        refilter = nullptr;
      } else if (l < evb) {
        Event e;
        e.score = esc;
        e.doc = edc;
        e.pad = 0;
        store_event_coherent(&ev_out[ev_n - evb + l], e);
      }
      finish_item<true>(qs, plan, qi, Q.n_items, item, refilter, r, ev_out, ev_n, events, ev_cnt, fr);
    }
    item = 0xFFFFFFFFu;
  }
  if (fr.oj.nq > 0)
    owner_replay_tail(fr.oj.qs, fr.oj.meta, fr.oj.recv, fr.oj.hits, fr.oj.n_hits, fr.oj.counters, wid,
                      gridDim.x * kLeanWaves, fr.oj.meta_stride, fr.oj.stride, fr.oj.q0, fr.oj.nq,
                      fr.oj.n_shards, fr.oj.hit_stride);
  if (l == 0) {
    stats[wid * kStatStride + 0] = n_surv;
    stats[wid * kStatStride + 1] = n_dblk;
    stats[wid * kStatStride + 2] = n_empty;
  }
}

template <bool kWide>
__device__ __forceinline__ void owner_replay_query(const QueryIn* __restrict__ qs, int qi, int q0, int n_shards,
                                                   const int32_t* __restrict__ meta, uint64_t meta_stride,
                                                   uint64_t stride, const Event* __restrict__ recv,
                                                   HitDev* __restrict__ hits, int hit_stride,
                                                   int32_t* __restrict__ n_hits, uint32_t* __restrict__ counters) {
  const int gq = q0 + qi;
  const uint32_t k = uni(qs[gq].k > 0 ? static_cast<uint32_t>(qs[gq].k) : 0u);
  if ((k > static_cast<uint32_t>(kMaxK)) != kWide) return;
  const uint32_t l = threadIdx.x & 63;
  auto meta_of = [&](uint32_t g) { return meta + g * meta_stride + 2ull * static_cast<uint32_t>(qi); };
  for (uint32_t g = l; g < static_cast<uint32_t>(n_shards); g += 64)
    if (meta_of(g)[0] < 0) atomicOr(&counters[kCtrError], static_cast<uint32_t>(kErrExchange));
  auto count_of = [&](uint32_t g) {
    const int32_t c = meta_of(g)[0];
    return static_cast<uint32_t>(c > 0 ? c : 0);
  };
  auto base_of = [&](uint32_t g) { return recv + g * stride + static_cast<uint32_t>(meta_of(g)[1]); };
  if constexpr (kWide) {
    __shared__ double s_hs[kMaxKWide];
    __shared__ int32_t s_hd[kMaxKWide];
    LdsHeapSink sink;
    sink.hs = s_hs;
    sink.hd = s_hd;
    sink.k = k;
    consume_stream(sink, static_cast<uint32_t>(n_shards), count_of, base_of, [](double, int32_t) {});
    sink.finish(hits + static_cast<int64_t>(gq) * hit_stride, &n_hits[gq]);
  } else {
    HeapSink sink;
    sink.k = k;
    consume_stream(sink, static_cast<uint32_t>(n_shards), count_of, base_of, [](double, int32_t) {});
    sink.finish(hits + static_cast<int64_t>(gq) * hit_stride, &n_hits[gq]);
  }
}

template <bool kWide>
__global__ __launch_bounds__(64) void owner_replay_meta_kernel(const QueryIn* __restrict__ qs, int q0, int nq,
                                                               int n_shards, const int32_t* __restrict__ meta,
                                                               uint64_t meta_stride, uint64_t stride,
                                                               const Event* __restrict__ recv,
                                                               HitDev* __restrict__ hits, int hit_stride,
                                                               int32_t* __restrict__ n_hits,
                                                               uint32_t* __restrict__ counters) {
  const int qi = blockIdx.x;
  if (qi >= nq) return;
  owner_replay_query<kWide>(qs, qi, q0, n_shards, meta, meta_stride, stride, recv, hits, hit_stride, n_hits,
                            counters);
}

__device__ __forceinline__ const void* uni_ptr(const void* p) {
  const uint64_t v = reinterpret_cast<uint64_t>(p);
  return reinterpret_cast<const void*>(static_cast<uint64_t>(uni(static_cast<uint32_t>(v))) |
                                       (static_cast<uint64_t>(uni(static_cast<uint32_t>(v >> 32))) << 32));
}
__device__ __noinline__ void owner_replay_tail(const QueryIn* qs, const int32_t* meta, const Event* recv,
                                               HitDev* hits, int32_t* n_hits, uint32_t* counters,
                                               uint32_t wave, uint32_t waves, uint64_t meta_stride,
                                               uint64_t stride, int32_t q0, int32_t nq, int32_t n_shards,
                                               int32_t hit_stride) {
  qs = static_cast<const QueryIn*>(uni_ptr(qs));
  meta = static_cast<const int32_t*>(uni_ptr(meta));
  recv = static_cast<const Event*>(uni_ptr(recv));
  hits = static_cast<HitDev*>(const_cast<void*>(uni_ptr(hits)));
  n_hits = static_cast<int32_t*>(const_cast<void*>(uni_ptr(n_hits)));
  counters = static_cast<uint32_t*>(const_cast<void*>(uni_ptr(counters)));
  const uint32_t w0 = uni(wave), nw = uni(waves), n = uni(static_cast<uint32_t>(nq));
  const uint64_t ms = static_cast<uint64_t>(uni(static_cast<uint32_t>(meta_stride))) |
                      (static_cast<uint64_t>(uni(static_cast<uint32_t>(meta_stride >> 32))) << 32);
  const uint64_t st = static_cast<uint64_t>(uni(static_cast<uint32_t>(stride))) |
                      (static_cast<uint64_t>(uni(static_cast<uint32_t>(stride >> 32))) << 32);
  const int32_t b0 = static_cast<int32_t>(uni(static_cast<uint32_t>(q0)));
  const int32_t ns = static_cast<int32_t>(uni(static_cast<uint32_t>(n_shards)));
  const int32_t hs = static_cast<int32_t>(uni(static_cast<uint32_t>(hit_stride)));
  for (uint32_t qi = w0; qi < n; qi += nw)
    owner_replay_query<false>(qs, static_cast<int>(qi), b0, ns, meta, ms, st, recv, hits, hs, n_hits, counters);
}

struct OrLds {
  double acc[kOrWindow];
  uint32_t bits[kOrWindow / 32];
  double norm[256];
  Event evs[64];
  uint32_t cur[kMaxOrTerms];
  uint32_t cached[kMaxOrTerms];
};
static_assert(kOrWindow == 2048, "or_kernel: one bitmap word per lane");
constexpr double kOrMargin = 0.998;

__global__ __launch_bounds__(64) void or_kernel(IndexArgs ix, const OrQuery* __restrict__ oqs,
                                                const OrItem* __restrict__ items, uint32_t n_items,
                                                Event* __restrict__ events, uint32_t* __restrict__ ev_cnt,
                                                uint32_t* __restrict__ counters,
                                                unsigned long long* __restrict__ stats) {
  __shared__ OrLds S;
  extern __shared__ uint32_t or_cache[];
// ... 345 lines not shown
```

Before: 26.77 million queries/s.

## Add 16-bit delta doc-id side array for eligible lists in two-term lean path

Builds a per-block array of 16-bit doc-id offsets from each block's prev doc for lists whose full packed blocks span at most 65535 docs, uploads it to the device, and records its base in the query descriptor. In the two-term conjunctive lean kernel, eligible driver lists read doc ids straight from this array instead of unpacking bit-packed words and doing a wave-wide prefix scan. This removes decode arithmetic and a scan per block, at the cost of extra HBM footprint, another load stream, and more template instances and code size. It is enabled by default through WSR_DOC16.

```diff
diff --git a/include/wiser_hip.h b/include/wiser_hip.h
--- a/include/wiser_hip.h
+++ b/include/wiser_hip.h
@@ -90,6 +90,7 @@
   uint64_t pos_bytes;
   uint32_t n_lists, dense_lists;
   uint64_t impact_bytes;
+  uint64_t doc16_bytes;
 } wsr_image_info;
 
 const char* wsr_last_error(void);
@@ -214,6 +215,11 @@
                            const char* term, const uint32_t* docs, int32_t n, int32_t* tf_out,
                            int32_t* is_dense);
 
+int wsr_debug_doc16(const char* dir, uint32_t doc_lo, uint32_t doc_hi, const char* term, int32_t max_blocks,
+                    uint16_t* out, uint32_t* prev, int32_t* n_blocks, int32_t* eligible, int32_t* probe);
+int wsr_doc16_survey(const char* dir, const char* const* terms, int32_t n, uint32_t* n_blocks,
+                     uint32_t* pack_blocks, uint32_t* ok_blocks, int32_t* eligible);
+
 typedef struct wsr_build_stats {
   int64_t n_docs, n_terms, n_postings, vacuum_bytes, docs_char4_ge_0x80;
   double avg_length;
diff --git a/wiser_amd/_capi.py b/wiser_amd/_capi.py
--- a/wiser_amd/_capi.py
+++ b/wiser_amd/_capi.py
@@ -61,7 +61,7 @@
     _fields_ = [("total_bytes", C.c_uint64), ("blob_bytes", C.c_uint64), ("dense_bytes", C.c_uint64),
                 ("tf8_bytes", C.c_uint64), ("plen_bytes", C.c_uint64), ("dir_bytes", C.c_uint64),
                 ("pos_bytes", C.c_uint64), ("n_lists", C.c_uint32), ("dense_lists", C.c_uint32),
-                ("impact_bytes", C.c_uint64)]
+                ("impact_bytes", C.c_uint64), ("doc16_bytes", C.c_uint64)]
 
 
 class ServeStats(C.Structure):
@@ -157,6 +157,11 @@
     "wsr_debug_dense_lookup": (C.c_int, [C.c_char_p, C.c_uint32, C.c_uint32, C.c_uint32, C.c_char_p,
                                          C.POINTER(C.c_uint32), C.c_int32, C.POINTER(C.c_int32),
                                          C.POINTER(C.c_int32)]),
+    "wsr_debug_doc16": (C.c_int, [C.c_char_p, C.c_uint32, C.c_uint32, C.c_char_p, C.c_int32,
+                                  C.POINTER(C.c_uint16), C.POINTER(C.c_uint32), C.POINTER(C.c_int32),
+                                  C.POINTER(C.c_int32), C.POINTER(C.c_int32)]),
+    "wsr_doc16_survey": (C.c_int, [C.c_char_p, C.POINTER(C.c_char_p), C.c_int32, C.POINTER(C.c_uint32),
+                                   C.POINTER(C.c_uint32), C.POINTER(C.c_uint32), C.POINTER(C.c_int32)]),
     "wsr_build_from_linedoc": (C.c_int, [C.c_char_p, C.c_int64, C.c_char_p, C.c_char_p,
                                          C.POINTER(BuildStats)]),
     "wsr_build_from_linedoc_bloom": (C.c_int, [C.c_char_p, C.c_int64, C.c_char_p, C.c_char_p,
diff --git a/wiser_amd/csrc/engine.cc b/wiser_amd/csrc/engine.cc
--- a/wiser_amd/csrc/engine.cc
+++ b/wiser_amd/csrc/engine.cc
@@ -58,6 +58,10 @@
                 dev_bytes(img.blk_meta) + dev_bytes(img.bmax) + std::max<uint64_t>(n_c4, 1);
   o.impact_bytes = dev_bytes(img.impact);
   o.dir_bytes += o.impact_bytes;
+  if (!img.doc16.empty()) {
+    o.doc16_bytes = dev_bytes(img.doc16);
+    o.dir_bytes += o.doc16_bytes + dev_bytes(img.d16_blk);
+  }
   o.dense_lists = img.dense_lists;
   o.n_lists = static_cast<uint32_t>(img.lists.size());
   o.total_bytes = o.blob_bytes + o.dense_bytes + o.tf8_bytes + o.plen_bytes + o.dir_bytes + o.pos_bytes;
@@ -66,6 +70,7 @@
 
 uint32_t dense_div_knob() { return static_cast<uint32_t>(env_number("WSR_DENSE_DIV", 8192)); }
 uint64_t dense_budget_knob() { return static_cast<uint64_t>(env_number("WSR_DENSE_BUDGET_GB", 48) * 1e9); }
+bool doc16_knob() { return env_number("WSR_DOC16", 1) != 0; }
 }
 
 extern "C" {
@@ -90,7 +95,8 @@
     idx.open(dir);
     const int t = threads > 0 ? threads : static_cast<int>(std::thread::hardware_concurrency());
     const HostImage img = build_image(idx, doc_lo, doc_hi ? doc_hi : 0xFFFFFFFFu, std::min(t, 32), dense_div_knob(),
-                                      positions != 0, dense_budget_knob(), positions && bloom_factor > 0);
+                                      positions != 0, dense_budget_knob(), positions && bloom_factor > 0, 0,
+                                      doc16_knob());
     *out = image_info_of(img, idx.char4_lengths().size());
   } catch (const std::exception& e) {
     return fail(WSR_E_IO, e.what());
@@ -138,7 +144,7 @@
     size_t hbm_free = 0, hbm_total = 0;
     HIP_OK(hipMemGetInfo(&hbm_free, &hbm_total));
     HostImage img = build_image(h->idx, lo, hi, std::min(threads, 32), dense_div, h->positions, dense_budget,
-                                bloom_factor > 0, hbm_free);
+                                bloom_factor > 0, hbm_free, doc16_knob());
     if (img.has_blooms) {
       h->info.pos_bytes += dev_upload(h->d_blm, img.blm);
       h->info.pos_bytes += dev_upload(h->d_blm_hash, img.blm_hash);
@@ -184,6 +190,13 @@
     h->info.impact_bytes = dev_upload(h->d_impact, img.impact);
     h->info.dir_bytes += h->info.impact_bytes;
     h->args.impact = h->d_impact.get();
+    if (!img.doc16.empty()) {
+      h->info.doc16_bytes = dev_upload(h->d_doc16, img.doc16);
+      h->info.dir_bytes += h->info.doc16_bytes + dev_upload(h->d_d16_blk, img.d16_blk);
+      h->args.doc16 = h->d_doc16.get();
+      h->args.d16_blk = h->d_d16_blk.get();
+      big_vector<uint16_t>().swap(img.doc16);
+    }
     {
       float nm = static_cast<float>(img.norm_min);
       if (static_cast<double>(nm) > img.norm_min) nm = std::nextafter(nm, 0.0f);
@@ -1068,6 +1081,53 @@
   return WSR_OK;
 }
 
+int wsr_debug_doc16(const char* dir, uint32_t doc_lo, uint32_t doc_hi, const char* term, int32_t max_blocks,
+                    uint16_t* out, uint32_t* prev, int32_t* n_blocks, int32_t* eligible, int32_t* probe) {
+  if (!dir || !term || !n_blocks || !eligible || !probe || max_blocks < 0 || (max_blocks > 0 && (!out || !prev)))
+    return fail(WSR_E_INVALID, "bad argument");
+  try {
+    VacuumIndex idx;
+    idx.open(dir);
+    const HostImage img = build_image(idx, doc_lo, doc_hi ? doc_hi : 0xFFFFFFFFu, 4, dense_div_knob(), false,
+                                      dense_budget_knob(), false, 0, doc16_knob());
+    const int32_t id = idx.find(term);
+    if (id < 0) return fail(WSR_E_INVALID, "no such term");
+    const ListDev& L = img.lists[id];
+    *n_blocks = static_cast<int32_t>(L.nblk);
+    *probe = L.bm == kNoDense ? -1 : static_cast<int32_t>(probe_shift(L.bm));
+    *eligible = !img.d16_blk.empty() && img.d16_blk[id] != kNoDoc16;
+    for (uint32_t b = 0; b < L.nblk && b < static_cast<uint32_t>(max_blocks); ++b) {
+      prev[b] = img.blocks[L.blk0 + b].prev;
+      if (*eligible)
+        std::memcpy(out + 128ull * b, &img.doc16[(static_cast<uint64_t>(img.d16_blk[id]) + b) * 128],
+                    128 * sizeof(uint16_t));
+    }
+  } catch (const std::exception& e) {
+    return fail(WSR_E_IO, e.what());
+  }
+  return WSR_OK;
+}
+
+int wsr_doc16_survey(const char* dir, const char* const* terms, int32_t n, uint32_t* n_blocks,
+                     uint32_t* pack_blocks, uint32_t* ok_blocks, int32_t* eligible) {
+  if (!dir || (n > 0 && (!terms || !n_blocks || !pack_blocks || !ok_blocks || !eligible)))
+    return fail(WSR_E_INVALID, "null argument");
+  try {
+    VacuumIndex idx;
+    idx.open(dir);
+    for (int32_t i = 0; i < n; ++i) {
+      const int32_t id = terms[i] ? idx.find(terms[i]) : -1;
+      n_blocks[i] = pack_blocks[i] = ok_blocks[i] = 0;
+      bool ok = false;
+      if (id >= 0) doc16_survey(idx, id, &n_blocks[i], &pack_blocks[i], &ok_blocks[i], &ok);
+      eligible[i] = ok ? 1 : 0;
+    }
+  } catch (const std::exception& e) {
+    return fail(WSR_E_IO, e.what());
+  }
+  return WSR_OK;
+}
+
 static void fill_stats(const BuildStats& s, wsr_build_stats* st) {
   if (!st) return;
   st->n_docs = s.n_docs;
diff --git a/wiser_amd/csrc/engine_impl.h b/wiser_amd/csrc/engine_impl.h
--- a/wiser_amd/csrc/engine_impl.h
+++ b/wiser_amd/csrc/engine_impl.h
@@ -55,6 +55,8 @@
   gpu::DevBuf<uint32_t> d_dense_rk;
   gpu::DevBuf<uint32_t> d_bkt;
   gpu::DevBuf<uint8_t> d_tf8, d_plen, d_impact;
+  gpu::DevBuf<uint16_t> d_doc16;
+  gpu::DevBuf<uint32_t> d_d16_blk;
   gpu::DevBuf<float> d_bmax;
   gpu::DevBuf<uint32_t> d_tails;
   gpu::DevBuf<uint8_t> d_pos_blob;
diff --git a/wiser_amd/csrc/engine_types.h b/wiser_amd/csrc/engine_types.h
--- a/wiser_amd/csrc/engine_types.h
+++ b/wiser_amd/csrc/engine_types.h
@@ -39,6 +39,12 @@
   uint32_t q = static_cast<uint32_t>(x * 255.0);
   while (q < 255 && impact_value(q) < x) ++q;
   return static_cast<uint8_t>(q);
+}
+
+constexpr uint32_t kDoc16Span = 65535;
+constexpr uint32_t kNoDoc16 = ~0u;
+inline bool doc16_block_ok(bool full_pack, uint32_t prev, uint32_t last) {
+  return full_pack && last >= prev && last - prev <= kDoc16Span;
 }
 
 constexpr uint32_t kProbeShiftBit = 56;
@@ -128,7 +134,9 @@
   uint64_t o_bm;
   uint64_t o_tf8;
   uint64_t ev_base;
-  uint64_t rsv0, rsv1;
+  uint32_t a_d16;
+  uint32_t rsv0;
+  uint64_t rsv1;
   double a_idf, o_idf;
   uint32_t a_blk0, a_nblk, a_tail_cnt;
   uint32_t min_last;
diff --git a/wiser_amd/csrc/index.cc b/wiser_amd/csrc/index.cc
--- a/wiser_amd/csrc/index.cc
+++ b/wiser_amd/csrc/index.cc
@@ -327,9 +327,20 @@
 }
 }
 
+template <class Last, class Cnt>
+static bool doc16_list_ok(const uint8_t* file, const SkipRow* rows, uint64_t r0, uint64_t r1, bool vtail, Last last,
+                          Cnt cnt) {
+  const uint64_t np = r1 - r0 - (vtail ? 1 : 0);
+  bool ok = r1 > r0 && np > 0;
+  for (uint64_t r = r0; r < r0 + np && ok; ++r)
+    ok = doc16_block_ok(file[rows[r].doc_off] == kPackMagic && cnt(r) == kPackSize, rows[r].prev_doc, last(r));
+  return ok;
+}
+constexpr uint64_t kDoc16MaxBlocks = 1ull << 26;
+
 HostImage build_image(const VacuumIndex& idx, uint32_t doc_lo, uint32_t doc_hi, int threads,
                       uint32_t dense_div, bool positions, uint64_t dense_budget, bool blooms,
-                      uint64_t hbm_free) {
+                      uint64_t hbm_free, bool doc16) {
   const int32_t L = idx.n_lists();
   const uint8_t* file = idx.file();
   const uint8_t* fend = file + idx.file_bytes();
@@ -345,6 +356,7 @@
     uint64_t bytes = 0;
     uint8_t dense = 0, vtail = 0;
     uint8_t shift = 0;
+    uint8_t d16 = 0;
   };
   std::vector<Info> info(L);
   struct Scratch {
@@ -405,6 +417,9 @@
     in.tail_cnt = (r1 == nrows) ? in.fcnt : kPackSize;
     in.vtail = r1 == nrows && file[s.rows[nrows - 1].doc_off] == kVIntsMagic;
     const uint64_t n_img = (r1 - r0 - 1) * kPackSize + in.tail_cnt;
+    if (doc16)
+      in.d16 = doc16_list_ok(file, s.rows.data(), r0, r1, in.vtail, [&](uint64_t r) { return s.last[r]; },
+                             [&](uint64_t r) { return row_cnt(in, r, nrows); });
     if (dense_div && span && n_img * dense_div >= span) {
       bool ok = true;
       const uint64_t lim = static_cast<uint64_t>(doc_lo) + span;
@@ -460,7 +475,8 @@
       const Info& in = info[id];
       if (in.r1 <= in.r0) continue;
       const uint64_t nbl = in.r1 - in.r0;
-      other += in.bytes + nbl * (sizeof(BlockDev) + 12 + 2 * kPackSize) + (in.vtail ? 8ull * in.tail_cnt : 0);
+      other += in.bytes + nbl * (sizeof(BlockDev) + 12 + (in.d16 ? 4 : 2) * kPackSize) +
+               (in.vtail ? 8ull * in.tail_cnt : 0);
       if (blooms && positions) other += nbl * kPackSize * 32;
     }
     const uint64_t cap = hbm_free / 10 * 9;
@@ -490,7 +506,15 @@
   img.lists.resize(L);
   img.list_bytes.resize(L);
   img.has_positions = positions;
-  uint64_t at = 0, nb = 0, ne = 0, ntf8 = 0, ntail = 0, nbk = 0;
+  uint64_t at = 0, nb = 0, ne = 0, ntf8 = 0, ntail = 0, nbk = 0, nd16 = 0;
+  {
+    uint64_t want = 0;
+    for (int32_t id = 0; id < L; ++id)
+      if (info[id].d16) want += info[id].r1 - info[id].r0;
+    if (want >= kDoc16MaxBlocks)
+      for (int32_t id = 0; id < L; ++id) info[id].d16 = 0;
+  }
+  if (doc16) img.d16_blk.assign(L, kNoDoc16);
   for (int32_t id = 0; id < L; ++id) {
     const Info& in = info[id];
     ListDev& ld = img.lists[id];
@@ -508,6 +532,7 @@
     ld.tfmax = 0;
     if (!nbl) { img.list_bytes[id] = 0; continue; }
     if (in.vtail) { ld.tail = ntail; ntail += 2ull * in.tail_cnt; }
+    if (in.d16) { img.d16_blk[id] = static_cast<uint32_t>(nd16); nd16 += nbl; }
     if (in.dense) {
       const uint64_t n_img = (nbl - 1) * static_cast<uint64_t>(kPackSize) + in.tail_cnt;
       if (in.shift) {
@@ -535,6 +560,7 @@
   img.blk_meta.resize(nb);
   img.plen.resize(nb * kPackSize);
   img.impact.resize(nb * kPackSize);
+  img.doc16.resize(nd16 * kPackSize);
   img.bmax.resize(nb);
   img.tails.resize(ntail);
   img.dense.resize(ne);
@@ -626,6 +652,12 @@
         s.code_used[o[i]] = true;
       }
       for (int i = cnt; i < kPackSize; ++i) im[i] = 0;
+      if (in.d16) {
+        uint16_t* dd = &img.doc16[(img.d16_blk[id] + (r - r0)) * kPackSize];
+        const int n16 = last_vints ? 0 : cnt;
+        for (int i = 0; i < n16; ++i) dd[i] = static_cast<uint16_t>(docs[i] - s.rows[r].prev_doc);
+        for (int i = n16; i < kPackSize; ++i) dd[i] = 0;
+      }
       float bmf = static_cast<float>(bm);
       if (static_cast<double>(bmf) < bm) bmf = std::nextafter(bmf, std::numeric_limits<float>::infinity());
       img.bmax[j] = bmf;
@@ -870,4 +902,31 @@
   return out[idx % kPackSize];
 }
 
-}
+void doc16_survey(const VacuumIndex& idx, int32_t id, uint32_t* nblk, uint32_t* pack_blocks, uint32_t* ok_blocks,
+                  bool* list_ok) {
+  const std::vector<SkipRow> rows = idx.rows(id);
+  const uint8_t* file = idx.file();
+  const uint64_t nrows = rows.size();
+  const uint32_t df = idx.df(id);
+  if (nrows == 0 || nrows != (df + kPackSize - 1) / kPackSize)
+    throw std::runtime_error("skip rows do not match df for '" + idx.term(id) + "'");
+  const uint32_t fcnt = static_cast<uint32_t>(df - kPackSize * (nrows - 1));
+  uint32_t tmp[kPackSize];
+  if (!host_decode_block(file + rows[nrows - 1].doc_off, file + idx.file_bytes(), static_cast<int>(fcnt), true,
+                         rows[nrows - 1].prev_doc, tmp))
+    throw std::runtime_error("cannot decode the last block of '" + idx.term(id) + "'");
+  uint32_t np = 0, ok = 0;
+  auto last = [&](uint64_t r) { return r + 1 < nrows ? rows[r + 1].prev_doc : tmp[fcnt - 1]; };
+  auto cnt = [&](uint64_t r) { return r + 1 < nrows ? kPackSize : static_cast<int>(fcnt); };
+  for (uint64_t r = 0; r < nrows; ++r) {
+    const bool full = file[rows[r].doc_off] == kPackMagic && cnt(r) == kPackSize;
+    np += full;
+    ok += doc16_block_ok(full, rows[r].prev_doc, last(r));
+  }
+  *nblk = static_cast<uint32_t>(nrows);
+  *pack_blocks = np;
+  *ok_blocks = ok;
+  *list_ok = doc16_list_ok(file, rows.data(), 0, nrows, file[rows[nrows - 1].doc_off] == kVIntsMagic, last, cnt);
+}
+
+}
diff --git a/wiser_amd/csrc/index.h b/wiser_amd/csrc/index.h
--- a/wiser_amd/csrc/index.h
+++ b/wiser_amd/csrc/index.h
@@ -108,6 +108,8 @@
   big_vector<uint8_t> plen;
   big_vector<float> bmax;
   big_vector<uint8_t> impact;
+  big_vector<uint16_t> doc16;
+  std::vector<uint32_t> d16_blk;
   double norm_min = 0.0;
   bool has_positions = false;
   std::vector<uint8_t> pos_blob;
@@ -127,7 +129,10 @@
 
 HostImage build_image(const VacuumIndex& idx, uint32_t doc_lo, uint32_t doc_hi, int threads,
                       uint32_t dense_div = 0, bool positions = false, uint64_t dense_budget = 0,
-                      bool blooms = false, uint64_t hbm_free = 0);
+                      bool blooms = false, uint64_t hbm_free = 0, bool doc16 = false);
+
+void doc16_survey(const VacuumIndex& idx, int32_t id, uint32_t* nblk, uint32_t* pack_blocks, uint32_t* ok_blocks,
+                  bool* list_ok);
 
 int64_t dense_lookup_host(const HostImage& img, const ListDev& L, uint32_t doc);
 
diff --git a/wiser_amd/csrc/kernels.h b/wiser_amd/csrc/kernels.h
--- a/wiser_amd/csrc/kernels.h
+++ b/wiser_amd/csrc/kernels.h
@@ -30,6 +30,8 @@
   const uint8_t* plen;
   const float* bmax;
   const uint8_t* impact;
+  const uint16_t* doc16;
+  const uint32_t* d16_blk;
   float norm_min;
   const uint32_t* tails;
   const uint8_t* pos_blob;
diff --git a/wiser_amd/csrc/kernels.hip b/wiser_amd/csrc/kernels.hip
--- a/wiser_amd/csrc/kernels.hip
+++ b/wiser_amd/csrc/kernels.hip
@@ -489,6 +489,8 @@
         D.a_blk0 = A.blk0;
         D.a_nblk = A.nblk;
         D.a_tail_cnt = A.tail_cnt;
+        D.a_d16 = ix.d16_blk ? ix.d16_blk[ql[d]] : kNoDoc16;
+        D.rsv0 = 0; D.rsv1 = 0;
         D.o_bm = 0; D.o_tf8 = 0; D.o_idf = 0.0; D.o_list = 0;
         if (o1 != kNoSlot) {
           const ListDev O = ix.lists[ql[o1]];
@@ -1496,7 +1498,7 @@
   uint32_t dmeta[64];
 };
 
-template <bool kPh, bool kTwo = false, bool kBk = false, int kDeep = 0>
+template <bool kPh, bool kTwo = false, bool kBk = false, int kDeep = 0, bool kD16 = false>
 __device__ __forceinline__ void lean_segment(const IndexArgs& ix, LeanLdsT<kPh>& S, const double* norm_tab,
                                              const QueryDesc& Q, const int32_t* qlist,
                                              bool phrase, uint32_t b0, uint32_t b1, bool dtail,
@@ -1533,6 +1535,7 @@
   const uint32_t hi_rel = in_vgpr(ix.doc_hi - ix.doc_lo);
   const double idf_d = in_vgpr(Q.a_idf), idf_o = in_vgpr(Q.o_idf);
   constexpr bool kImp = !kPh;
+  static_assert(!kD16 || kImp, "16-bit doc ids: the conjunctive instances only");
   uint32_t* qdoc = S.q;
   uint32_t* qc4 = qdoc + 256;
   uint32_t* qtd = qdoc + 512;
@@ -1726,7 +1729,10 @@
     const uint32_t m = uni(S.dmeta[bi]);
     const uint4 e = S.dblk[bi];
     uint32_t sh;
-    pair_words(a_blob + uni(e.z) + 2, (m & 0xFF) ? (m & 0xFF) : 1u, l, Y.w0, Y.w1, Y.w2, sh);
+    if constexpr (kD16)
+      Y.w0 = reinterpret_cast<const uint32_t*>(ix.doc16)[(Q.a_d16 + (b < b1 ? b : b0)) * 64u + l];
+    else
+      pair_words(a_blob + uni(e.z) + 2, (m & 0xFF) ? (m & 0xFF) : 1u, l, Y.w0, Y.w1, Y.w2, sh);
     if constexpr (kImp) {
       Y.wi = reinterpret_cast<const uint16_t*>(ix.impact)[(Q.a_blk0 + (b < b1 ? b : b0)) * 64u + l];
     } else {
@@ -1850,12 +1856,18 @@
       const uint32_t prev = uni(be.x);
       const uint32_t wbits = (m & 0xFF) ? (m & 0xFF) : 1u;
       const uint32_t cnt = live ? ((j == Q.a_nblk - 1) ? Q.a_tail_cnt : 128u) : 0u;
-      uint32_t x0, x1;
-      pair_values(X.w0, X.w1, X.w2, pair_shift(uni(be.z), wbits), wbits, x0, x1);
-      const uint32_t sm = x0 + x1;
-      const uint32_t inc = wave_incl_scan(sm);
-      uint32_t a0 = prev + (inc - sm) + x0;
-      uint32_t a1 = a0 + x1;
+      uint32_t a0, a1;
+      if constexpr (kD16) {
+        a0 = prev + (X.w0 & 0xFFFFu);
+        a1 = prev + (X.w0 >> 16);
+      } else {
+        uint32_t x0, x1;
+        pair_values(X.w0, X.w1, X.w2, pair_shift(uni(be.z), wbits), wbits, x0, x1);
+        const uint32_t sm = x0 + x1;
+        const uint32_t inc = wave_incl_scan(sm);
+        a0 = prev + (inc - sm) + x0;
+        a1 = a0 + x1;
+      }
       const bool tl = live && dtail && j == b1 - 1;
       if (tl) { a0 = tdoc0; a1 = tdoc1; }
       const bool ok0 = (2 * l < cnt) & (a0 - lo < hi_rel);
@@ -2633,6 +2645,7 @@
     uint64_t* __restrict__ pub, const QueryDesc* __restrict__ desc) {
   __shared__ LeanLdsT<kPh> SW[kLeanWaves];
   __shared__ double norm[256];
+  constexpr bool kD16Item = kTwo && !kPh;
   const uint32_t l = threadIdx.x & 63;
   const uint32_t w = uni(threadIdx.x >> 6);
   for (uint32_t i = threadIdx.x; i < 256; i += 64 * kLeanWaves) norm[i] = ix.cache[i];
@@ -2693,6 +2706,12 @@
         single_segment<kPh>(ix, S, norm, Q, b0, b1, dtail, tdoc0, tdoc1, ttf0, ttf1, floor0, prev_pub, r, my_pub,
                             ev_out,
                             ev_n, evb, pt, pt_n, last_pub, n_surv, n_dblk);
+      else if (kD16Item && uni(Q.a_d16) != kNoDoc16 && uni(static_cast<uint32_t>(Q.o_bm >> kProbeShiftBit)))
+        lean_segment<kPh, kTwo, true, kPh ? 0 : kLeanDeep, kD16Item>(ix, S, norm, Q, ql, phrase, b0, b1, dtail, tdoc0, tdoc1, ttf0, ttf1,
+                                      floor0, prev_pub, r, my_pub, ev_out, ev_n, evb, pt, pt_n, last_pub, n_surv, n_dblk, n_empty);
+      else if (kD16Item && uni(Q.a_d16) != kNoDoc16)
+        lean_segment<kPh, kTwo, false, kPh ? 0 : kLeanDeep, kD16Item>(ix, S, norm, Q, ql, phrase, b0, b1, dtail, tdoc0, tdoc1, ttf0, ttf1,
+                                       floor0, prev_pub, r, my_pub, ev_out, ev_n, evb, pt, pt_n, last_pub, n_surv, n_dblk, n_empty);
       else if (uni(static_cast<uint32_t>(Q.o_bm >> kProbeShiftBit)))
         lean_segment<kPh, kTwo, true, kPh ? 0 : kLeanDeep>(ix, S, norm, Q, ql, phrase, b0, b1, dtail, tdoc0, tdoc1, ttf0, ttf1,
                                       floor0, prev_pub, r, my_pub, ev_out, ev_n, evb, pt, pt_n, last_pub, n_surv, n_dblk, n_empty);
```

Result: faster. 27.28 million queries/s, median of 6 (+1.9%).
